# calavera/patrol

Hardware: AMD Instinct MI355X
Metric: bucket-state merges/sec + achieved HBM GB/s at 1/2/4/8 MI355X (higher is better)
Workload: dtype f64; 1 GPU; C2 merge: 100000000 replica messages -> 10000000-bucket table (2^25 slots), Zipf(1.1); keys_per_gpu=10000000, slots_per_gpu=33554432, parallelism=shard1, name_bytes=2-8 (b<id>), world_size=1, full=False, exchange=False, batches_in_hbm=28

## Files before the change

### patrol_amd/csrc/phip_engine.hip

```cpp
#include <sys/random.h>

#include <chrono>
#include <cstdlib>
#include <cstring>
#include <hip/hip_runtime.h>
#include <rocprim/rocprim.hpp>

#include <algorithm>
#include <cstdarg>
#include <cstdio>
#include <cstring>
#include <mutex>
#include <string>
#include <vector>

#include "patrolhip.h"
#include "phip_kernels.hpp"
#include "phip_host.hpp"

using namespace phip;

namespace {

#ifndef PHIP_SORT_BITS
#define PHIP_SORT_BITS 9
#endif
#ifndef PHIP_SORT_BLOCK
#define PHIP_SORT_BLOCK 1024
#endif
#ifndef PHIP_SORT_ITEMS
#define PHIP_SORT_ITEMS 8
#endif
using SlotSortConfig = rocprim::radix_sort_config<
    rocprim::default_config, rocprim::default_config,
    rocprim::radix_sort_onesweep_config<
        rocprim::kernel_config<PHIP_SORT_BLOCK, PHIP_SORT_ITEMS>,
        rocprim::kernel_config<PHIP_SORT_BLOCK, PHIP_SORT_ITEMS>, PHIP_SORT_BITS,
        rocprim::block_radix_rank_algorithm::match>>;

enum BufId {
  B_NAMES, B_OFFS, B_A, B_T, B_E, B_KIND, B_NOW, B_FREQ, B_PER, B_COUNT,
  B_STATUS, B_REM, B_HAVE, B_REPLY,
  B_BYTES, B_DOFFS, B_NOFF, B_NLEN, B_DA, B_DT, B_DE,
  B_MISS, B_MISS2, B_RETRY, B_CSLOT, B_CMSG,
  B_SLOT, B_IDX, B_SSLOT, B_SIDX, B_USLOT, B_SCNT, B_SSTART, B_LONG, B_HUGE, B_TEMP, B_DUMP,
  B_OPS, B_HOFF, B_HOP, B_HVAL, B_RPOS, B_RST, B_RUNN, B_SEGEX, B_WOFF, B_SUMS, B_WRUN,
  B_WING, B_SEGXF, B_FOLDDBG, B_SMALL, B_HUGE2, B_LONG2,
  B_STATES, B_NAME1, B_HOT, B_ROUTE, B_EXPORT, B_MSHARD, B_MSCNT, B_FSCNT, B_DEDUP, B_DSET, B_TSTATS, B_SEGT, B_RHOT,
  B_DLIST, B_DTAB, B_DMARK, B_SMAP, B_SOFF, B_SLEN, B_SA, B_ST, B_SE, B_SSTAT, B_SREP, B_NCHK,
  B_EVICT, B_ULOG, B_ULCNT, B_SWEEP, B_DIGEST, B_DIGOUT,
  B_COUNT_
};

struct DevBuf {
  void* p = nullptr;
  size_t cap = 0;
};

struct Timing {
  const char* name;
  hipEvent_t a, b;
};

enum class PassKind { kOptimistic, kClassified, kIsolating };
struct FastPass {
  PassKind kind = PassKind::kClassified;
  u32 n = 0;
  u32 par = 0;
  u32* c = nullptr;
  const HotHdr* hot = nullptr;
  const HotEntry* dir = nullptr;
  void* hot_zero = nullptr;
  bool hot_join = false;
  u8* mark = nullptr;
  UndoLog log{};
};

}

struct phip_handle {
  int device = 0;
  int ncu = 256;
  bool iso_always = false;
  u32 iso_left = 0;
  bool classify_first = false;
  u32 opt_left = 0;
  struct LastStats {
    uint64_t hot_entries = 0, hot_hits = 0, misses = 0;
    uint64_t ordered = 0;
    uint64_t log_count = 0, log_over = 0;
  } stats;
  hipStream_t stream = nullptr;
  hipStream_t own_stream = nullptr;
  hipStream_t stream2 = nullptr;
  hipStream_t stream3 = nullptr;
  hipStream_t stream4 = nullptr;
  hipEvent_t ev_t4a = nullptr, ev_t4b = nullptr;
  hipEvent_t ev_fork = nullptr, ev_join = nullptr;
  void* hot_clean = nullptr;
  hipEvent_t ev_fork3 = nullptr, ev_join3 = nullptr;
  hipEvent_t ev_gather = nullptr, ev_gather3 = nullptr;
  hipEvent_t ev_pack = nullptr;
  std::mutex mu;
  std::string err;
  u32 L = 0;
  u32 L_open = 0;
  u64 cap = 0;
  u64 max_load = 0;
  u32 load_pct = 90;
  bool grow = true;
  bool small = true;
  u64 grows = 0;
  u64 layout_gen = 1;
  u64 long_need = 0;
  Rec* recs = nullptr;
  u32* aux = nullptr;
  u8* arena = nullptr;
  u64 arena_cap = 0;
  u64 arena_open = 0;
  u64* arena_cursor = nullptr;
  u32* ctr = nullptr;
  u32* ctr_host = nullptr;
  u32* ctr_map = nullptr;
  u32 fpar = 0;
  u64 nfast = 0;
  u64 n_buckets = 0;
  u64 tag_mask = ~0ull;
  u64 seed = 0;
  DevBuf buf[B_COUNT_];
  bool timing = false;
  bool timing_accumulate = false;
  std::vector<Timing> timings;
  std::vector<Timing> event_pool;
  size_t pool_used = 0;
  u8* small_pin = nullptr;
  size_t small_pin_cap = 0;
  struct Pending {
    bool active = false;
    SoaIn<NamesOffs> in{};
    i64 now = 0;
    OutView ow{};
    FastPass pass{};
  } pend;
  hipEvent_t ev_ctr = nullptr;
  int deferred_rc = 0;
};

namespace {

int set_err(phip_handle* h, int code, const char* fmt, ...) {
  char tmp[512];
  va_list ap;
  va_start(ap, fmt);
  vsnprintf(tmp, sizeof tmp, fmt, ap);
  va_end(ap);
  if (h) h->err = tmp;
  return code;
}

#define HIPCHK(h, x)                                                                      \
  do {                                                                                    \
    hipError_t e_ = (x);                                                                  \
    if (e_ != hipSuccess)                                                                 \
      return set_err((h), PHIP_ERR_HIP, "%s failed: %s (%s:%d)", #x, hipGetErrorString(e_), \
                     __FILE__, __LINE__);                                                 \
  } while (0)

template <class T>
int ensure(phip_handle* h, BufId id, size_t count, T** out) {
  size_t bytes = std::max<size_t>(count * sizeof(T), 64) + 64;
  DevBuf& b = h->buf[id];
  if (b.cap < bytes) {
    size_t want = std::max(bytes, b.cap * 3 / 2);
    if (b.p) HIPCHK(h, hipFree(b.p));
    b.p = nullptr;
    b.cap = 0;
    HIPCHK(h, hipMalloc(&b.p, want));
    b.cap = want;
  }
  *out = (T*)b.p;
  return PHIP_OK;
}

inline Table table(phip_handle* h) {
  Table t;
  t.recs = h->recs;
  t.aux = h->aux;
  t.arena = h->arena;
  t.L = h->L;
  t.tag_mask = h->tag_mask;
  t.seed = h->seed;
  return t;
}

inline unsigned grid_for(u64 n, unsigned block = kBlock) {
  return (unsigned)std::max<u64>(1, (n + block - 1) / block);
}

struct Launch {
  phip_handle* h;
  const char* name;
  size_t idx = ~size_t(0);
  hipStream_t s;
  Launch(phip_handle* h_, const char* n, hipStream_t st = nullptr)
      : h(h_), name(n), s(st ? st : h_->stream) {
    if (!h->timing) return;
    if (h->pool_used == h->event_pool.size()) {
      Timing tm{n, nullptr, nullptr};
      if (hipEventCreate(&tm.a) != hipSuccess) return;
      if (hipEventCreate(&tm.b) != hipSuccess) {
        (void)hipEventDestroy(tm.a);
        return;
      }
      h->event_pool.push_back(tm);
    }
    idx = h->pool_used++;
    h->event_pool[idx].name = n;
    if (hipEventRecord(h->event_pool[idx].a, s) != hipSuccess) idx = ~size_t(0);
  }
  ~Launch() {
    if (idx < h->event_pool.size()) {
      Timing& t = h->event_pool[idx];
      if (hipEventRecord(t.b, s) == hipSuccess) h->timings.push_back(t);
    }
  }
};

int read_ctr(phip_handle* h) {
  HIPCHK(h, hipMemcpyAsync(h->ctr_host, h->ctr, kCtrWords * sizeof(u32), hipMemcpyDeviceToHost,
                           h->stream));
  HIPCHK(h, hipStreamSynchronize(h->stream));
  return PHIP_OK;
}

int reset_ctr(phip_handle* h) {
  k_batch_reset<<<1, kShards, 0, h->stream>>>(h->ctr, nullptr);
  HIPCHK(h, hipGetLastError());
  return PHIP_OK;
}

int check_flags(phip_handle* h) {
  if (h->ctr_host[kCtrBadName])
    return set_err(h, PHIP_ERR_INVALID, "malformed name offsets (names_len check): nothing applied");
  if (h->ctr_host[kCtrTableFull]) return set_err(h, PHIP_ERR_FULL, "hash table full (probe wrapped)");
  if (h->ctr_host[kCtrArenaFull]) return set_err(h, PHIP_ERR_ARENA, "long-name arena exhausted");
  return PHIP_OK;
}

template <int N>
int copy_words(const uint64_t (&v)[N], uint64_t* out, int max) {
  int k = 0;
  for (; k < max && k < N; ++k) out[k] = v[k];
  return k;
}

int finish_pending(phip_handle* h, bool* worked = nullptr);
int after_error(phip_handle* h, int rc);

int begin_call(phip_handle* h, bool finish_queued = true) {
  if (h->deferred_rc) {
    const int rc = h->deferred_rc;
    h->deferred_rc = 0;
    return rc;
  }
  h->err.clear();
  if (h->timing && !h->timing_accumulate) {
    h->timings.clear();
    h->pool_used = 0;
  }
  HIPCHK(h, hipSetDevice(h->device));
  if (finish_queued && h->pend.active) {
    int rc = finish_pending(h);
    if (rc) return after_error(h, rc);
  }
  return PHIP_OK;
}

template <class T>
int stage(phip_handle* h, BufId id, const T* src, size_t count, bool dev, const T** out) {
  if (!src) { *out = nullptr; return PHIP_OK; }
  if (dev) { *out = src; return PHIP_OK; }
  T* d;
  int rc = ensure(h, id, count, &d);
  if (rc) return rc;
  if (count) HIPCHK(h, hipMemcpyAsync(d, src, count * sizeof(T), hipMemcpyHostToDevice, h->stream));
  *out = d;
  return PHIP_OK;
}

template <class T>
int out_buf(phip_handle* h, BufId id, T* user, size_t count, bool dev, T** out) {
  if (!user) { *out = nullptr; return PHIP_OK; }
  if (dev) { *out = user; return PHIP_OK; }
  return ensure(h, id, count, out);
}

template <class T>
int copy_back(phip_handle* h, T* user, const T* dev_buf, size_t count, bool dev) {
  if (!user || dev || !count) return PHIP_OK;
  HIPCHK(h, hipMemcpyAsync(user, dev_buf, count * sizeof(T), hipMemcpyDeviceToHost, h->stream));
  return PHIP_OK;
}

inline u64 load_limit(u64 cap, u32 pct) { return cap * pct / 100; }

int grow_table(phip_handle* h, u32 newL) {
  const u64 ncap = 1ull << newL;
  Rec* nrecs = nullptr;
  u32* naux = nullptr;
  if (hipMalloc(&nrecs, ncap * sizeof(Rec)) != hipSuccess) {
    (void)hipGetLastError();
    return set_err(h, PHIP_ERR_FULL, "table growth to 2^%u slots: device memory", newL);
  }
  if (hipMalloc(&naux, ncap * sizeof(u32)) != hipSuccess) {
    (void)hipGetLastError();
    (void)hipFree(nrecs);
    return set_err(h, PHIP_ERR_FULL, "table growth to 2^%u slots: device memory", newL);
  }
  auto drop_new = [&](int rc) {
    (void)hipStreamSynchronize(h->stream);
    (void)hipFree(nrecs);
    (void)hipFree(naux);
    return rc;
  };
  if (hipMemsetAsync(nrecs, 0, ncap * sizeof(Rec), h->stream) != hipSuccess ||
      hipMemsetAsync(naux, 0, ncap * sizeof(u32), h->stream) != hipSuccess ||
      hipMemsetAsync(h->ctr + kCtrTableFull, 0, sizeof(u32), h->stream) != hipSuccess)
    return drop_new(set_err(h, PHIP_ERR_HIP, "table growth: clearing the new table failed"));
  Table nt = table(h);
  nt.recs = nrecs;
  nt.aux = naux;
  nt.L = newL;
  {
    Launch l(h, "k_rehash");
    k_rehash<<<grid_for(h->cap), kBlock, 0, h->stream>>>(h->recs, h->aux, h->cap, nt, h->ctr);
  }
  if (hipGetLastError() != hipSuccess)
    return drop_new(set_err(h, PHIP_ERR_HIP, "k_rehash launch failed"));
  int rc;
  if ((rc = read_ctr(h))) return drop_new(rc);
  if (h->ctr_host[kCtrTableFull])
    return drop_new(set_err(h, PHIP_ERR_INVALID, "internal: rehash probe wrapped"));
  HIPCHK(h, hipFree(h->recs));
  HIPCHK(h, hipFree(h->aux));
  h->recs = nrecs;
  h->aux = naux;
  h->L = newL;
  h->cap = ncap;
  h->max_load = load_limit(ncap, h->load_pct);
  ++h->grows;
  ++h->layout_gen;
  return PHIP_OK;
}

int grow_arena(phip_handle* h, u64 used, u64 want) {
  u64 ncap = std::max<u64>(h->arena_cap * 2, want);
  u8* na = nullptr;
  if (hipMalloc(&na, ncap + 64) != hipSuccess) {
    (void)hipGetLastError();
    return set_err(h, PHIP_ERR_ARENA, "arena growth to %llu bytes: device memory",
                   (unsigned long long)ncap);
  }
  if (used) HIPCHK(h, hipMemcpyAsync(na, h->arena, used, hipMemcpyDeviceToDevice, h->stream));
  HIPCHK(h, hipStreamSynchronize(h->stream));
  HIPCHK(h, hipFree(h->arena));
  h->arena = na;
  h->arena_cap = ncap;
  return PHIP_OK;
}

template <class Src>
int reserve(phip_handle* h, Src src, const u32* list, u32 nlist, u64 bound, bool* grew) {
  u64* lb = (u64*)(h->ctr + kCtrLongBytes);
  HIPCHK(h, hipMemsetAsync(lb, 0, sizeof(u64), h->stream));
  k_list_long_bytes<Src><<<grid_for(nlist), kBlock, 0, h->stream>>>(src, nlist, list, lb);
  HIPCHK(h, hipGetLastError());
  u64 used = 0;
  HIPCHK(h, hipMemcpyAsync(&used, h->arena_cursor, sizeof(u64), hipMemcpyDeviceToHost, h->stream));
  int rc;
  if ((rc = read_ctr(h))) return rc;
  u64 need;
  std::memcpy(&need, h->ctr_host + kCtrLongBytes, sizeof need);
  h->long_need = need;
  if (used + need > h->arena_cap) {
    if (!h->grow)
      return set_err(h, PHIP_ERR_ARENA, "long-name arena: %llu of %llu bytes used, %llu more needed",
                     (unsigned long long)used, (unsigned long long)h->arena_cap,
                     (unsigned long long)need);
    if ((rc = grow_arena(h, used, used + need))) return rc;
  }
  if (h->n_buckets + bound > h->max_load) {
    u32 L = h->L;
    while (L < 31 && h->n_buckets + bound > load_limit(1ull << L, h->load_pct)) ++L;
    if (!h->grow || h->n_buckets + bound > load_limit(1ull << L, h->load_pct))
      return set_err(h, PHIP_ERR_FULL,
                     "table load limit: %llu buckets + up to %llu new > %llu allowed in 2^%u slots",
                     (unsigned long long)h->n_buckets, (unsigned long long)bound,
                     (unsigned long long)(h->grow ? load_limit(1ull << L, h->load_pct) : h->max_load),
                     h->grow ? L : h->L);
    if ((rc = grow_table(h, L))) return rc;
    *grew = true;
  }
  return PHIP_OK;
}

template <class Src>
int dedupe_names(phip_handle* h, Src src, const u32* list, u32 n, u32** out, u32* nout);

template <class Src>
int insert_names(phip_handle* h, Src src, u32* list, u32 nlist, const int64_t* now_arr, i64 now0,
                 u32* n_claimed, bool* grew = nullptr, bool distinct = false) {
  u32 *cslot, *cmsg, *retry, *cur = list;
  int rc;
  *n_claimed = 0;
  bool g = false;
  u64 bound = nlist;
  const u32* blist = list;
  u32 nb = nlist;
  if (!distinct && nlist > 1 && h->n_buckets + nlist > h->max_load) {
    u32 *dd, nd = 0;
    if ((rc = dedupe_names(h, src, list, nlist, &dd, &nd))) return rc;
    if (h->tag_mask == ~0ull) {
      bound = nd;
      blist = dd;
      nb = nd;
    }
  }
  if ((rc = reserve(h, src, blist, nb, bound, &g))) return rc;
  if (grew) *grew = g;
  if ((rc = ensure(h, B_CSLOT, nlist, &cslot)) || (rc = ensure(h, B_CMSG, nlist, &cmsg)) ||
      (rc = ensure(h, B_RETRY, nlist, &retry)))
    return rc;
  u32 total = 0, ncur = nlist;
  HIPCHK(h, hipMemsetAsync(h->ctr + kCtrClaimed, 0, sizeof(u32), h->stream));
  u32* nxt = retry;
  u32* spare = nullptr;
  if ((rc = ensure(h, B_MISS2, nlist, &spare))) return rc;
  while (ncur > 0) {
    HIPCHK(h, hipMemsetAsync(h->ctr + kCtrRetry, 0, sizeof(u32), h->stream));
    {
      Launch l(h, "k_claim");
      k_claim<Src><<<grid_for(ncur), kBlock, 0, h->stream>>>(src, ncur, cur, table(h), cslot, cmsg,
                                                              nxt, h->ctr);
    }
    HIPCHK(h, hipGetLastError());
    if ((rc = read_ctr(h))) return rc;
    u32 claimed_total = h->ctr_host[kCtrClaimed];
    u32 fresh = claimed_total - total;
    if (fresh) {
      Launch l(h, "k_publish");
      k_publish<Src><<<grid_for(fresh), kBlock, 0, h->stream>>>(
          src, total, fresh, cslot, cmsg, table(h), h->arena, h->arena_cap, h->arena_cursor, now_arr,
          now0, h->ctr);
    }
    HIPCHK(h, hipGetLastError());
    h->n_buckets += fresh;
    total = claimed_total;
    *n_claimed = total;
    ncur = h->ctr_host[kCtrRetry];
    if ((rc = check_flags(h))) return rc;
    if (fresh == 0 && ncur != 0)
      return set_err(h, PHIP_ERR_INVALID, "internal: insert round made no progress");
    cur = nxt;
    nxt = (nxt == retry) ? spare : retry;
  }
  *n_claimed = total;
  if (h->long_need) {
    if ((rc = read_ctr(h)) || (rc = check_flags(h))) return rc;
  }
  return PHIP_OK;
}

int clear_new(phip_handle* h, u32 n_claimed) {
  if (!n_claimed) return PHIP_OK;
  u32* cslot = (u32*)h->buf[B_CSLOT].p;
  Launch l(h, "k_clear_new");
  k_clear_new<<<grid_for(n_claimed), kBlock, 0, h->stream>>>(cslot, n_claimed, table(h));
  HIPCHK(h, hipGetLastError());
  return PHIP_OK;
}

int after_error(phip_handle* h, int rc) {
  if (rc == PHIP_OK) return rc;
  if (h->stream2) (void)hipStreamSynchronize(h->stream2);
  if (h->stream3) (void)hipStreamSynchronize(h->stream3);
  if (h->stream4) (void)hipStreamSynchronize(h->stream4);
  if (rc == PHIP_ERR_HIP) return rc;
  std::string keep = h->err;
  k_clear_new_all<<<grid_for(h->cap), kBlock, 0, h->stream>>>(table(h), h->cap);
  if (hipGetLastError() == hipSuccess) (void)hipStreamSynchronize(h->stream);
  h->err = keep;
  return rc;
}

template <class Src>
int build_hot(phip_handle* h, Src src, u32 n, hipStream_t st, u8* status, const HotHdr** hdr_out,
              const HotEntry** dir_out, void** zero_out) {
  *hdr_out = nullptr;
  *dir_out = nullptr;
  *zero_out = nullptr;
  if (n < kHotMinBatch) return PHIP_OK;
  constexpr size_t kCnt = size_t(1) << kHotCntBits;
  u8* base;
  int rc;
  if ((rc = ensure(h, B_HOT, kHotZeroBytes + kHotCandMax * sizeof(u32) + sizeof(HotHdr) +
                                 kHotMax * sizeof(HotEntry), &base)))
    return rc;
  u32* ckeys = (u32*)base;
  u32* ccnt = ckeys + kCnt;
  u32* sync = ccnt + kCnt;
  u32* cand = sync + kHotSyncWords;
  HotHdr* hdr = (HotHdr*)(cand + kHotCandMax);
  HotEntry* dir = (HotEntry*)(hdr + 1);
  if (h->hot_clean != base) HIPCHK(h, hipMemsetAsync(base, 0, kHotZeroBytes, st));
  h->hot_clean = nullptr;
  const u32 stride = std::max<u32>(64, (n + kHotSampleMax - 1) / kHotSampleMax);
  const u32 nsample = (n + stride - 1) / stride;
  {
    Launch l(h, "k_hot_dir", st);
    if (status) {
      constexpr unsigned kT = kHotAloneThreads;
      const unsigned nblk = grid_for(nsample, kT);
      const unsigned fill =
          std::min<unsigned>(grid_for(n, kT * 64), 1024 / kT * (unsigned)h->ncu);
      k_hot_dir<Src, kT, 1><<<nblk + fill, kT, 0, st>>>(
          src, n, stride, nsample, table(h), ckeys, ccnt, sync, cand, hdr, dir, nblk, status);
    } else {
      const unsigned nblk = grid_for(nsample, kHotSamplePerBlock);
      k_hot_dir<Src, 256, 4><<<nblk, 256, 0, st>>>(
          src, n, stride, nsample, table(h), ckeys, ccnt, sync, cand, hdr, dir, nblk, nullptr);
    }
  }
  HIPCHK(h, hipGetLastError());
  *hdr_out = hdr;
  *dir_out = dir;
  *zero_out = base;
  return PHIP_OK;
}

inline unsigned fast_grid_on(u32 ncu, u32 n) {
  const u64 tiles = ((u64)n + kFastBlock - 1) / kFastBlock;
  return (unsigned)std::max<u64>(1, std::min<u64>(tiles, (u64)ncu * kFastPerCU));
}
inline unsigned fast_grid(phip_handle* h, u32 n) { return fast_grid_on((u32)h->ncu, n); }


int sharded(phip_handle* h, BufId base_id, u32 units, u32 per_unit, Sharded* out,
            bool zero = true) {
  int rc;
  out->cap = shard_cap(units, per_unit);
  if ((rc = ensure(h, base_id, (size_t)kShards * out->cap, &out->base)) ||
      (rc = ensure(h, B_MSCNT, 2 * kShards, &out->cnt)))
    return rc;
  if (zero) HIPCHK(h, hipMemsetAsync(out->cnt, 0, kShards * sizeof(u32), h->stream));
  return PHIP_OK;
}

int pack_sharded(phip_handle* h, const Sharded& sh, u32 total_slot, u32* out, u32* total) {
  k_shard_scan<<<1, kShards, 0, h->stream>>>(sh.cnt, h->ctr, total_slot, nullptr, 0, nullptr,
                                             nullptr);
  HIPCHK(h, hipGetLastError());
  int rc;
  if ((rc = read_ctr(h))) return rc;
  *total = h->ctr_host[total_slot];
  if (*total) {
    Launch l(h, "k_shard_compact");
    dim3 grid(grid_for(h->ctr_host[kCtrShardMax]), kShards);
    k_shard_compact<<<grid, 256, 0, h->stream>>>(sh.base, sh.cap, sh.cnt, out);
    HIPCHK(h, hipGetLastError());
  }
  return PHIP_OK;
}


enum class PassAsk { kPolicy, kMayUndo, kIsolate, kNoIsolate };

template <class In>
PassKind pass_kind(const phip_handle* h, PassAsk ask) {
  if (ask == PassAsk::kIsolate) return PassKind::kIsolating;
  if (ask == PassAsk::kNoIsolate) return PassKind::kClassified;
  if (h->iso_always || h->iso_left > 0) return PassKind::kIsolating;
  if (ask == PassAsk::kMayUndo && In::kSoa && !h->classify_first && h->opt_left == 0)
    return PassKind::kOptimistic;
  return PassKind::kClassified;
}

inline size_t undo_counts(const phip_handle* h) { return (size_t)h->ncu * kFastPerCU * (kFastBlock / 64); }

struct UndoLayout {
  u32 grid, waves, cap;
  u64 halves;
};
inline UndoLayout undo_layout(u32 n, u32 ncu) {
  UndoLayout l;
  l.grid = fast_grid_on(ncu, n);
  l.waves = l.grid * (kFastBlock / 64);
  l.cap = undo_wave_cap(n, l.grid);
  l.halves = (u64)l.waves * l.cap * 2;
  return l;
}

inline u32* fctr(phip_handle* h, u32 par) { return h->ctr + kCtrWords * (1 + par); }

inline u32* fast_counts(phip_handle* h, u32 par) {
  return (u32*)h->buf[B_FSCNT].p + par * 2 * kShards;
}

int dirty_set(phip_handle* h, DirtySet* d, u32** dlist) {
  int rc;
  u64* b;
  if ((rc = ensure(h, B_DTAB, DirtySet::kWords, &b)) || (rc = ensure(h, B_DLIST, kDirtyCap, dlist)))
    return rc;
  *d = DirtySet::at(b);
  return PHIP_OK;
}
struct SubBatch {
  uint64_t *off, *a, *t;
  int64_t* e;
  u8* len;
  u32* map;
};
int sub_batch(phip_handle* h, SubBatch* b) {
  constexpr size_t m = kSubBatchCap;
  int rc;
  if ((rc = ensure(h, B_SOFF, m, &b->off)) || (rc = ensure(h, B_SLEN, m, &b->len)) ||
      (rc = ensure(h, B_SA, m, &b->a)) || (rc = ensure(h, B_ST, m, &b->t)) ||
      (rc = ensure(h, B_SE, m, &b->e)) || (rc = ensure(h, B_SMAP, m, &b->map)))
    return rc;
  return PHIP_OK;
}

int fast_shards(phip_handle* h, u32 n, u32 par, Sharded* out) {
  int rc;
  u32* c;
  out->cap = shard_cap((n + 63) / 64, 64);
  if ((rc = ensure(h, B_MSHARD, (size_t)kShards * out->cap, &out->base)) ||
      (rc = ensure(h, B_FSCNT, 4 * kShards, &c)))
    return rc;
  out->cnt = fast_counts(h, par);
  return PHIP_OK;
}

template <class Src>
int fork_hot(phip_handle* h, Src src, FastPass* p) {
  if (p->n < kHotMinBatch) return PHIP_OK;
  HIPCHK(h, hipStreamWaitEvent(h->stream2, h->ev_fork, 0));
  int rc;
  if ((rc = build_hot(h, src, p->n, h->stream2, nullptr, &p->hot, &p->dir, &p->hot_zero))) return rc;
  HIPCHK(h, hipEventRecord(h->ev_join, h->stream2));
  p->hot_join = true;
  return PHIP_OK;
}

template <class HotSrc>
int front_optimistic(phip_handle* h, HotSrc hsrc, u8* status, FastPass* p) {
  int rc;
  if ((rc = ensure(h, B_ULCNT, undo_counts(h), &p->log.cnt))) return rc;
  if (p->n >= kHotMinBatch && status)
    return build_hot(h, hsrc, p->n, h->stream, status, &p->hot, &p->dir, &p->hot_zero);
  if (status) HIPCHK(h, hipMemsetAsync(status, PHIP_ST_MERGED, p->n, h->stream));
  if (p->n >= kHotMinBatch) HIPCHK(h, hipEventRecord(h->ev_fork, h->stream));
  return fork_hot(h, hsrc, p);
}

template <class In, class HotSrc>
int front_classified(phip_handle* h, In in, HotSrc hsrc, u8* status, FastPass* p) {
  int rc;
  const u32 n = p->n;
  u32* dlist = nullptr;
  DirtySet dset;
  if ((rc = dirty_set(h, &dset, &dlist))) return rc;
  if (p->kind == PassKind::kIsolating) {
    p->mark = status;
    if (!status) {
      if ((rc = ensure(h, B_DMARK, n, &p->mark))) return rc;
      HIPCHK(h, hipMemsetAsync(p->mark, 0, n, h->stream));
    }
  }
  const bool hot_first = n < (1u << 23);
  if (n >= kHotMinBatch) HIPCHK(h, hipEventRecord(h->ev_fork, h->stream));
  if (hot_first && (rc = fork_hot(h, hsrc, p))) return rc;
  {
    bool done = false;
    if constexpr (In::kSoa) {
      if ((((uintptr_t)in.ma | (uintptr_t)in.mt) & 15) == 0) {
        Launch l(h, "k_classify");
        NamesOffs chk{};
        if constexpr (In::kOffs) chk = in.src;
        k_classify_soa2<<<grid_for((n + 1) / 2), kBlock, 0, h->stream>>>(in.ma, in.mt, in.me, n,
                                                                          p->c, status, chk, dlist);
        done = true;
      }
    }
    if (!done) {
      if (status) HIPCHK(h, hipMemsetAsync(status, PHIP_ST_MERGED, n, h->stream));
      Launch l(h, "k_classify");
      k_classify<In><<<grid_for(n), kBlock, 0, h->stream>>>(in, n, p->c, dlist);
    }
  }
  HIPCHK(h, hipGetLastError());
  return hot_first ? PHIP_OK : fork_hot(h, hsrc, p);
}

template <class In, class HotSrc>
int fast_begin(phip_handle* h, In in, HotSrc hsrc, u32 n, u8* status, PassAsk ask, bool reset,
               FastPass* p) {
  int rc;
  u32* c;
  *p = FastPass{};
  p->kind = pass_kind<In>(h, ask);
  p->n = n;
  if ((rc = ensure(h, B_FSCNT, 4 * kShards, &c))) return rc;
  p->par = h->fpar ^= 1u;
  p->c = fctr(h, p->par);
  ++h->nfast;
  if (reset) {
    k_batch_reset<<<1, kShards, 0, h->stream>>>(p->c, fast_counts(h, p->par));
    HIPCHK(h, hipGetLastError());
  }
  if (p->kind == PassKind::kOptimistic) return front_optimistic(h, hsrc, status, p);
  return front_classified(h, in, hsrc, status, p);
}

template <class In>
int fast_back(phip_handle* h, In in, FastPass& p, bool queued) {
  const u32 n = p.n;
  const bool iso = p.kind == PassKind::kIsolating;
  u32* miss;
  int rc;
  Sharded msh;
  DirtySet dset{};
  SubBatch sb{};
  u32* dlist = nullptr;
  if ((rc = ensure(h, B_MISS, n, &miss)) || (rc = fast_shards(h, n, p.par, &msh))) return rc;
  if (iso) {
    if ((rc = dirty_set(h, &dset, &dlist)) || (rc = sub_batch(h, &sb))) return rc;
    Launch l(h, "k_dirty_build");
    k_dirty_build<In><<<1, 1024, 0, h->stream>>>(in, n, p.c, dlist, dset, table(h));
    HIPCHK(h, hipGetLastError());
  }
  if (p.hot_join) HIPCHK(h, hipStreamWaitEvent(h->stream, h->ev_join, 0));
  switch (p.kind) {
    case PassKind::kOptimistic:
      if constexpr (In::kSoa) {
        const UndoLayout ul = undo_layout(n, (u32)h->ncu);
        p.log.cap = ul.cap;
        if ((rc = ensure(h, B_ULOG, (size_t)ul.halves, &p.log.base))) return rc;
        Launch l(h, "k_receive_fast");
        k_receive_fast<In, true><<<ul.grid, kFastBlock, 0, h->stream>>>(
            in, 0, n, table(h), msh, p.c, p.hot, p.dir, nullptr, nullptr, p.log,
            (uint4*)p.hot_zero);
      }
      break;
    case PassKind::kClassified:
    case PassKind::kIsolating: {
      Launch l(h, "k_receive_fast");
      k_receive_fast<In><<<fast_grid(h, n), kFastBlock, 0, h->stream>>>(
          in, 0, n, table(h), msh, p.c, p.hot, p.dir, iso ? dset.key : nullptr, p.mark,
          UndoLog{}, (uint4*)p.hot_zero);
    }
  }
  HIPCHK(h, hipGetLastError());
  if (p.hot_zero) h->hot_clean = p.hot_zero;
  if (iso) {
    {
      Launch l(h, "k_dirty_pass");
      const unsigned g = (unsigned)std::max<u64>(
          1, std::min<u64>(((u64)n + 1023) / 1024, (u64)h->ncu * 2));
      k_dirty_pass<In><<<g, 1024, 0, h->stream>>>(in, n, p.c, p.mark, dset.key, table(h), msh);
      HIPCHK(h, hipGetLastError());
    }
    k_batch_end<In><<<1, kShards, 0, h->stream>>>(
        in, p.c, dset.key, table(h),
        SubOut{sb.off, sb.len, sb.a, sb.t, sb.e, sb.map, kSubBatchCap}, msh.cnt, h->ctr_map,
        kCtrWords, queued ? fast_counts(h, p.par ^ 1u) : nullptr, fctr(h, p.par ^ 1u));
  } else {
    k_shard_scan<<<1, kShards, 0, h->stream>>>(msh.cnt, p.c, kCtrMiss, h->ctr_map, kCtrWords,
                                               queued ? fast_counts(h, p.par ^ 1u) : nullptr,
                                               fctr(h, p.par ^ 1u));
  }
  HIPCHK(h, hipGetLastError());
  HIPCHK(h, hipEventRecord(h->ev_ctr, h->stream));
  if (!queued) HIPCHK(h, hipEventSynchronize(h->ev_ctr));
  return PHIP_OK;
}

constexpr u32 kIsoKeep = 256;
constexpr u32 kOptBackoff = 256;

bool apply_policy(phip_handle* h, const FastPass& p) {
  const u32* c = h->ctr_host;
  if (p.kind == PassKind::kOptimistic) {
    h->stats.log_count = c[kCtrLogCount];
    h->stats.log_over = c[kCtrLogOver];
    if (c[kCtrLogOver]) h->opt_left = kOptBackoff;
    if (c[kCtrDirty] < p.n || c[kCtrStop] < p.n || c[kCtrLogOver]) return true;
  } else if (h->opt_left) {
    --h->opt_left;
  }
  if (c[kCtrDirty] < p.n) h->iso_left = kIsoKeep;
  else if (h->iso_left) --h->iso_left;
  return false;
}

struct FastOutcome {
  u32 first_dirty = 0;
  u32 nmiss = 0;
  u32 stop = 0;
  u32 ndef = 0;
  bool iso_ran = false;
  bool again = false;
};

int fast_collect(phip_handle* h, const FastPass& p, FastOutcome* o) {
  int rc;
  if ((rc = check_flags(h))) return rc;
  o->nmiss = h->ctr_host[kCtrMiss];
  if (o->nmiss) {
    Sharded msh;
    if ((rc = fast_shards(h, p.n, p.par, &msh))) return rc;
    Launch l(h, "k_shard_compact");
    dim3 grid(grid_for(h->ctr_host[kCtrShardMax]), kShards);
    k_shard_compact<<<grid, 256, 0, h->stream>>>(msh.base, msh.cap, msh.cnt,
                                                 (u32*)h->buf[B_MISS].p);
    HIPCHK(h, hipGetLastError());
  }
  const u32 nd = h->ctr_host[kCtrNDirty];
  o->iso_ran = p.kind == PassKind::kIsolating;
  const bool apart = o->iso_ran && nd != 0 && nd <= kDirtyCap;
  o->first_dirty = apart ? p.n : std::min<u32>(h->ctr_host[kCtrDirty], p.n);
  o->stop = std::min<u32>(h->ctr_host[kCtrStop], p.n);
  o->ndef = apart ? h->ctr_host[kCtrNDefer] : 0;
  h->stats.ordered = 0;
  h->stats.hot_entries = h->ctr_host[kCtrHotEntries];
  h->stats.hot_hits = h->ctr_host[kCtrHotHits];
  h->stats.misses = o->nmiss;
  return PHIP_OK;
}

template <class In, class HotSrc>
int fast_settle(phip_handle* h, In in, HotSrc hsrc, u8* status, FastPass* p, FastOutcome* o) {
  int rc;
  o->again = apply_policy(h, *p);
  if (o->again) {
    {
      Launch l(h, "k_undo");
      k_undo<<<fast_grid(h, p->n) * (kFastBlock / 64), 256, 0, h->stream>>>(p->log, table(h));
      HIPCHK(h, hipGetLastError());
    }
    if ((rc = fast_begin(h, in, hsrc, p->n, status, PassAsk::kPolicy, true, p)) ||
        (rc = fast_back(h, in, *p, false)))
      return rc;
    (void)apply_policy(h, *p);
  }
  return fast_collect(h, *p, o);
}

template <class In, class HotSrc>
int fast_apply(phip_handle* h, In in, HotSrc hsrc, u32 n, u8* status, PassAsk ask,
               FastOutcome* o) {
  int rc;
  FastPass p;
  if ((rc = fast_begin(h, in, hsrc, n, status, ask, true, &p)) ||
      (rc = fast_back(h, in, p, false)))
    return rc;
  return fast_settle(h, in, hsrc, status, &p, o);
}

template <class Src>
int dedupe_names(phip_handle* h, Src src, const u32* list, u32 n, u32** out, u32* nout) {
  int rc;
  u32 setbits = 1;
  while ((1ull << setbits) < 2ull * n) ++setbits;
  u64* set;
  Sharded dsh;
  if ((rc = ensure(h, B_DSET, size_t(1) << setbits, &set)) ||
      (rc = ensure(h, B_DEDUP, n, out)) ||
      (rc = sharded(h, B_MSHARD, grid_for(n), kBlock, &dsh)))
    return rc;
  HIPCHK(h, hipMemsetAsync(set, 0, (size_t(1) << setbits) * sizeof(u64), h->stream));
  {
    Launch l(h, "k_dedupe");
    k_dedupe<Src><<<grid_for(n), kBlock, 0, h->stream>>>(src, n, list, table(h), set, setbits, dsh);
    HIPCHK(h, hipGetLastError());
  }
  return pack_sharded(h, dsh, kCtrAux, *out, nout);
}

template <class Src>
int finish_many_misses(phip_handle* h, Src src, const uint64_t* a, const uint64_t* t,
                       const int64_t* e, u32 prefix, i64 now, u8* status, FastOutcome* o) {
  u32* miss = (u32*)h->buf[B_MISS].p;
  const u32 nmiss = o->nmiss;
  int rc;
  u32 *dedup, nd = 0;
  if ((rc = dedupe_names(h, src, miss, nmiss, &dedup, &nd))) return rc;
  u32 n_claimed = 0;
  if ((rc = insert_names(h, src, dedup, nd, nullptr, now, &n_claimed, nullptr, true))) return rc;
  if (status) {
    Launch l(h, "k_first_seen");
    k_first_seen<Src><<<grid_for(nmiss), kBlock, 0, h->stream>>>(src, nmiss, miss, table(h));
    HIPCHK(h, hipGetLastError());
  }
  FastOutcome o2;
  if ((rc = fast_apply(h, SoaIn<Src>{src, a, t, e}, src, prefix, status,
                       o->iso_ran ? PassAsk::kIsolate : PassAsk::kNoIsolate, &o2)))
    return rc;
  o->nmiss = o2.nmiss;
  o->ndef = o2.ndef;
  if (status && n_claimed) {
    Launch l(h, "k_mark_created");
    k_mark_created_slots<<<grid_for(n_claimed), kBlock, 0, h->stream>>>(
        (const u32*)h->buf[B_CSLOT].p, n_claimed, table(h), status);
    HIPCHK(h, hipGetLastError());
  }
  return clear_new(h, n_claimed);
}

template <class Src>
int finish_misses(phip_handle* h, Src src, const uint64_t* a, const uint64_t* t, const int64_t* e,
                  i64 now, u8* status, FastOutcome* o) {
  if (o->nmiss == 0) return PHIP_OK;
  int rc;
  if (o->nmiss >= kManyMisses &&
      (rc = finish_many_misses(h, src, a, t, e, std::min(o->stop, o->first_dirty), now, status, o)))
    return rc;
  const u32 nmiss = o->nmiss;
  if (nmiss == 0) return PHIP_OK;
  u32* miss = (u32*)h->buf[B_MISS].p;
  u32 n_claimed = 0;
  if ((rc = insert_names(h, src, miss, nmiss, nullptr, now, &n_claimed))) return rc;
  HIPCHK(h, hipMemsetAsync(h->ctr + kCtrMiss, 0, sizeof(u32), h->stream));
  u32* miss2;
  if ((rc = ensure(h, B_MISS2, nmiss, &miss2))) return rc;
  {
    Launch l(h, "k_receive_list");
    k_receive_list<Src><<<grid_for(nmiss), kBlock, 0, h->stream>>>(
        src, a, t, e, nmiss, miss, table(h), status, miss2, h->ctr);
  }
  HIPCHK(h, hipGetLastError());
  {
    Launch l(h, "k_mark_created");
    k_mark_created<Src><<<grid_for(nmiss), kBlock, 0, h->stream>>>(src, nmiss, miss, table(h),
                                                                    status);
  }
  HIPCHK(h, hipGetLastError());
  if ((rc = read_ctr(h))) return rc;
  if (const u32 left = h->ctr_host[kCtrMiss])
    return set_err(h, PHIP_ERR_INVALID, "internal: %u names missing after insert", left);
  return clear_new(h, n_claimed);
}


#define PHIP_OUT_DISPATCH(mask, CALL) \
  switch (mask) {                     \
    case 0: CALL(0); break;           \
    case 1: CALL(1); break;           \
    case 2: CALL(2); break;           \
    case 3: CALL(3); break;           \
    case 4: CALL(4); break;           \
    case 5: CALL(5); break;           \
    case 6: CALL(6); break;           \
    case 7: CALL(7); break;           \
    case 8: CALL(8); break;           \
    case 9: CALL(9); break;           \
    case 10: CALL(10); break;         \
    case 11: CALL(11); break;         \
    case 12: CALL(12); break;         \
    case 13: CALL(13); break;         \
    case 14: CALL(14); break;         \
    default: CALL(15); break;         \
  }

template <class Src>
int resolve_all(phip_handle* h, Src src, u32 n, const int64_t* now_arr, i64 now0, u32** slot_out,
                u32* n_claimed, SortVals sv = SortVals{nullptr, 0, nullptr}) {
  u32 *slot, *miss;
  int rc;
  Sharded rsh;
  if ((rc = ensure(h, B_SLOT, n, &slot)) || (rc = ensure(h, B_MISS, n, &miss)) ||
      (rc = sharded(h, B_MSHARD, grid_for(n), kBlock, &rsh)))
    return rc;
  if ((rc = reset_ctr(h))) return rc;
  {
    Launch l(h, "k_resolve");
    k_resolve_batch<Src><<<grid_for(n, kBlock * kResPer), kBlock, 0, h->stream>>>(
        src, n, table(h), slot, rsh, h->ctr, sv);
  }
  HIPCHK(h, hipGetLastError());
// ... 269 lines not shown
int stage_names(phip_handle* h, const uint8_t* names, const uint32_t* offs, u32 n, bool dev,
                NamesOffs* src, u32 names_len = 0) {
  const u32* d_offs;
  int rc;
  if ((rc = stage(h, B_OFFS, offs, (size_t)n + 1, dev, &d_offs))) return rc;
  const u8* d_names;
  size_t nb = 0;
  if (!dev) nb = offs[n];
  if ((rc = stage(h, B_NAMES, names, nb, dev, &d_names))) return rc;
  if (!dev && nb == 0) {
    u8* p;
    if ((rc = ensure(h, B_NAMES, 1, &p))) return rc;
    d_names = p;
  }
  src->blob = d_names;
  src->offs = d_offs;
  src->lim = dev ? names_len : 0;
  return PHIP_OK;
}

bool datagrams_ok(const uint64_t* offs, u32 n) {
  for (u32 i = 0; i < n; ++i)
    if (offs[i + 1] < offs[i]) return false;
  return true;
}

bool names_ok(const uint32_t* offs, u32 n) {
  for (u32 i = 0; i < n; ++i) {
    if (offs[i + 1] < offs[i]) return false;
    if (offs[i + 1] - offs[i] > PHIP_MAX_NAME_LEN) return false;
  }
  return true;
}

int outputs(phip_handle* h, const phip_results* res, u32 n, bool dev, OutView* ow) {
  int rc;
  phip_results r{};
  if (res) r = *res;
  if ((rc = out_buf(h, B_STATUS, r.status, n, dev, &ow->status)) ||
      (rc = out_buf(h, B_REM, r.remaining, n, dev, &ow->remaining)) ||
      (rc = out_buf(h, B_HAVE, r.have, n, dev, &ow->have)) ||
      (rc = out_buf(h, B_REPLY, r.reply, n, dev, &ow->reply)))
    return rc;
  if (ow->reply) HIPCHK(h, hipMemsetAsync(ow->reply, 0, (size_t)n * sizeof(phip_state), h->stream));
  return PHIP_OK;
}

int copy_outputs(phip_handle* h, const phip_results* res, u32 n, bool dev, const OutView& ow) {
  if (!res || dev) {
    HIPCHK(h, hipStreamSynchronize(h->stream));
    return PHIP_OK;
  }
  int rc;
  if ((rc = copy_back(h, res->status, ow.status, n, dev)) ||
      (rc = copy_back(h, res->remaining, ow.remaining, n, dev)) ||
      (rc = copy_back(h, res->have, ow.have, n, dev)) ||
      (rc = copy_back(h, res->reply, ow.reply, n, dev)))
    return rc;
  HIPCHK(h, hipStreamSynchronize(h->stream));
  return PHIP_OK;
}

inline NamesOffs shifted(NamesOffs s, u32 k) {
  s.offs += k;
  return s;
}
inline NamesPairs shifted(NamesPairs s, u32 k) {
  s.off += k;
  s.len += k;
  return s;
}
inline OutView shifted(OutView o, u32 k) {
  if (o.status) o.status += k;
  if (o.remaining) o.remaining += k;
  if (o.have) o.have += k;
  if (o.reply) o.reply += k;
  return o;
}

template <class Src>
int run_deferred(phip_handle* h, Src src, i64 now, const OutView& ow, u32 nd) {
  if (nd > kSubBatchCap) {
    h->stats.ordered = 0;
    return set_err(h, PHIP_ERR_HIP, "ordered sub-batch over its %u entries", kSubBatchCap);
  }
  h->stats.ordered = nd;
  if (nd == 0) return PHIP_OK;
  int rc;
  SubBatch sb;
  u8* st2 = nullptr;
  phip_state* rep2 = nullptr;
  if ((rc = sub_batch(h, &sb)) || (ow.status && (rc = ensure(h, B_SSTAT, nd, &st2))) ||
      (ow.reply && (rc = ensure(h, B_SREP, nd, &rep2))))
    return rc;
  if (rep2) HIPCHK(h, hipMemsetAsync(rep2, 0, (size_t)nd * sizeof(phip_state), h->stream));
  OpView ov{};
  ov.kind = nullptr; ov.kind0 = PHIP_OP_RECEIVE;
  ov.now = nullptr; ov.now0 = now;
  ov.a = sb.a; ov.t = sb.t; ov.e = sb.e;
  if ((rc = ordered(h, NamesPairs{src.blob, sb.off, sb.len}, nd, ov,
                    OutView{st2, nullptr, nullptr, rep2})))
    return rc;
  if (st2 || rep2) {
    k_defer_scatter<<<grid_for(nd), kBlock, 0, h->stream>>>(sb.map, nd, st2, rep2, ow);
    HIPCHK(h, hipGetLastError());
  }
  return PHIP_OK;
}

template <class Src>
int finish_receive(phip_handle* h, Src src, const uint64_t* a, const uint64_t* t,
                   const int64_t* e, i64 now, const OutView& ow, FastOutcome o) {
  int rc;
  const bool deferred = o.ndef != 0;
  if ((rc = finish_misses(h, src, a, t, e, now, ow.status, &o))) return rc;
  if (deferred) return run_deferred(h, src, now, ow, o.ndef);
  const u32 stop = o.stop, k = o.first_dirty;
  h->stats.ordered = k < stop ? stop - k : 0;
  if (k >= stop) return PHIP_OK;
  OpView ov{};
  ov.kind = nullptr; ov.kind0 = PHIP_OP_RECEIVE;
  ov.now = nullptr; ov.now0 = now;
  ov.a = a + k; ov.t = t + k; ov.e = e + k;
  return ordered(h, shifted(src, k), stop - k, ov, shifted(ow, k));
}

int fill_stopped(phip_handle* h, u8* status, u32 n, u32 stop) {
  if (!status || stop >= n) return PHIP_OK;
  HIPCHK(h, hipMemsetAsync(status + stop, PHIP_ST_NOT_PROCESSED, n - stop, h->stream));
  HIPCHK(h, hipMemsetAsync(status + stop, PHIP_ST_SHORT, 1, h->stream));
  return PHIP_OK;
}

int stopped_at_bad_name(phip_handle* h, const OutView& ow, u32 n, u32 stop) {
  if (stop >= n) return PHIP_OK;
  if (int rc = fill_stopped(h, ow.status, n, stop)) return rc;
  if (ow.status) HIPCHK(h, hipStreamSynchronize(h->stream));
  return set_err(h, PHIP_ERR_INVALID,
                 "malformed name offsets at message %u (names_len check): the batch stopped there",
                 stop);
}

template <class Src>
int receive_decoded(phip_handle* h, Src src, const uint64_t* a, const uint64_t* t,
                    const int64_t* e, u32 n, i64 now, const OutView& ow, PassAsk ask) {
  int rc;
  FastOutcome o;
  if ((rc = fast_apply(h, SoaIn<Src>{src, a, t, e}, src, n, ow.status, ask, &o)) ||
      (rc = finish_receive(h, src, a, t, e, now, ow, o)))
    return rc;
  return stopped_at_bad_name(h, ow, n, o.stop);
}

int finish_pending(phip_handle* h, bool* worked) {
  if (worked) *worked = false;
  if (!h->pend.active) return PHIP_OK;
  phip_handle::Pending p = h->pend;
  h->pend.active = false;
  HIPCHK(h, hipEventSynchronize(h->ev_ctr));
  int rc;
  FastOutcome o;
  if ((rc = fast_settle(h, p.in, p.in.src, p.ow.status, &p.pass, &o))) return rc;
  if (!o.again && o.nmiss == 0 && o.first_dirty >= o.stop && o.ndef == 0)
    return stopped_at_bad_name(h, p.ow, p.pass.n, o.stop);
  if (worked) *worked = true;
  if ((rc = finish_receive(h, p.in.src, p.in.ma, p.in.mt, p.in.me, p.now, p.ow, o)) ||
      (rc = stopped_at_bad_name(h, p.ow, p.pass.n, o.stop)))
    return rc;
  HIPCHK(h, hipStreamSynchronize(h->stream));
  return PHIP_OK;
}

inline bool has_reply_state(u8 status, u8 kind) {
  const u8 st = status & 0x7F;
  return kind == PHIP_OP_TAKE || kind == PHIP_OP_UPSERT || st == PHIP_ST_INCAST_REPLY ||
         st == PHIP_ST_INCAST_NOREPLY;
}

int small_mixed(phip_handle* h, const phip_ops* ops, const phip_results* res, bool* done) {
  *done = false;
  const u32 n = ops->n;
  if (n > kSmallMax || h->n_buckets + n > h->max_load) return PHIP_OK;
  const u64 nbytes = ops->name_offs[n];
  if (nbytes > (u64)kSmallMax * PHIP_MAX_NAME_LEN) return PHIP_OK;
  auto al = [](size_t x) { return (x + 15) & ~(size_t)15; };
  const bool take = ops->freq != nullptr, state = ops->added != nullptr;
  const size_t o_kind = al(4 * ((size_t)n + 1)), o_now = o_kind + al(n), o_freq = o_now + 8 * n;
  const size_t o_per = o_freq + 8 * n, o_count = o_per + 8 * n, o_a = o_count + 8 * n;
  const size_t o_t = o_a + 8 * n, o_e = o_t + 8 * n, o_names = o_e + 8 * n;
  const size_t in_bytes = al(o_names + nbytes + 8);
  const size_t o_st = sizeof(SmallHdr), o_rem = al(o_st + n), o_have = o_rem + 8 * n;
  const size_t o_reply = o_have + 8 * n, out_bytes = o_reply + sizeof(phip_state) * n;
  const size_t total = in_bytes + out_bytes;
  if (h->small_pin_cap < total) {
    if (h->small_pin) HIPCHK(h, hipHostFree(h->small_pin));
    h->small_pin = nullptr;
    h->small_pin_cap = 0;
    const size_t want = std::max<size_t>(total, 1 << 20);
    HIPCHK(h, hipHostMalloc(&h->small_pin, want, 0));
    h->small_pin_cap = want;
  }
  u8 *d = nullptr, *pin = h->small_pin;
  int rc;
  if ((rc = ensure(h, B_SMALL, total, &d))) return rc;
  std::memcpy(pin, ops->name_offs, 4 * ((size_t)n + 1));
  std::memcpy(pin + o_kind, ops->kind, n);
  std::memcpy(pin + o_now, ops->now, 8 * n);
  if (take) {
    std::memcpy(pin + o_freq, ops->freq, 8 * n);
    std::memcpy(pin + o_per, ops->per, 8 * n);
    std::memcpy(pin + o_count, ops->count, 8 * n);
  }
  if (state) {
    std::memcpy(pin + o_a, ops->added, 8 * n);
    std::memcpy(pin + o_t, ops->taken, 8 * n);
    std::memcpy(pin + o_e, ops->elapsed, 8 * n);
  }
  std::memcpy(pin + o_names, ops->names, nbytes);
  std::memset(pin + o_names + nbytes, 0, 8);
  std::memset(pin + in_bytes, 0, sizeof(SmallHdr));
  HIPCHK(h, hipMemcpyAsync(d, pin, in_bytes + sizeof(SmallHdr), hipMemcpyHostToDevice, h->stream));
  NamesOffs src{d + o_names, (const u32*)d};
  OpView ov{};
  ov.kind = d + o_kind;
  ov.now = (const int64_t*)(d + o_now);
  if (take) {
    ov.freq = (const int64_t*)(d + o_freq);
    ov.per = (const int64_t*)(d + o_per);
    ov.count = (const uint64_t*)(d + o_count);
  }
  if (state) {
    ov.a = (const uint64_t*)(d + o_a);
    ov.t = (const uint64_t*)(d + o_t);
    ov.e = (const int64_t*)(d + o_e);
  }
  u8* dout = d + in_bytes;
  phip_results r{};
  if (res) r = *res;
  OutView ow{};
  ow.status = r.status ? dout + o_st : nullptr;
  ow.remaining = r.remaining ? (uint64_t*)(dout + o_rem) : nullptr;
  ow.have = r.have ? (uint64_t*)(dout + o_have) : nullptr;
  ow.reply = r.reply ? (phip_state*)(dout + o_reply) : nullptr;
  {
    Launch l(h, "k_small_mixed");
    k_small_mixed<<<1, kSmallMax, 0, h->stream>>>(src, ov, n, table(h), h->arena, h->arena_cap,
                                                  h->arena_cursor, ow, (SmallHdr*)dout);
  }
  HIPCHK(h, hipGetLastError());
  const size_t back = r.reply ? out_bytes : r.have ? o_reply : r.remaining ? o_have : o_rem;
  u8* pout = pin + in_bytes;
  HIPCHK(h, hipMemcpyAsync(pout, dout, back, hipMemcpyDeviceToHost, h->stream));
  HIPCHK(h, hipStreamSynchronize(h->stream));
  SmallHdr hd;
  std::memcpy(&hd, pout, sizeof hd);
  h->n_buckets += hd.created;
  if (hd.fallback) return PHIP_OK;
  if (hd.full) return set_err(h, PHIP_ERR_FULL, "internal: small batch probe wrapped the table");
  if (r.status) std::memcpy(r.status, pout + o_st, n);
  if (r.remaining) std::memcpy(r.remaining, pout + o_rem, 8 * n);
  if (r.have) std::memcpy(r.have, pout + o_have, 8 * n);
  if (r.reply) {
    const phip_state* src_r = (const phip_state*)(pout + o_reply);
    std::vector<u8> st;
    const u8* stp = r.status;
    if (!stp) {
      st.assign(n, 0);
      HIPCHK(h, hipMemcpy(st.data(), dout + o_st, n, hipMemcpyDeviceToHost));
      stp = st.data();
    }
    for (u32 i = 0; i < n; ++i)
      r.reply[i] = has_reply_state(stp[i], ops->kind ? ops->kind[i] : (u8)PHIP_OP_RECEIVE)
                       ? src_r[i] : phip_state{};
  }
  *done = true;
  return PHIP_OK;
}


int small_uniform(phip_handle* h, const phip_msgs* m, u8 kind, int64_t now, const phip_results* res,
                  bool* done) {
  *done = false;
  if (!h->small || m->n > kSmallMax) return PHIP_OK;
  std::vector<u8> kinds(m->n, kind);
  std::vector<int64_t> nows(m->n, now);
  phip_ops ops{};
  ops.n = m->n;
  ops.kind = kinds.data();
  ops.names = m->names;
  ops.name_offs = m->name_offs;
  ops.now = nows.data();
  ops.added = m->added;
  ops.taken = m->taken;
  ops.elapsed = m->elapsed;
  return small_mixed(h, &ops, res, done);
}

int small_datagrams(phip_handle* h, const uint8_t* bytes, const uint64_t* offs, uint32_t n,
                    int64_t now, const phip_results* res, uint32_t* stop_index, bool* done) {
  *done = false;
  if (!h->small || n > kSmallMax) return PHIP_OK;
  std::vector<uint64_t> a(n), t(n);
  std::vector<int64_t> e(n);
  std::vector<uint32_t> no(n + 1);
  std::vector<uint8_t> names;
  names.reserve((size_t)n * 16 + 8);
  auto be64 = [](const uint8_t* p) {
    uint64_t v = 0;
    for (int k = 0; k < 8; ++k) v = (v << 8) | p[k];
    return v;
  };
  u32 stop = n;
// ... 115 lines not shown
  u8 *base, *temp;
  RouteCells c;
  size_t tb;
  int rc;
  if ((rc = route_scratch(h, n, world, &base, &c.pctr, &tb, &temp))) return rc;
  c.cnt = (u32*)base;
  c.bytes = c.cnt + p.cells;
  c.cbase = c.bytes + p.cells;
  c.bbase = c.cbase + p.cells;
  c.code = (u16*)(c.bbase + p.cells);
  count(p, c);
  HIPCHK(h, hipGetLastError());
  {
    Launch l(h, "route_scan", st);
    HIPCHK(h, rocprim::exclusive_scan(temp, tb, c.cnt, c.cbase, 0u, p.cells, rocprim::plus<u32>(),
                                      st));
    HIPCHK(h, rocprim::exclusive_scan(temp, tb, c.bytes, c.bbase, 0u, p.cells, rocprim::plus<u32>(),
                                      st));
  }
  scatter(p, c);
  k_route_totals<<<1, kRouteMaxWorld, 0, st>>>(c.cnt, c.bytes, c.cbase, c.bbase, p.ntile, world,
                                               counts, nbytes);
  HIPCHK(h, hipGetLastError());
  return PHIP_OK;
}

static int route_pack_on(phip_handle* h, hipStream_t st, const phip_msgs& m, u32 world, const void* dir,
                  uint8_t* send_names, uint32_t* send_lens, uint64_t* send_added,
                  uint64_t* send_taken, int64_t* send_elapsed, uint64_t* counts,
                  uint64_t* nbytes) {
  const u32 n = m.n;
  const HotHdr* hot = (const HotHdr*)dir;
  const RouteHot* rdir = hot ? (const RouteHot*)(hot + 1) : nullptr;
  NamesOffs src{m.names, m.name_offs, m.names_len};
  return route_pack_with(
      h, st, n, world, counts, nbytes,
      [&](const RoutePlan& p, const RouteCells& c) {
        k_batch_reset<<<1, kShards, 0, st>>>(c.pctr, nullptr);
        Launch l(h, "k_route_count", st);
        k_route_count<NamesOffs><<<p.nblk, kRouteBlock, 0, st>>>(
            src, m.added, m.taken, m.elapsed, n, p.span, world, p.ntile, hot, rdir, c.pctr, c.code,
            c.cnt, c.bytes, hot ? kRouteCombine : kRoutePlain);
        if (hot)
          k_route_count<NamesOffs><<<p.nblk, kRouteBlock, 0, st>>>(
              src, m.added, m.taken, m.elapsed, n, p.span, world, p.ntile, hot, rdir, c.pctr, c.code,
              c.cnt, c.bytes, kRouteRecount);
      },
      [&](const RoutePlan& p, const RouteCells& c) {
        Launch l(h, "k_route_scatter", st);
        k_route_scatter<NamesOffs><<<p.nblk, kRouteBlock, 0, st>>>(
            src, m.added, m.taken, m.elapsed, n, p.span, world, p.ntile, hot, rdir, c.pctr, c.code,
            c.cbase, c.bbase, send_names, send_lens, send_added, send_taken, send_elapsed);
      });
}

static int route_pack_ops_on(phip_handle* h, hipStream_t st, const phip_ops& ops, u32 world,
                             uint8_t* send_names, uint32_t* send_lens, uint8_t* send_kind,
                             int64_t* send_now, uint64_t* send_x0, uint64_t* send_x1,
                             uint64_t* send_x2, uint32_t* send_src, uint64_t* counts,
                             uint64_t* nbytes) {
  const u32 n = ops.n;
  NamesOffs src{ops.names, ops.name_offs, ops.names_len};
  const RouteOps ro{ops.kind, ops.now, ops.freq, ops.per, ops.count, ops.added, ops.taken,
                    ops.elapsed};
  return route_pack_with(
      h, st, n, world, counts, nbytes,
      [&](const RoutePlan& p, const RouteCells& c) {
        Launch l(h, "k_route_ops_count", st);
        k_route_ops_count<NamesOffs><<<p.nblk, kRouteBlock, 0, st>>>(src, n, p.span, world, p.ntile,
                                                                      c.code, c.cnt, c.bytes);
      },
      [&](const RoutePlan& p, const RouteCells& c) {
        Launch l(h, "k_route_ops_scatter", st);
        k_route_ops_scatter<NamesOffs><<<p.nblk, kRouteBlock, 0, st>>>(
            src, ro, n, p.span, world, p.ntile, c.code, c.cbase, c.bbase, send_names, send_lens,
            send_kind, send_now, send_x0, send_x1, send_x2, send_src);
      });
}

static int check_offsets_on(phip_handle* h, hipStream_t st, const uint8_t* names,
                            const uint32_t* name_offs, u32 names_len, u32 n, u32* first_bad) {
  *first_bad = ~0u;
  if (n == 0 || names_len == 0) return PHIP_OK;
  u32* d;
  int rc;
  if ((rc = ensure(h, B_NCHK, 1, &d))) return rc;
  HIPCHK(h, hipMemsetAsync(d, 0xFF, sizeof(u32), st));
  {
    Launch l(h, "k_offs_check", st);
    k_offs_check<<<grid_for(n), kBlock, 0, st>>>(NamesOffs{names, name_offs, names_len}, n, d);
  }
  HIPCHK(h, hipGetLastError());
  HIPCHK(h, hipMemcpyAsync(first_bad, d, sizeof(u32), hipMemcpyDeviceToHost, st));
  HIPCHK(h, hipStreamSynchronize(st));
  return PHIP_OK;
}

extern "C" {

int phip_abi_version(void) { return PHIP_ABI_VERSION; }

#ifdef PHIP_BUILD_ID
const char* phip_build_id(void) { return PHIP_BUILD_ID; }
#endif

int phip_open(const phip_config* cfg, phip_handle** out) {
  if (!cfg || !out) return PHIP_ERR_INVALID;
  *out = nullptr;
  if (cfg->log2_slots < 4 || cfg->log2_slots > 31) return PHIP_ERR_INVALID;
  int ndev = 0;
  if (hipGetDeviceCount(&ndev) != hipSuccess || ndev == 0) return PHIP_ERR_NO_DEVICE;
  if (cfg->device < 0 || cfg->device >= ndev) return PHIP_ERR_NO_DEVICE;
  phip_handle* h = new phip_handle;
  h->device = cfg->device;
  h->L = h->L_open = cfg->log2_slots;
  h->cap = 1ull << h->L;
  h->load_pct = cfg->max_load_pct ? std::min<u32>(cfg->max_load_pct, 95) : 90;
  h->max_load = load_limit(h->cap, h->load_pct);
  h->grow = !(cfg->flags & PHIP_CFG_NO_GROW);
  h->iso_always = cfg->flags & PHIP_CFG_ISOLATE;
  h->classify_first = cfg->flags & PHIP_CFG_CLASSIFY_FIRST;
  h->small = !(cfg->flags & PHIP_CFG_NO_SMALL);
  h->arena_cap = h->arena_open = cfg->arena_bytes ? cfg->arena_bytes : (1ull << 20);
  if (cfg->debug_tag_bits && cfg->debug_tag_bits < 64) h->tag_mask = (1ull << cfg->debug_tag_bits) - 1;
  if (cfg->flags & PHIP_CFG_FIXED_SEED) {
    h->seed = cfg->hash_seed;
  } else if (getrandom(&h->seed, sizeof h->seed, 0) != (ssize_t)sizeof h->seed) {
    h->seed = seeded_mix((u64)std::chrono::steady_clock::now().time_since_epoch().count(),
                         (u64)(uintptr_t)h);
  }
  auto fail = [&](hipError_t e) {
    phip_close(h);
    (void)e;
    return PHIP_ERR_HIP;
  };
  hipError_t e;
  if ((e = hipSetDevice(h->device)) != hipSuccess) return fail(e);
  if ((e = hipDeviceGetAttribute(&h->ncu, hipDeviceAttributeMultiprocessorCount, h->device)) !=
      hipSuccess)
    return fail(e);
  if ((e = hipStreamCreateWithFlags(&h->own_stream, hipStreamNonBlocking)) != hipSuccess)
    return fail(e);
  h->stream = h->own_stream;
  if ((e = hipStreamCreateWithFlags(&h->stream2, hipStreamNonBlocking)) != hipSuccess) return fail(e);
  if ((e = hipStreamCreateWithFlags(&h->stream3, hipStreamNonBlocking)) != hipSuccess) return fail(e);
  if ((e = hipEventCreateWithFlags(&h->ev_fork, hipEventDisableTiming)) != hipSuccess) return fail(e);
  if ((e = hipEventCreateWithFlags(&h->ev_join, hipEventDisableTiming)) != hipSuccess) return fail(e);
  if ((e = hipEventCreateWithFlags(&h->ev_fork3, hipEventDisableTiming)) != hipSuccess) return fail(e);
  if ((e = hipEventCreateWithFlags(&h->ev_join3, hipEventDisableTiming)) != hipSuccess) return fail(e);
  if ((e = hipEventCreateWithFlags(&h->ev_gather, hipEventDisableTiming)) != hipSuccess) return fail(e);
  if ((e = hipEventCreateWithFlags(&h->ev_gather3, hipEventDisableTiming)) != hipSuccess)
    return fail(e);
  if ((e = hipEventCreateWithFlags(&h->ev_pack, hipEventDisableTiming)) != hipSuccess) return fail(e);
  if ((e = hipEventCreateWithFlags(&h->ev_ctr, hipEventDisableTiming)) != hipSuccess) return fail(e);
  if ((e = hipMalloc(&h->recs, h->cap * sizeof(Rec))) != hipSuccess) return fail(e);
  if ((e = hipMalloc(&h->aux, h->cap * sizeof(u32))) != hipSuccess) return fail(e);
  if ((e = hipMalloc(&h->arena, h->arena_cap + 64)) != hipSuccess) return fail(e);
  if ((e = hipMalloc(&h->arena_cursor, 64)) != hipSuccess) return fail(e);
  if ((e = hipMalloc(&h->ctr, 3 * kCtrWords * sizeof(u32))) != hipSuccess) return fail(e);
  if ((e = hipHostMalloc(&h->ctr_host, kCtrWords * sizeof(u32),
                         hipHostMallocMapped | hipHostMallocCoherent)) != hipSuccess ||
      (e = hipHostGetDevicePointer((void**)&h->ctr_map, h->ctr_host, 0)) != hipSuccess)
    return fail(e);
  if ((e = hipMemsetAsync(h->recs, 0, h->cap * sizeof(Rec), h->stream)) != hipSuccess) return fail(e);
  if ((e = hipMemsetAsync(h->aux, 0, h->cap * sizeof(u32), h->stream)) != hipSuccess) return fail(e);
  if ((e = hipMemsetAsync(h->arena_cursor, 0, 64, h->stream)) != hipSuccess) return fail(e);
  if ((e = hipMemsetAsync(h->ctr, 0, 3 * kCtrWords * sizeof(u32), h->stream)) != hipSuccess)
    return fail(e);
  if ((e = hipStreamSynchronize(h->stream)) != hipSuccess) return fail(e);
  *out = h;
  return PHIP_OK;
}

void phip_close(phip_handle* h) {
  if (!h) return;
  (void)hipSetDevice(h->device);
  if (h->pend.active) (void)after_error(h, finish_pending(h));
  if (h->stream) (void)hipStreamSynchronize(h->stream);
  if (h->stream2) (void)hipStreamSynchronize(h->stream2);
  if (h->stream3) (void)hipStreamSynchronize(h->stream3);
  if (h->stream4) (void)hipStreamSynchronize(h->stream4);
  for (auto& b : h->buf)
    if (b.p) (void)hipFree(b.p);
  for (auto& t : h->event_pool) {
    (void)hipEventDestroy(t.a);
    (void)hipEventDestroy(t.b);
  }
  if (h->recs) (void)hipFree(h->recs);
  if (h->aux) (void)hipFree(h->aux);
  if (h->arena) (void)hipFree(h->arena);
  if (h->arena_cursor) (void)hipFree(h->arena_cursor);
  if (h->ctr) (void)hipFree(h->ctr);
  if (h->ctr_host) (void)hipHostFree(h->ctr_host);
  if (h->small_pin) (void)hipHostFree(h->small_pin);
  if (h->ev_fork) (void)hipEventDestroy(h->ev_fork);
  if (h->ev_join) (void)hipEventDestroy(h->ev_join);
  if (h->ev_fork3) (void)hipEventDestroy(h->ev_fork3);
  if (h->ev_join3) (void)hipEventDestroy(h->ev_join3);
  if (h->ev_gather) (void)hipEventDestroy(h->ev_gather);
  if (h->ev_gather3) (void)hipEventDestroy(h->ev_gather3);
  if (h->ev_pack) (void)hipEventDestroy(h->ev_pack);
  if (h->ev_ctr) (void)hipEventDestroy(h->ev_ctr);
  if (h->stream2) (void)hipStreamDestroy(h->stream2);
  if (h->stream3) (void)hipStreamDestroy(h->stream3);
  if (h->stream4) (void)hipStreamDestroy(h->stream4);
  if (h->ev_t4a) (void)hipEventDestroy(h->ev_t4a);
  if (h->ev_t4b) (void)hipEventDestroy(h->ev_t4b);
  if (h->own_stream) {
    (void)hipStreamSynchronize(h->own_stream);
    (void)hipStreamDestroy(h->own_stream);
  }
  delete h;
}

const char* phip_last_error(const phip_handle* h) { return h ? h->err.c_str() : "null handle"; }

int phip_flush(phip_handle* h) {
  if (!h) return PHIP_ERR_INVALID;
  std::lock_guard<std::mutex> g(h->mu);
  if (int rc0 = begin_call(h)) return rc0;
  HIPCHK(h, hipStreamSynchronize(h->stream));
  return PHIP_OK;
}

uint64_t phip_len(phip_handle* h) {
  if (!h) return 0;
  std::lock_guard<std::mutex> g(h->mu);
  if (!h->deferred_rc) h->deferred_rc = begin_call(h);
  return h->n_buckets;
}
uint64_t phip_capacity(phip_handle* h) {
  if (!h) return 0;
  std::lock_guard<std::mutex> g(h->mu);
  if (!h->deferred_rc) h->deferred_rc = begin_call(h);
  return h->cap;
}

int phip_seed(phip_handle* h, const uint8_t* names, const uint32_t* name_offs, uint32_t n,
              const phip_state* states, uint32_t flags) {
  if (!h || (n && (!names || !name_offs || !states))) return PHIP_ERR_INVALID;
  std::lock_guard<std::mutex> g(h->mu);
  if (int rc0 = begin_call(h)) return rc0;
  if (n == 0) return PHIP_OK;
  bool dev = flags & PHIP_DEVICE_PTRS;
  if (!dev && !names_ok(name_offs, n)) return set_err(h, PHIP_ERR_NAME_TOO_LARGE, "name > 231 bytes");
  int rc;
  NamesOffs src;
  if ((rc = stage_names(h, names, name_offs, n, dev, &src))) return rc;
  const phip_state* d_st;
  if ((rc = stage(h, B_STATES, states, n, dev, &d_st))) return rc;
  u32* slot;
  u32 n_claimed = 0;
  if ((rc = resolve_all(h, src, n, nullptr, 0, &slot, &n_claimed))) return after_error(h, rc);
  k_seed_finish<<<grid_for(n), kBlock, 0, h->stream>>>(slot, n, table(h));
  k_seed_pick<<<grid_for(n), kBlock, 0, h->stream>>>(slot, n, table(h));
  k_seed_apply<<<grid_for(n), kBlock, 0, h->stream>>>(slot, n, d_st, table(h));
  k_seed_finish<<<grid_for(n), kBlock, 0, h->stream>>>(slot, n, table(h));
  HIPCHK(h, hipGetLastError());
  HIPCHK(h, hipStreamSynchronize(h->stream));
  return PHIP_OK;
}

int phip_get(phip_handle* h, const uint8_t* name, uint32_t len, phip_state* out) {
  if (!h || (!name && len) || !out) return PHIP_ERR_INVALID;
  if (len > PHIP_MAX_NAME_LEN) return 0;
  std::lock_guard<std::mutex> g(h->mu);
  if (int rc0 = begin_call(h)) return rc0;
  u8* d_name;
  Rec* d_rec;
  int rc;
  if ((rc = ensure(h, B_NAME1, 256 + sizeof(Rec) + 16, &d_name))) return rc;
  d_rec = (Rec*)(d_name + 256);
  int* d_found = (int*)(d_name + 256 + sizeof(Rec));
  if (len) HIPCHK(h, hipMemcpyAsync(d_name, name, len, hipMemcpyHostToDevice, h->stream));
  k_get_one<<<1, 64, 0, h->stream>>>(d_name, len, table(h), d_rec, d_found);
  HIPCHK(h, hipGetLastError());
  Rec r;
  int found = 0;
  HIPCHK(h, hipMemcpyAsync(&r, d_rec, sizeof(Rec), hipMemcpyDeviceToHost, h->stream));
  HIPCHK(h, hipMemcpyAsync(&found, d_found, sizeof(int), hipMemcpyDeviceToHost, h->stream));
  HIPCHK(h, hipStreamSynchronize(h->stream));
  if (!found) return 0;
  out->added = dec_f64(r.added);
  out->taken = dec_f64(r.taken);
  out->elapsed = r.elapsed;
  out->created = r.created;
  return 1;
}

struct SnapHeader {
  char magic[8];
  u32 abi, log2_slots;
  u64 n_buckets, arena_used, rec_bytes, reserved[3];
};
static_assert(sizeof(SnapHeader) == 64, "snapshot header");
constexpr char kSnapMagic[8] = {'P', 'H', 'I', 'P', 'S', 'N', 'P', '1'};

static u64 arena_used(phip_handle* h) {
  u64 used = 0;
  if (hipMemcpyAsync(&used, h->arena_cursor, sizeof(u64), hipMemcpyDeviceToHost, h->stream) !=
          hipSuccess ||
      hipStreamSynchronize(h->stream) != hipSuccess)
    return ~0ull;
  return std::min<u64>(used, h->arena_cap);
}

uint64_t phip_snapshot_bytes(phip_handle* h) {
  if (!h) return 0;
  std::lock_guard<std::mutex> g(h->mu);
  if (begin_call(h)) return 0;
  const u64 used = arena_used(h);
  if (used == ~0ull) return 0;
  return sizeof(SnapHeader) + h->cap * sizeof(Rec) + used;
}

int phip_snapshot(phip_handle* h, uint8_t* out, uint64_t cap) {
  if (!h || !out) return PHIP_ERR_INVALID;
  std::lock_guard<std::mutex> g(h->mu);
  if (int rc0 = begin_call(h)) return rc0;
  const u64 used = arena_used(h);
  if (used == ~0ull) return set_err(h, PHIP_ERR_HIP, "snapshot: arena cursor read failed");
  const u64 need = sizeof(SnapHeader) + h->cap * sizeof(Rec) + used;
  if (cap < need) return set_err(h, PHIP_ERR_INVALID, "snapshot needs %llu bytes", (unsigned long long)need);
  SnapHeader hd{};
  std::memcpy(hd.magic, kSnapMagic, 8);
  hd.abi = PHIP_ABI_VERSION;
  hd.log2_slots = h->L;
  hd.n_buckets = h->n_buckets;
  hd.arena_used = used;
  hd.rec_bytes = sizeof(Rec);
  hd.reserved[0] = h->seed;
  std::memcpy(out, &hd, sizeof hd);
  u8* p = out + sizeof hd;
  HIPCHK(h, hipMemcpyAsync(p, h->recs, h->cap * sizeof(Rec), hipMemcpyDeviceToHost, h->stream));
  if (used) HIPCHK(h, hipMemcpyAsync(p + h->cap * sizeof(Rec), h->arena, used, hipMemcpyDeviceToHost, h->stream));
  HIPCHK(h, hipStreamSynchronize(h->stream));
  return PHIP_OK;
}

int phip_restore(phip_handle* h, const uint8_t* in, uint64_t len) {
  if (!h || !in || len < sizeof(SnapHeader)) return PHIP_ERR_INVALID;
  std::lock_guard<std::mutex> g(h->mu);
  if (int rc0 = begin_call(h)) return rc0;
  SnapHeader hd;
  std::memcpy(&hd, in, sizeof hd);
  if (std::memcmp(hd.magic, kSnapMagic, 8) || hd.abi != PHIP_ABI_VERSION || hd.rec_bytes != sizeof(Rec))
    return set_err(h, PHIP_ERR_INVALID, "not a snapshot of this ABI");
  if (hd.log2_slots < 4 || hd.log2_slots > 31)
    return set_err(h, PHIP_ERR_INVALID, "snapshot of 2^%u slots", hd.log2_slots);
  const u64 scap = 1ull << hd.log2_slots;
  if (len != sizeof hd + scap * sizeof(Rec) + hd.arena_used)
    return set_err(h, PHIP_ERR_INVALID, "snapshot truncated");
  if (hd.n_buckets > load_limit(scap, h->load_pct))
    return set_err(h, PHIP_ERR_FULL, "snapshot above the handle's load limit");
  if (hd.arena_used > h->arena_cap) {
    if (!h->grow) return set_err(h, PHIP_ERR_ARENA, "snapshot arena larger than the handle's");
    if (int rc = grow_arena(h, 0, hd.arena_used)) return rc;
  }
  if (hd.log2_slots != h->L) {
    Rec* nrecs = nullptr;
    u32* naux = nullptr;
    if (hipMalloc(&nrecs, scap * sizeof(Rec)) != hipSuccess ||
        hipMalloc(&naux, scap * sizeof(u32)) != hipSuccess) {
      (void)hipGetLastError();
      if (nrecs) (void)hipFree(nrecs);
      return set_err(h, PHIP_ERR_FULL, "restore: no device memory for 2^%u slots", hd.log2_slots);
    }
    HIPCHK(h, hipStreamSynchronize(h->stream));
    HIPCHK(h, hipFree(h->recs));
    HIPCHK(h, hipFree(h->aux));
    h->recs = nrecs;
    h->aux = naux;
    h->L = hd.log2_slots;
    h->cap = scap;
    h->max_load = load_limit(scap, h->load_pct);
  }
  ++h->layout_gen;
  const u8* p = in + sizeof hd;
  HIPCHK(h, hipMemcpyAsync(h->recs, p, h->cap * sizeof(Rec), hipMemcpyHostToDevice, h->stream));
  if (hd.arena_used)
    HIPCHK(h, hipMemcpyAsync(h->arena, p + h->cap * sizeof(Rec), hd.arena_used, hipMemcpyHostToDevice, h->stream));
  HIPCHK(h, hipMemsetAsync(h->aux, 0, h->cap * sizeof(u32), h->stream));
  HIPCHK(h, hipMemcpyAsync(h->arena_cursor, &hd.arena_used, sizeof(u64), hipMemcpyHostToDevice, h->stream));
  HIPCHK(h, hipStreamSynchronize(h->stream));
  h->n_buckets = hd.n_buckets;
  h->seed = hd.reserved[0];
  return PHIP_OK;
}

int phip_export_datagrams(phip_handle* h, const uint8_t* names, const uint32_t* name_offs,
                          uint32_t n, uint8_t* out, uint8_t* found, uint32_t flags) {
  if (!h || (n && (!names || !name_offs || !out || !found))) return PHIP_ERR_INVALID;
  std::lock_guard<std::mutex> g(h->mu);
  if (int rc0 = begin_call(h)) return rc0;
  if (n == 0) return PHIP_OK;
  const bool dev = flags & PHIP_DEVICE_PTRS;
  if (!dev && !names_ok(name_offs, n)) return set_err(h, PHIP_ERR_NAME_TOO_LARGE, "name > 231 bytes");
  int rc;
  NamesOffs src;
  if ((rc = stage_names(h, names, name_offs, n, dev, &src))) return rc;
  const size_t nbytes = dev ? 0 : (size_t)PHIP_BUCKET_FIXED_SIZE * n + (name_offs[n] - name_offs[0]);
  u8 *d_out, *d_found;
  if ((rc = out_buf(h, B_EXPORT, out, nbytes, dev, &d_out)) ||
      (rc = out_buf(h, B_STATUS, found, n, dev, &d_found)))
    return rc;
  {
    Launch l(h, "k_export");
    k_export<<<grid_for(n), kBlock, 0, h->stream>>>(src, n, table(h), d_out, d_found);
  }
  HIPCHK(h, hipGetLastError());
  if ((rc = copy_back(h, out, d_out, nbytes, dev)) || (rc = copy_back(h, found, d_found, n, dev)))
    return rc;
  HIPCHK(h, hipStreamSynchronize(h->stream));
  return PHIP_OK;
}

int phip_dump(phip_handle* h, uint8_t* names, uint64_t names_cap, uint64_t* name_offs,
              phip_state* states, uint64_t max_n, uint64_t* n_out, uint64_t* names_bytes_out) {
  if (!h) return PHIP_ERR_INVALID;
  std::lock_guard<std::mutex> g(h->mu);
  if (int rc0 = begin_call(h)) return rc0;
  int rc;
  u32* list;
  if ((rc = reset_ctr(h))) return rc;
  k_dump_collect<<<grid_for(h->cap), kBlock, 0, h->stream>>>(h->recs, h->cap, nullptr, h->ctr);
  HIPCHK(h, hipGetLastError());
  if ((rc = read_ctr(h))) return rc;
  const u32 occupied = h->ctr_host[kCtrOccupied];
  if ((rc = ensure(h, B_DUMP, (size_t)occupied + 1, &list))) return rc;
  if ((rc = reset_ctr(h))) return rc;
  k_dump_collect<<<grid_for(h->cap), kBlock, 0, h->stream>>>(h->recs, h->cap, list, h->ctr);
  HIPCHK(h, hipGetLastError());
  if ((rc = read_ctr(h))) return rc;
  u32 n = h->ctr_host[kCtrOccupied];
  if (n != occupied) return set_err(h, PHIP_ERR_INVALID, "internal: table changed during dump");
  Rec* d_out;
  if ((rc = ensure(h, B_TEMP, (size_t)n * sizeof(Rec), (u8**)&d_out))) return rc;
  k_dump_gather<<<grid_for(n), kBlock, 0, h->stream>>>(list, n, h->recs, d_out);
  HIPCHK(h, hipGetLastError());
  std::vector<Rec> recs(n);
  if (n) HIPCHK(h, hipMemcpyAsync(recs.data(), d_out, n * sizeof(Rec), hipMemcpyDeviceToHost, h->stream));
  HIPCHK(h, hipStreamSynchronize(h->stream));
  std::vector<u8> arena;
  u64 cursor = 0;
  HIPCHK(h, hipMemcpy(&cursor, h->arena_cursor, 8, hipMemcpyDeviceToHost));
  cursor = std::min(cursor, h->arena_cap);
  if (cursor) {
    arena.resize(cursor);
    HIPCHK(h, hipMemcpy(arena.data(), h->arena, cursor, hipMemcpyDeviceToHost));
  }
  u64 total = 0;
  for (auto& r : recs) total += r.name0 & 0xFF;
  if (n_out) *n_out = n;
  if (names_bytes_out) *names_bytes_out = total;
  if (!names) return PHIP_OK;
  if (total > names_cap || n > max_n || !name_offs || !states)
    return set_err(h, PHIP_ERR_INVALID, "dump buffers too small");
  u64 o = 0;
  for (u32 k = 0; k < n; ++k) {
    const Rec& r = recs[k];
    u32 len = r.name0 & 0xFF;
    name_offs[k] = o;
    if (len <= kInlineName) {
      const u64 w[3] = {r.name0, r.name1, r.name2};
      for (u32 j = 0; j < len; ++j) names[o + j] = (u8)(w[(j + 2) >> 3] >> (((j + 2) & 7) * 8));
    } else {
      u64 aoff = r.name0 >> 32;
      if (aoff + len <= arena.size()) std::memcpy(names + o, arena.data() + aoff, len);
    }
    o += len;
    states[k].added = dec_f64(r.added);
    states[k].taken = dec_f64(r.taken);
    states[k].elapsed = r.elapsed;
    states[k].created = r.created;
  }
  name_offs[n] = o;
  return PHIP_OK;
}

int phip_receive_soa(phip_handle* h, const phip_msgs* m, int64_t now, const phip_results* res,
                     uint32_t flags) {
  if (!h || !m) return PHIP_ERR_INVALID;
  std::lock_guard<std::mutex> g(h->mu);
  bool dev = flags & PHIP_DEVICE_PTRS;
  u32 n = m->n;
  const PassAsk ask = (flags & PHIP_RECV_CLASSIFY) ? PassAsk::kPolicy : PassAsk::kMayUndo;
  if ((flags & PHIP_RECV_ASYNC) && dev && n >= kHotMinBatch && m->names && m->name_offs &&
      m->added && m->taken && m->elapsed) {
    if (int rc0 = begin_call(h, false)) return rc0;
    NamesOffs src{m->names, m->name_offs, m->names_len};
    SoaIn<NamesOffs> in{src, m->added, m->taken, m->elapsed};
    OutView ow{};
    FastPass pass;
    int rc;
    bool worked = false;
    if ((rc = outputs(h, res, n, true, &ow))) return rc;
    const bool prev = h->pend.active;
    if ((rc = fast_begin(h, in, src, n, ow.status, ask, !prev, &pass)))
      return after_error(h, rc);
    const u64 nfast = h->nfast, grows = h->grows;
    if (prev && (rc = finish_pending(h, &worked))) return after_error(h, rc);
    if (worked && (h->nfast != nfast || h->grows != grows) &&
        (rc = fast_begin(h, in, src, n, ow.status, ask, true, &pass)))
      return after_error(h, rc);
    if ((rc = fast_back(h, in, pass, true))) return after_error(h, rc);
    h->pend = {true, in, now, ow, pass};
    return PHIP_OK;
  }
  if (int rc0 = begin_call(h)) return rc0;
  if (n == 0) return PHIP_OK;
  if (!m->names || !m->name_offs || !m->added || !m->taken || !m->elapsed) return PHIP_ERR_INVALID;
  if (!dev && !names_ok(m->name_offs, n)) return set_err(h, PHIP_ERR_NAME_TOO_LARGE, "name > 231 bytes");
  int rc;
  if (!dev) {
    bool done = false;
    if ((rc = small_uniform(h, m, PHIP_OP_RECEIVE, now, res, &done))) return after_error(h, rc);
    if (done) return PHIP_OK;
  }
  NamesOffs src;
  const uint64_t *a, *t;
  const int64_t* e;
  OutView ow{};
  if ((rc = stage_names(h, m->names, m->name_offs, n, dev, &src, m->names_len)) ||
      (rc = stage(h, B_A, m->added, n, dev, &a)) || (rc = stage(h, B_T, m->taken, n, dev, &t)) ||
      (rc = stage(h, B_E, m->elapsed, n, dev, &e)) || (rc = outputs(h, res, n, dev, &ow)))
    return rc;
  if ((rc = receive_decoded(h, src, a, t, e, n, now, ow, ask))) return after_error(h, rc);
  return copy_outputs(h, res, n, dev, ow);
}

}

namespace {
int receive_datagrams_dev(phip_handle* h, const u8* d_bytes, const uint64_t* d_offs, u32 n,
                          int64_t now, const phip_results* res, uint32_t* stop_index, bool dev) {
  int rc;
  OutView ow{};
  if ((rc = outputs(h, res, n, dev, &ow))) return rc;
  FastOutcome o;
  if ((rc = fast_apply(h, WireIn{d_bytes, d_offs}, Datagrams{d_bytes, d_offs}, n, ow.status,
                       PassAsk::kPolicy, &o)))
    return after_error(h, rc);
  const u32 stop = o.stop;
  if ((rc = fill_stopped(h, ow.status, n, stop))) return rc;
  if (o.first_dirty < stop || o.nmiss || o.ndef) {
    uint64_t *a, *t, *no;
    int64_t* e;
    u8* nl;
    if ((rc = ensure(h, B_DA, n, &a)) || (rc = ensure(h, B_DT, n, &t)) ||
        (rc = ensure(h, B_DE, n, &e)) || (rc = ensure(h, B_NOFF, n, &no)) ||
        (rc = ensure(h, B_NLEN, n, &nl)))
      return rc;
    if (o.first_dirty < stop || o.nmiss) {
      Launch l(h, "k_decode");
      k_decode<<<grid_for(stop), kBlock, 0, h->stream>>>(d_bytes, d_offs, stop, a, t, e, no, nl,
                                                          h->ctr);
      HIPCHK(h, hipGetLastError());
    }
    if ((rc = finish_receive(h, NamesPairs{d_bytes, no, nl}, a, t, e, now, ow, o)))
      return after_error(h, rc);
  }
  if ((rc = copy_outputs(h, res, n, dev, ow))) return rc;
  if (dev) HIPCHK(h, hipStreamSynchronize(h->stream));
  if (stop_index) *stop_index = stop;
  if (stop < n) return set_err(h, PHIP_ERR_SHORT_BUFFER, "short buffer at datagram %u", stop);
  return PHIP_OK;
}
}

extern "C" {

int phip_receive_datagrams(phip_handle* h, const uint8_t* bytes, const uint64_t* offs, uint32_t n,
                           int64_t now, const phip_results* res, uint32_t* stop_index,
                           uint32_t flags) {
  if (!h || (n && (!bytes || !offs))) return PHIP_ERR_INVALID;
  std::lock_guard<std::mutex> g(h->mu);
  if (int rc0 = begin_call(h)) return rc0;
  if (stop_index) *stop_index = n;
  if (n == 0) return PHIP_OK;
  bool dev = flags & PHIP_DEVICE_PTRS;
  int rc;
  const uint64_t* d_offs;
  const u8* d_bytes;
  if (!dev && !datagrams_ok(offs, n))
    return set_err(h, PHIP_ERR_INVALID, "datagram offsets decrease");
  if (!dev) {
    bool done = false;
    rc = small_datagrams(h, bytes, offs, n, now, res, stop_index, &done);
    if (done || (rc && rc != PHIP_ERR_SHORT_BUFFER)) return rc == PHIP_ERR_SHORT_BUFFER ? rc : after_error(h, rc);
  }
  if ((rc = stage(h, B_DOFFS, offs, (size_t)n + 1, dev, &d_offs))) return rc;
  size_t nb = dev ? 0 : offs[n];
  if ((rc = stage(h, B_BYTES, bytes, nb, dev, &d_bytes))) return rc;
  return receive_datagrams_dev(h, d_bytes, d_offs, n, now, res, stop_index, dev);
}

struct phip_ring {
  phip_handle* h = nullptr;
  hipStream_t copy = nullptr;
  std::mutex mu;
  u32 max_msgs = 0;
  u64 max_bytes = 0;
  enum State { kFree, kAcquired, kSubmitted };
  struct Slot {
    u8* hbytes = nullptr;
    uint64_t* hoffs = nullptr;
    u8* dbytes = nullptr;
    uint64_t* doffs = nullptr;
    hipEvent_t copied = nullptr;
    u32 n = 0;
    State state = kFree;
  };
  std::vector<Slot> slots;
  u32 next_acquire = 0, next_receive = 0;
  std::string err;
};

void phip_ring_close(phip_ring* r) {
  if (!r) return;
  (void)hipSetDevice(r->h->device);
  if (r->copy) (void)hipStreamSynchronize(r->copy);
  for (auto& s : r->slots) {
    if (s.hbytes) (void)hipHostFree(s.hbytes);
    if (s.hoffs) (void)hipHostFree(s.hoffs);
    if (s.dbytes) (void)hipFree(s.dbytes);
    if (s.doffs) (void)hipFree(s.doffs);
    if (s.copied) (void)hipEventDestroy(s.copied);
  }
  if (r->copy) (void)hipStreamDestroy(r->copy);
  delete r;
}

int phip_ring_open(phip_handle* h, uint32_t nslots, uint32_t max_msgs, uint64_t max_bytes,
                   phip_ring** out) {
  if (!out) return PHIP_ERR_INVALID;
  *out = nullptr;
  if (!h || nslots < 1 || nslots > 64 || max_msgs < 1 || max_bytes < 1) return PHIP_ERR_INVALID;
  std::lock_guard<std::mutex> g(h->mu);
  if (int rc0 = begin_call(h)) return rc0;
  phip_ring* r = new phip_ring;
  r->h = h;
  r->max_msgs = max_msgs;
  r->max_bytes = max_bytes;
  r->slots.resize(nslots);
  auto fail = [&](hipError_t e, const char* what) {
    set_err(h, PHIP_ERR_HIP, "phip_ring_open: %s failed: %s", what, hipGetErrorString(e));
    phip_ring_close(r);
    return PHIP_ERR_HIP;
  };
  hipError_t e;
  if ((e = hipStreamCreateWithFlags(&r->copy, hipStreamNonBlocking)) != hipSuccess)
    return fail(e, "hipStreamCreate");
// ... 593 lines not shown
            h->recs, s0, s_end, now, idle_ns, tile_cnt, tile_bytes, ctr, SweepParts<false>{});
    }
    {
      Launch l(h, "k_sweep_scan");
      k_sweep_scan<<<1, kSweepBlock, 0, h->stream>>>(tile_cnt, tile_bytes, ntiles, ctr);
    }
    HIPCHK(h, hipGetLastError());
    u8* d_out = out;
    u64* d_offs = reinterpret_cast<u64*>(offs);
    if (!dev) {
      HIPCHK(h, hipMemcpyAsync(c, ctr, sizeof c, hipMemcpyDeviceToHost, h->stream));
      HIPCHK(h, hipStreamSynchronize(h->stream));
      if ((rc = ensure(h, B_EXPORT, (size_t)std::min<u64>(out_cap, c[kSwBytes]), &d_out)) ||
          (rc = ensure(h, B_OFFS, (size_t)std::min<u64>(max_msgs, c[kSwN]) + 1, &d_offs)))
        return rc;
    }
    {
      Launch l(h, "k_sweep_write");
      if (parts)
        k_sweep_write<true><<<ntiles, kSweepBlock, 0, h->stream>>>(
            h->recs, h->arena, h->arena_cap, s0, s_end, now, idle_ns, tile_cnt, tile_bytes,
            max_msgs, budget, d_out, d_offs, ctr, sp);
      else
        k_sweep_write<false><<<ntiles, kSweepBlock, 0, h->stream>>>(
            h->recs, h->arena, h->arena_cap, s0, s_end, now, idle_ns, tile_cnt, tile_bytes,
            max_msgs, budget, d_out, d_offs, ctr, SweepParts<false>{});
    }
    HIPCHK(h, hipGetLastError());
    HIPCHK(h, hipMemcpyAsync(c, ctr, sizeof c, hipMemcpyDeviceToHost, h->stream));
    HIPCHK(h, hipStreamSynchronize(h->stream));
    if (c[kSwErr]) return set_err(h, PHIP_ERR_INVALID, "internal: sweep met a long name outside the arena");
    if (c[kSwN] > max_msgs || c[kSwBytes] > budget)
      return set_err(h, PHIP_ERR_INVALID, "internal: sweep wrote %llu datagrams, %llu bytes",
                     (unsigned long long)c[kSwN], (unsigned long long)c[kSwBytes]);
    s.n = c[kSwN];
    s.bytes = c[kSwBytes];
    if (c[kSwNext] != ~0ull) next = c[kSwNext];
    if (!dev) {
      if (s.bytes) HIPCHK(h, hipMemcpyAsync(out, d_out, s.bytes, hipMemcpyDeviceToHost, h->stream));
      HIPCHK(h, hipMemcpyAsync(offs, d_offs, (s.n + 1) * sizeof(u64), hipMemcpyDeviceToHost,
                               h->stream));
      HIPCHK(h, hipStreamSynchronize(h->stream));
    }
  } else if (dev) {
    HIPCHK(h, hipMemsetAsync(offs, 0, sizeof(u64), h->stream));
    HIPCHK(h, hipStreamSynchronize(h->stream));
  } else {
    offs[0] = 0;
  }
  cur->slot = next;
  cur->layout = h->layout_gen;
  s.done = next >= h->cap;
  *st = s;
  return PHIP_OK;
}

int phip_export_sweep(phip_handle* h, phip_sweep_cursor* cur, int64_t now, int64_t idle_ns,
                      uint8_t* out, uint64_t out_cap, uint64_t* offs, uint32_t max_msgs,
                      phip_sweep_stats* st, uint32_t flags) {
  return export_sweep(h, cur, now, idle_ns, false, 0, nullptr, out, out_cap, offs, max_msgs, st,
                      flags);
}

int phip_export_sweep_parts(phip_handle* h, phip_sweep_cursor* cur, int64_t now, int64_t idle_ns,
                            uint32_t log2_parts, const uint64_t* part_mask, uint8_t* out,
                            uint64_t out_cap, uint64_t* offs, uint32_t max_msgs,
                            phip_sweep_stats* st, uint32_t flags) {
  return export_sweep(h, cur, now, idle_ns, true, log2_parts, part_mask, out, out_cap, offs,
                      max_msgs, st, flags);
}

int phip_table_digest(phip_handle* h, uint32_t log2_parts, phip_digest_part* out,
                      phip_digest_stats* st, uint32_t flags) {
  if (!h) return PHIP_ERR_INVALID;
  std::lock_guard<std::mutex> g(h->mu);
  if (int rc0 = begin_call(h)) return rc0;
  if (flags & ~PHIP_DEVICE_PTRS)
    return set_err(h, PHIP_ERR_INVALID, "digest: unknown flag bits 0x%x", flags);
  if (!out || log2_parts > PHIP_DIGEST_MAX_LOG2_PARTS)
    return set_err(h, PHIP_ERR_INVALID, "digest: out and log2_parts <= %d are required",
                   PHIP_DIGEST_MAX_LOG2_PARTS);
  const bool dev = flags & PHIP_DEVICE_PTRS;
  if (dev && (reinterpret_cast<uintptr_t>(out) & 7))
    return set_err(h, PHIP_ERR_INVALID, "digest: a device buffer is 8-byte aligned");
  const u32 k = log2_parts;
  const size_t nparts = (size_t)1 << k;
  const bool lds = k <= kDigestLdsLog2;
  const unsigned grid =
      std::min<unsigned>(grid_for(h->cap, 2 * kDigestBlock), 2u * (unsigned)h->ncu);
  int rc;
  u64* stats;
  if ((rc = ensure(h, B_DIGEST, kDgWords + (size_t)grid * kDgWords + (lds ? 2 * grid * nparts : 0),
                   &stats)))
    return rc;
  u64* pstat = stats + kDgWords;
  u64* partial = pstat + (size_t)grid * kDgWords;
  phip_digest_part* res = out;
  if (!dev && (rc = ensure(h, B_DIGOUT, nparts, &res))) return rc;
  if (!lds) HIPCHK(h, hipMemsetAsync(res, 0, nparts * sizeof(phip_digest_part), h->stream));
  {
    Launch l(h, "k_digest");
    if (lds)
      k_digest<true><<<grid, kDigestBlock, 0, h->stream>>>(h->recs, h->cap, k, partial, nullptr,
                                                           pstat);
    else
      k_digest<false><<<grid, kDigestBlock, 0, h->stream>>>(h->recs, h->cap, k, nullptr, res,
                                                            pstat);
  }
  {
    Launch l(h, "k_digest_reduce");
    const unsigned rgrid = lds ? (unsigned)((nparts + 63) / 64) + 1 : 1;
    k_digest_reduce<<<rgrid, kDigestBlock, 0, h->stream>>>(partial, grid, k, res, pstat, stats);
  }
  HIPCHK(h, hipGetLastError());
  u64 sw[kDgWords] = {};
  HIPCHK(h, hipMemcpyAsync(sw, stats, sizeof sw, hipMemcpyDeviceToHost, h->stream));
  if (!dev)
    HIPCHK(h, hipMemcpyAsync(out, res, nparts * sizeof(phip_digest_part), hipMemcpyDeviceToHost,
                             h->stream));
  HIPCHK(h, hipStreamSynchronize(h->stream));
  if (st) {
    st->records = sw[kDgRecords];
    st->bytes = sw[kDgBytes];
    st->slots_scanned = h->cap;
  }
  return PHIP_OK;
}

int phip_table_stats(phip_handle* h, uint64_t* out, int max) {
  if (!h || !out) return PHIP_ERR_INVALID;
  std::lock_guard<std::mutex> g(h->mu);
  if (int rc0 = begin_call(h)) return rc0;
  u64* d;
  int rc;
  if ((rc = ensure(h, B_TSTATS, 2, &d))) return rc;
  HIPCHK(h, hipMemsetAsync(d, 0, 2 * sizeof(u64), h->stream));
  {
    Launch l(h, "k_table_stats");
    k_table_stats<<<grid_for(h->cap), kBlock, 0, h->stream>>>(table(h), h->cap, d);
  }
  HIPCHK(h, hipGetLastError());
  u64 r[2] = {0, 0};
  HIPCHK(h, hipMemcpyAsync(r, d, sizeof r, hipMemcpyDeviceToHost, h->stream));
  HIPCHK(h, hipStreamSynchronize(h->stream));
  const uint64_t v[4] = {h->n_buckets, h->cap, r[0], r[1]};
  return copy_words(v, out, max);
}

int phip_last_stats(phip_handle* h, uint64_t* out, int max) {
  if (!h || !out) return 0;
  std::lock_guard<std::mutex> g(h->mu);
  if (h->pend.active && !h->deferred_rc) h->deferred_rc = begin_call(h);
  const phip_handle::LastStats& s = h->stats;
  const uint64_t v[7] = {s.hot_entries, s.hot_hits,  s.misses,  h->grows,
                         s.ordered,     s.log_count, s.log_over};
  return copy_words(v, out, max);
}

int phip_undo_log_layout(uint32_t n, uint32_t compute_units, uint64_t* out, int max) {
  if (!out || !compute_units) return 0;
  const UndoLayout l = undo_layout(n, compute_units);
  const uint64_t v[4] = {l.grid, l.waves, l.cap, l.halves * sizeof(u64x2)};
  return copy_words(v, out, max);
}

}

namespace phip_host {
void* handle_stream(phip_handle* h) { return h ? (void*)h->stream : nullptr; }
int finish_queued(phip_handle* h) {
  HIPCHK(h, hipSetDevice(h->device));
  if (!h->pend.active) return PHIP_OK;
  const int rc = finish_pending(h);
  return rc ? after_error(h, rc) : PHIP_OK;
}
int route_dir(phip_handle* h, void* stream, const phip_msgs* m, uint32_t world, const void** dir) {
  std::lock_guard<std::mutex> g(h->mu);
  if (int rc0 = finish_queued(h)) return rc0;
  return route_dir_on(h, (hipStream_t)stream, *m, world, dir);
}
int route_pack(phip_handle* h, void* stream, const phip_msgs* m, uint32_t world, const void* dir,
               uint8_t* names, uint32_t* lens, uint64_t* a, uint64_t* t, int64_t* e,
               uint64_t* counts, uint64_t* nbytes) {
  std::lock_guard<std::mutex> g(h->mu);
  if (int rc0 = finish_queued(h)) return rc0;
  return route_pack_on(h, (hipStream_t)stream, *m, world, dir, names, lens, a, t, e, counts, nbytes);
}
int route_pack_ops(phip_handle* h, void* stream, const phip_ops* ops, uint32_t world,
                   uint8_t* names, uint32_t* lens, uint8_t* kind, int64_t* now, uint64_t* x0,
                   uint64_t* x1, uint64_t* x2, uint32_t* src, uint64_t* counts, uint64_t* nbytes) {
  std::lock_guard<std::mutex> g(h->mu);
  if (int rc0 = finish_queued(h)) return rc0;
  return route_pack_ops_on(h, (hipStream_t)stream, *ops, world, names, lens, kind, now, x0, x1, x2,
                           src, counts, nbytes);
}
int results_scatter(phip_handle* h, void* stream, const uint32_t* src, uint32_t n,
                    const uint8_t* status, const uint64_t* remaining, const uint64_t* have,
                    const phip_state* reply, const phip_results* out) {
  if (!n || !out) return PHIP_OK;
  const OutView ow{out->status, out->remaining, out->have, out->reply};
  if (!ow.status && !ow.remaining && !ow.have && !ow.reply) return PHIP_OK;
  k_route_results_scatter<<<grid_for(n), kBlock, 0, (hipStream_t)stream>>>(src, n, status, remaining,
                                                                           have, reply, ow);
  HIPCHK(h, hipGetLastError());
  return PHIP_OK;
}
int check_offsets(phip_handle* h, void* stream, const uint8_t* names, const uint32_t* name_offs,
                  uint32_t names_len, uint32_t n, uint32_t* first_bad) {
  std::lock_guard<std::mutex> g(h->mu);
  if (int rc0 = finish_queued(h)) return rc0;
  return check_offsets_on(h, (hipStream_t)stream, names, name_offs, names_len, n, first_bad);
}
const char* last_error(phip_handle* h) { return h ? h->err.c_str() : ""; }
int handle_device(const phip_handle* h) { return h ? h->device : -1; }
}
```

### patrol_amd/csrc/phip_kernels.hpp

```cpp
#pragma once
#include <type_traits>

#include "phip_device.hpp"

namespace phip {

constexpr int kBlock = 256;

template <bool NT, class T>
__device__ inline T ld(const T* p) {
  if constexpr (NT) return __builtin_nontemporal_load(p);
  else return *p;
}

__device__ inline u64 load_be64(const u8* p) {
  u64 v = 0;
#pragma unroll
  for (int k = 0; k < 8; ++k) v = (v << 8) | p[k];
  return v;
}

struct NamesOffs {
  const u8* blob;
  const u32* offs;
// ... 18 lines not shown
  template <bool NT = false>
  __device__ inline bool get(u32 i, u64& o, u32& l) const {
    o = ld<NT>(off + i);
    l = ld<NT>(len + i);
    return false;
  }
};

struct Datagrams {
  const u8* blob;
  const uint64_t* offs;
  template <bool NT = false>
  __device__ inline bool get(u32 i, u64& o, u32& l) const {
    const u64 a = ld<NT>(offs + i), b = ld<NT>(offs + i + 1);
    o = a + 25;
    const u64 room = b > o ? b - o : 0;
    const u32 want = b >= a + 25 ? blob[a + 24] : 0;
    l = want < room ? want : (u32)room;
    return false;
  }
};

__device__ inline u64 ld_co(const u64* p) {
  return __hip_atomic_load(p, __ATOMIC_RELAXED, __HIP_MEMORY_SCOPE_AGENT);
}
template <bool Co = false>
__device__ inline u64 str_word(const u64* p, u32 sh, u32 k, u32 lastw) {
  const u64* a = p + (k < lastw ? k : lastw);
  const u64* b = p + (k + 1 < lastw ? k + 1 : lastw);
  const u64 lo = Co ? ld_co(a) : *a, hi = Co ? ld_co(b) : *b;
  return sh ? (lo >> sh) | (hi << (64 - sh)) : lo;
}
__device__ inline u64 low_bytes(u64 w, u32 n) { return n >= 8 ? w : (w & ((1ull << (8 * n)) - 1)); }

__device__ inline void fnv_step32(u32& lo, u32& hi, u32 c) {
  lo ^= c;
  const u64 p = (u64)lo * 0x1b3u;
  hi = (u32)((u64)hi * 0x1b3u + (p >> 32)) + (lo << 8);
  lo = (u32)p;
}
__device__ inline void fnv_word32(u32& lo, u32& hi, u64 w, u32 n) {
#pragma unroll
  for (u32 b = 0; b < 8; ++b)
    if (b < n) fnv_step32(lo, hi, (u32)(w >> (8 * b)) & 0xFFu);
}

__device__ inline void load_name_long(const u8* src, u64 off, u32 len, Name& nm) {
  const u64* p = reinterpret_cast<const u64*>(src + (off & ~7ull));
  const u32 sh = (u32)(off & 7) * 8;
  const u32 lastw = ((u32)(off & 7) + len - 1) >> 3;
  u32 lo = (u32)kFnvOffset, hi = (u32)(kFnvOffset >> 32);
  const u64 w1 = str_word(p, sh, 0, lastw), w2 = str_word(p, sh, 1, lastw);
  fnv_word32(lo, hi, w1, 8);
  fnv_word32(lo, hi, w2, 8);
  for (u32 k = 16; k < len; k += 8) {
    const u32 n = len - k < 8 ? len - k : 8;
    fnv_word32(lo, hi, str_word(p, sh, k >> 3, lastw), n);
  }
  nm.h = ((u64)hi << 32) | lo; nm.len = len; nm.off = off;
  nm.w0 = len; nm.w1 = w1; nm.w2 = w2;
}

template <bool Co = false>
__device__ inline bool long_tail_equal(const u8* arena, u64 aoff, const u8* src, u64 off, u32 len) {
  const u64 a0 = aoff + 16, s0 = off + 16;
  const u32 n = len - 16;
  const u64* pa = reinterpret_cast<const u64*>(arena + (a0 & ~7ull));
  const u64* ps = reinterpret_cast<const u64*>(src + (s0 & ~7ull));
  const u32 sha = (u32)(a0 & 7) * 8, shs = (u32)(s0 & 7) * 8;
  const u32 la = ((u32)(a0 & 7) + n - 1) >> 3, ls = ((u32)(s0 & 7) + n - 1) >> 3;
  for (u32 k = 0; k < n; k += 8) {
    const u32 m = n - k < 8 ? n - k : 8;
    if (low_bytes(str_word<Co>(pa, sha, k >> 3, la), m) != low_bytes(str_word(ps, shs, k >> 3, ls), m))
      return false;
  }
  return true;
}

template <bool NT>
__device__ inline void load_name_wide(const u8* src, u64 off, u32 len, Name& nm) {
  if (len > kInlineName) { load_name_long(src, off, len, nm); return; }
  const u32 sh = (u32)(off & 7) * 8;
  const u32 nw = ((u32)(off & 7) + len + 7) >> 3;
  const u64* p = reinterpret_cast<const u64*>(src + (off & ~7ull));
  const u64 w0 = nw > 0 ? ld<NT>(p) : 0, w1 = nw > 1 ? ld<NT>(p + 1) : 0;
  const u64 w2 = nw > 2 ? ld<NT>(p + 2) : 0, w3 = nw > 3 ? ld<NT>(p + 3) : 0;
  u64 b0 = sh ? (w0 >> sh) | (w1 << (64 - sh)) : w0;
  u64 b1 = sh ? (w1 >> sh) | (w2 << (64 - sh)) : w1;
  u64 b2 = sh ? (w2 >> sh) | (w3 << (64 - sh)) : w2;
  if (len < 8) { b0 = len ? b0 & ((1ull << (8 * len)) - 1) : 0; b1 = 0; b2 = 0; }
  else if (len < 16) { b1 = len > 8 ? b1 & ((1ull << (8 * (len - 8))) - 1) : 0; b2 = 0; }
  else if (len < 24) { b2 = len > 16 ? b2 & ((1ull << (8 * (len - 16))) - 1) : 0; }
  u32 lo = (u32)kFnvOffset, hi = (u32)(kFnvOffset >> 32);
  fnv_word32(lo, hi, b0, len);
  if (len > 8) fnv_word32(lo, hi, b1, len - 8);
  if (len > 16) fnv_word32(lo, hi, b2, len - 16);
  nm.h = ((u64)hi << 32) | lo; nm.len = len; nm.off = off;
  nm.w0 = (u64)len | (b0 << 16);
  nm.w1 = (b0 >> 48) | (b1 << 16);
  nm.w2 = (b1 >> 48) | (b2 << 16);
}

__device__ inline u32 wave_append(u32* counter, bool pred) {
  u64 mask = __ballot(pred);
  if (!pred) return 0;
  u32 lane = __lane_id();
  u32 leader = __ffsll((long long)mask) - 1;
  u32 rank = __popcll(mask & ((1ull << lane) - 1));
  u32 base = 0;
  if (lane == leader) base = atomicAdd(counter, (u32)__popcll(mask));
  base = __shfl(base, leader);
  return base + rank;
}

constexpr u32 kShards = 256;
__host__ __device__ inline u32 shard_cap(u32 units, u32 per_unit) {
  return per_unit * ((units + kShards - 1) / kShards);
}
struct Sharded {
  u32* base = nullptr;
  u32* cnt = nullptr;
  u32 cap = 0;
  __device__ inline void append(u32 unit, bool pred, u32 v) const {
    const u32 sh = unit & (kShards - 1);
    const u32 pos = wave_append(&cnt[sh], pred);
    if (pred) base[(size_t)sh * cap + pos] = v;
  }
};


constexpr u32 kCtrNDirty = 0;
constexpr u32 kCtrBadName = 1;
constexpr u32 kCtrMiss = 2;
constexpr u32 kCtrOccupied = kCtrMiss;
constexpr u32 kCtrClaimed = 3;
constexpr u32 kCtrRetry = 4;
constexpr u32 kCtrStop = 5;
constexpr u32 kCtrLongSegs = 6;
constexpr u32 kCtrHugeSegs = 9;
constexpr u32 kCtrLogOver = kCtrLongSegs;
constexpr u32 kCtrLogCount = kCtrHugeSegs;
constexpr u32 kCtrArenaFull = 7;
constexpr u32 kCtrTableFull = 8;
constexpr u32 kCtrHotHits = 10;
constexpr u32 kCtrHotEntries = 11;
constexpr u32 kCtrDirty = 12;
constexpr u32 kCtrShardMax = 13;
constexpr u32 kCtrAux = 14;
constexpr u32 kCtrSegs = 15;
constexpr u32 kCtrResetWords = 16;
constexpr u32 kCtrLongBytes = 16;
constexpr u32 kCtrNDefer = 18;
constexpr u32 kCtrNSorted = 19;
constexpr u32 kCtrWords = 32;
__host__ __device__ constexpr u32 ctr_reset_value(u32 w) {
  return (w == kCtrStop || w == kCtrDirty) ? ~0u : 0u;
}
static_assert(kCtrNDirty < kCtrResetWords && kCtrBadName < kCtrResetWords &&
                  kCtrOccupied < kCtrResetWords && kCtrStop < kCtrResetWords &&
                  kCtrLogOver < kCtrResetWords && kCtrLogCount < kCtrResetWords &&
                  kCtrArenaFull < kCtrResetWords && kCtrTableFull < kCtrResetWords &&
                  kCtrHotHits < kCtrResetWords && kCtrDirty < kCtrResetWords,
              "the words kernels accumulate into from the batch's reset value");
static_assert(kCtrTableFull == kCtrArenaFull + 1, "evict_idle clears both flags in one memset");
static_assert(kCtrLongBytes % 2 == 0 && kCtrLongBytes >= kCtrResetWords &&
              kCtrLongBytes + 2 <= kCtrWords, "an aligned u64 outside the reset");
static_assert(kCtrNDefer >= kCtrResetWords && kCtrNDefer < kCtrWords &&
              kCtrNSorted >= kCtrResetWords && kCtrNSorted < kCtrWords, "outside the reset");
static_assert(kCtrResetWords <= kShards && kCtrWords <= kShards,
              "k_batch_reset and shard_scan's host mirror: one lane per word");

__global__ __launch_bounds__(kShards) void k_batch_reset(u32* ctr, u32* shard_cnt) {
  const u32 t = threadIdx.x;
  if (t < kCtrResetWords) ctr[t] = ctr_reset_value(t);
  if (shard_cnt) shard_cnt[t] = 0;
}

__device__ inline void shard_scan(u32* cnt, u32* ctr, u32 tot, u32* host, u32 words, u32* next,
                                  u32* next_ctr);
__global__ __launch_bounds__(kShards) void k_shard_scan(u32* cnt, u32* ctr, u32 tot, u32* host,
                                                        u32 words, u32* next, u32* next_ctr) {
  shard_scan(cnt, ctr, tot, host, words, next, next_ctr);
}
__device__ inline void shard_scan(u32* cnt, u32* ctr, u32 tot, u32* host, u32 words, u32* next,
                                  u32* next_ctr) {
  __shared__ u32 v[kShards];
  __shared__ u32 wmax[kShards / 64];
  const u32 t = threadIdx.x, c = cnt[t];
  v[t] = c;
  u32 m = c;
  for (u32 d = 32; d; d >>= 1) m = max(m, (u32)__shfl_xor((int)m, d));
  if ((t & 63) == 0) wmax[t >> 6] = m;
  __syncthreads();
  for (u32 off = 1; off < kShards; off <<= 1) {
    const u32 x = t >= off ? v[t - off] : 0u;
    __syncthreads();
    v[t] += x;
    __syncthreads();
  }
  cnt[kShards + t] = v[t] - c;
  const u32 total = v[kShards - 1];
  u32 mx = 0;
  for (u32 w = 0; w < kShards / 64; ++w) mx = max(mx, wmax[w]);
  if (t == 0) {
    ctr[tot] = total;
    ctr[kCtrShardMax] = mx;
  }
  if (host && t < words) {
    const u32 w = t == tot ? total : t == kCtrShardMax ? mx : ctr[t];
    __hip_atomic_store(&host[t], w, __ATOMIC_RELAXED, __HIP_MEMORY_SCOPE_SYSTEM);
  }
  if (next) {
    if (t < kCtrResetWords) next_ctr[t] = ctr_reset_value(t);
    next[t] = 0;
  }
}

__global__ __launch_bounds__(256) void k_shard_compact(const u32* __restrict__ base, u32 cap,
                                                       const u32* __restrict__ cnt,
                                                       u32* __restrict__ out) {
  const u32 s = blockIdx.y, j = blockIdx.x * 256 + threadIdx.x;
  if (j < cnt[s]) out[cnt[kShards + s] + j] = base[(size_t)s * cap + j];
}

template <bool Co = false>
__device__ inline bool name_equal(const Rec& r, const Name& nm, const u8* src, const u8* arena) {
  const u64 r0 = r.name0 & ~0xFF00ull;
  if ((r0 & 0xFFu) != (nm.w0 & 0xFFu)) return false;
  if (nm.len <= kInlineName) return r0 == nm.w0 && r.name1 == nm.w1 && r.name2 == nm.w2;
  if (r.name1 != nm.w1 || r.name2 != nm.w2) return false;
  return long_tail_equal<Co>(arena, r.name0 >> 32, src, nm.off, nm.len);
}

enum ProbeResult : int { kFound = 0, kMiss = 1, kPending = 2, kFull = 3 };

__host__ __device__ inline u64 seeded_mix(u64 tag, u64 seed) {
  u64 x = tag ^ seed;
  x ^= x >> 33;
  x *= 0xff51afd7ed558ccdull;
  x ^= x >> 33;
  x *= 0xc4ceb9fe1a85ec53ull;
  x ^= x >> 33;
  return x;
}

struct Table {
  Rec* recs;
  u32* aux;
  const u8* arena;
  u32 L;
  u64 tag_mask;
  u64 seed;
  __device__ inline u64 tag(u64 h) const { return tag_of(h & tag_mask); }
  __device__ inline u32 home(u64 tag) const { return (u32)(seeded_mix(tag, seed) >> (64 - L)); }
  __device__ inline u32 mask() const { return (u32)((1ull << L) - 1); }
};

__device__ inline Rec load_rec(const Rec* p) {
  const uint4* q = reinterpret_cast<const uint4*>(p);
  uint4 a = q[0], b = q[1], c = q[2], d = q[3];
  Rec r;
  r.tag = ((u64)a.y << 32) | a.x;
  r.added = ((u64)a.w << 32) | a.z;
  r.taken = ((u64)b.y << 32) | b.x;
  r.elapsed = (i64)(((u64)b.w << 32) | b.z);
  r.name0 = ((u64)c.y << 32) | c.x;
  r.name1 = ((u64)c.w << 32) | c.z;
  r.created = (i64)(((u64)d.y << 32) | d.x);
  r.name2 = ((u64)d.w << 32) | d.z;
  return r;
}

#ifndef PHIP_REC48_X2
#define PHIP_REC48_X2 1
#endif
__device__ inline Rec load_rec48(const Rec* p) {
#if PHIP_REC48_X2
  const u64* w = reinterpret_cast<const u64*>(p);
  const u64 w0 = w[0], w1 = w[1], w2 = w[2], w3 = w[3], w4 = w[4], w5 = w[5];
  const uint4 a{(u32)w0, (u32)(w0 >> 32), (u32)w1, (u32)(w1 >> 32)};
  const uint4 b{(u32)w2, (u32)(w2 >> 32), (u32)w3, (u32)(w3 >> 32)};
  const uint4 c{(u32)w4, (u32)(w4 >> 32), (u32)w5, (u32)(w5 >> 32)};
#else
  const uint4* q = reinterpret_cast<const uint4*>(p);
  uint4 a = q[0], b = q[1], c = q[2];
#endif
  Rec r;
  r.tag = ((u64)a.y << 32) | a.x;
  r.added = ((u64)a.w << 32) | a.z;
  r.taken = ((u64)b.y << 32) | b.x;
  r.elapsed = (i64)(((u64)b.w << 32) | b.z);
  r.name0 = ((u64)c.y << 32) | c.x;
  r.name1 = ((u64)c.w << 32) | c.z;
  r.created = 0;
  r.name2 = 0;
  return r;
}

__device__ inline int probe(const Table& T, const Name& nm, const u8* src, u32* slot, Rec* rec) {
  const u64 tag = T.tag(nm.h);
  const u32 mask = T.mask();
  u32 s = T.home(tag);
  const bool shortname = nm.len <= kShortName;
  for (u32 k = 0; k <= mask; ++k) {
    Rec r = shortname ? load_rec48(&T.recs[s]) : load_rec(&T.recs[s]);
    if (r.tag == 0) return kMiss;
    if (r.tag == tag) {
      if (!(rec_flags(r) & kRecPublished)) return kPending;
      if (name_equal(r, nm, src, T.arena)) { *slot = s; *rec = r; return kFound; }
    }
    s = (s + 1) & mask;
  }
  return kFull;
}


__device__ inline void note_min(bool d, u32 i, u32* word) {
  const u64 m = __ballot(d);
  if (m && __lane_id() == (u32)(__ffsll((long long)m) - 1)) atomicMin(word, i);
}
__device__ inline void note_dirty(bool d, u32 i, u32* ctr) { note_min(d, i, &ctr[kCtrDirty]); }

constexpr u32 kDirtyCap = 4096;
constexpr u32 kDirtySlots = 2 * kDirtyCap;
constexpr u32 kSubBatchCap = 5 * kDirtyCap;
constexpr u32 kSubBatchOver = ~0u;
constexpr u64 kRecDirty = 4u;
__device__ inline void note_dirty_list(bool d, u32 i, u32* ctr, u32* dlist) {
  const u32 pos = wave_append(&ctr[kCtrNDirty], d);
  if (d && pos < kDirtyCap) dlist[pos] = i;
}
struct DirtySet {
  u64* key;
  u64* w;
  u32* ready;
  u32* first;
  u32* start;
  u32* cnt;
  u32* rslot;
  u32* idx;
// ... 33 lines not shown
  if (x == 0) return 0x7FF8000000000000ull;
  if (x == kInfBits) return 0;
  if (x > kInfBits) return x - kInfBits - 1;
  return kSign | (kInfBits - x);
}

__device__ inline bool replica_dirty(u64 ab, u64 tb, i64 e) {
  const bool inc = is_zero_bits(ab) && is_zero_bits(tb) && e == 0;
  return inc || ab == kSign || tb == kSign;
}

constexpr u32 kCombEmpty = 0xFFFFFFFFu;
constexpr u32 kCombSlots = 256;
constexpr u32 kCombBits = 8;
static_assert((1u << kCombBits) == kCombSlots, "combining table size");

template <bool NT>
__device__ inline void load_words3(const u8* blob, u64 off, u32 len, u64& w0, u64& w1, u64& w2) {
  const u64* p = reinterpret_cast<const u64*>(blob);
  const u64 wb = off >> 3;
  const u64 we = (off + (len ? len : 1u) - 1) >> 3;
  w0 = ld<NT>(p + wb);
  w1 = ld<NT>(p + (wb + 1 < we ? wb + 1 : we));
  w2 = ld<NT>(p + (wb + 2 < we ? wb + 2 : we));
}

__device__ inline void short_name(u64 w0, u64 w1, u64 w2, u64 off, u32 len, Name& nm) {
  const u32 sh = (u32)(off & 7) * 8;
  u64 b0 = (w0 >> sh) | ((w1 << 1) << (63 - sh));
  u64 b1 = (w1 >> sh) | ((w2 << 1) << (63 - sh));
  b0 = len >= 8 ? b0 : (b0 & ((1ull << (8 * len)) - 1));
  b1 = len > 8 ? (b1 & ((1ull << (8 * (len - 8))) - 1)) : 0;
  u32 lo = (u32)kFnvOffset, hi = (u32)(kFnvOffset >> 32);
  const u32 q[4] = {(u32)b0, (u32)(b0 >> 32), (u32)b1, (u32)(b1 >> 32)};
  if (__builtin_amdgcn_ballot_w64(len > 8) == 0) {
#pragma unroll
    for (u32 k = 0; k < 8; ++k)
      if (k < len) fnv_step32(lo, hi, (q[k >> 2] >> (8 * (k & 3))) & 0xFFu);
  } else
  {
#pragma unroll
    for (u32 k = 0; k < kShortName; ++k)
      if (k < len) fnv_step32(lo, hi, (q[k >> 2] >> (8 * (k & 3))) & 0xFFu);
  }
  nm.h = ((u64)hi << 32) | lo; nm.len = len; nm.off = off;
  nm.w0 = (u64)len | (b0 << 16);
  nm.w1 = (b0 >> 48) | (b1 << 16);
  nm.w2 = 0;
}

__device__ inline void inline_name(u64 w0, u64 w1, u64 w2, u64 w3, u64 off, u32 len, Name& nm) {
  const u32 sh = (u32)(off & 7) * 8;
  const u64 b0 = sh ? (w0 >> sh) | (w1 << (64 - sh)) : w0;
  u64 b1 = sh ? (w1 >> sh) | (w2 << (64 - sh)) : w1;
  u64 b2 = sh ? (w2 >> sh) | (w3 << (64 - sh)) : w2;
  b1 = low_bytes(b1, len - 8);
  b2 = len > 16 ? low_bytes(b2, len - 16) : 0;
  u32 lo = (u32)kFnvOffset, hi = (u32)(kFnvOffset >> 32);
  fnv_word32(lo, hi, b0, 8);
  fnv_word32(lo, hi, b1, len - 8);
  if (len > 16) fnv_word32(lo, hi, b2, len - 16);
  nm.h = ((u64)hi << 32) | lo; nm.len = len; nm.off = off;
  nm.w0 = (u64)len | (b0 << 16);
  nm.w1 = (b0 >> 48) | (b1 << 16);
  nm.w2 = (b1 >> 48) | (b2 << 16);
}

__device__ inline u64 enc_replica_nz(u64 b) {
  const u64 mag = b & ~kSign;
  const u64 e = (b >> 63) ? kInfBits - mag : kInfBits + mag + (mag != 0);
  return mag > kInfBits ? 0ull : e;
}

#ifndef PHIP_HOT_MAX
#define PHIP_HOT_MAX 736
#endif
#ifndef PHIP_HOT_LDS
#define PHIP_HOT_LDS 4096
#endif
constexpr u32 kHotMax = PHIP_HOT_MAX;
constexpr u32 kHotLds = PHIP_HOT_LDS;
constexpr u32 kRouteHotMax = 512;
static_assert(kHotLds * 2 >= kRouteHotMax * 3 && kHotLds * 2 >= kHotMax * 3, "LDS lookup load");
constexpr u32 kHotCntBits = 18;
constexpr u32 kHotSampleMax = 1u << 17;
constexpr u32 kHotSamplePerBlock = 1024;
#ifndef PHIP_HOT_ALONE
#define PHIP_HOT_ALONE 256
#endif
constexpr u32 kHotAloneThreads = PHIP_HOT_ALONE;
constexpr u32 kHotHist = 4096;
constexpr u32 kHotMinCount = 8;
constexpr u32 kHotCandMax = kHotSampleMax / kHotMinCount;
constexpr u32 kHotSyncWords = 16;
constexpr size_t kHotZeroBytes = (2 * (size_t(1) << kHotCntBits) + kHotSyncWords) * sizeof(u32);
constexpr u32 kHotMinBatch = 1u << 16;
constexpr u32 kRouteMinBatch = 1u << 20;
#ifndef PHIP_MANY_MISSES
#define PHIP_MANY_MISSES (1u << 16)
#endif
constexpr u32 kManyMisses = PHIP_MANY_MISSES;

constexpr u32 kHotTailName = 40;
constexpr u32 kHotTailWords = (kHotTailName - 16) / 8;
struct HotEntry {
  u64 tag, w0, w1, w2;
  u64 tail[kHotTailWords];
  u32 slot, aoff;
};
struct HotHdr {
  u32 n;
  u32 thresh;
  u32 pad[14];
};

__device__ inline u32 hot_home(u64 tag) { return (u32)(tag ^ (tag >> 29)) & (kHotLds - 1); }

__device__ inline HotEntry hot_entry(const Table& T, u32 s) {
  const Rec r = load_rec(&T.recs[s]);
  HotEntry d;
  const bool arena = (r.name0 & 0xFFu) > kInlineName;
  d.tag = r.tag;
  d.w0 = arena ? (r.name0 & 0xFFu) : (r.name0 & ~0xFF00ull);
  d.w1 = r.name1;
  d.w2 = r.name2;
  d.slot = s;
  d.aoff = arena ? (u32)(r.name0 >> 32) : 0u;
  const u32 len = (u32)(r.name0 & 0xFFu);
  for (u32 k = 0; k < kHotTailWords; ++k) d.tail[k] = 0;
  if (arena && len <= kHotTailName) {
    const u64 a0 = (r.name0 >> 32) + 16;
    const u64* p = reinterpret_cast<const u64*>(T.arena + (a0 & ~7ull));
    const u32 sh = (u32)(a0 & 7) * 8, lastw = ((u32)(a0 & 7) + len - 17) >> 3;
    for (u32 k = 0; 8 * k < len - 16; ++k) {
      const u32 m = len - 16 - 8 * k;
      d.tail[k] = low_bytes(str_word(p, sh, k, lastw), m);
    }
  }
  return d;
}

__device__ inline u32 ld_co32(const u32* p) {
  return __hip_atomic_load(p, __ATOMIC_RELAXED, __HIP_MEMORY_SCOPE_AGENT);
}
__device__ inline void st_co32(u32* p, u32 v) {
  __hip_atomic_store(p, v, __ATOMIC_RELAXED, __HIP_MEMORY_SCOPE_AGENT);
}

template <class Src, u32 kThreads, u32 kRounds>
__global__ __launch_bounds__(kThreads) void k_hot_dir(Src src, u32 n, u32 stride, u32 nsample,
                                                      Table T, u32* ckeys, u32* ccnt, u32* sync,
                                                      u32* cand, HotHdr* hdr,
                                                      HotEntry* __restrict__ dir, u32 nblk,
                                                      u8* __restrict__ status) {
  constexpr u32 kPerBlock = kThreads * kRounds;
  constexpr u32 kL = 2 * kPerBlock;
  static_assert(kHotHist % kThreads == 0 && 4096 % kThreads == 0, "the last workgroup's shares");
  constexpr u32 kWords = 2 * kL > kHotHist ? 2 * kL : kHotHist;
  __shared__ u32 lds[kWords];
  __shared__ u32 part[kThreads];
  __shared__ u32 sel[kHotMax];
  __shared__ u32 best, nsel, last;
  if (blockIdx.x >= nblk) {
    constexpr u32 b4 = PHIP_ST_MERGED * 0x01010101u;
    const u64 head = min((u64)n, (u64)(-(uintptr_t)status & 15));
    const u64 n16 = (n - head) / 16;
    uint4* body = reinterpret_cast<uint4*>(status + head);
    const u64 step = (u64)(gridDim.x - nblk) * kThreads;
    for (u64 k = (u64)(blockIdx.x - nblk) * kThreads + threadIdx.x; k < n16; k += step)
      body[k] = uint4{b4, b4, b4, b4};
    if (blockIdx.x == nblk) {
      if (threadIdx.x < head) status[threadIdx.x] = PHIP_ST_MERGED;
      const u64 done = head + n16 * 16;
      if (done + threadIdx.x < n) status[done + threadIdx.x] = PHIP_ST_MERGED;
    }
    return;
  }
  u32* lkey = lds;
  u32* lcnt = lds + kL;
  for (u32 e = threadIdx.x; e < 2 * kL; e += kThreads) lds[e] = 0;
  __syncthreads();
  for (u32 r = 0; r < kRounds; ++r) {
    const u32 j = blockIdx.x * kPerBlock + r * kThreads + threadIdx.x;
    const u64 i = (u64)j * stride;
    if (j >= nsample || i >= n) continue;
    u64 off; u32 len;
    src.template get<true>((u32)i, off, len);
    Name nm;
    load_name_wide<true>(src.blob, off, len, nm);
    u32 s;
    Rec rec;
    if (probe(T, nm, src.blob, &s, &rec) != kFound) continue;
    u32 h = (s * 2654435761u) & (kL - 1);
    for (;;) {
      const u32 old = atomicCAS(&lkey[h], 0u, s + 1);
      if (old == 0 || old == s + 1) { atomicAdd(&lcnt[h], 1u); break; }
      h = (h + 1) & (kL - 1);
    }
  }
  __syncthreads();
  constexpr u32 mask = (1u << kHotCntBits) - 1;
  constexpr u32 kE = kL / kThreads;
  u32 key[kE], cnt[kE], hh[kE], before[kE];
#pragma unroll
  for (u32 k = 0; k < kE; ++k) {
    key[k] = lkey[k * kThreads + threadIdx.x];
    cnt[k] = lcnt[k * kThreads + threadIdx.x];
    hh[k] = ((key[k] - 1) * 2654435761u) >> (32 - kHotCntBits);
    before[k] = ~0u;
  }
  for (u32 tries = 0; tries <= mask; ++tries) {
    u32 old[kE];
#pragma unroll
    for (u32 k = 0; k < kE; ++k)
      if (key[k] && before[k] == ~0u) old[k] = atomicCAS(&ckeys[hh[k]], 0u, key[k]);
    bool again = false;
#pragma unroll
    for (u32 k = 0; k < kE; ++k) {
      if (!key[k] || before[k] != ~0u) continue;
      if (old[k] == 0 || old[k] == key[k]) before[k] = atomicAdd(&ccnt[hh[k]], cnt[k]);
      else { hh[k] = (hh[k] + 1) & mask; again = true; }
    }
    if (!again) break;
  }
  u32 ncross = 0;
#pragma unroll
  for (u32 k = 0; k < kE; ++k) {
    const bool cross = key[k] && before[k] < kHotMinCount && before[k] + cnt[k] >= kHotMinCount;
    if (!cross) key[k] = 0;
    ncross += cross;
  }
  if (ncross) {
    u32 at = atomicAdd(&sync[1], ncross);
#pragma unroll
    for (u32 k = 0; k < kE; ++k)
      if (key[k] && at < kHotCandMax) st_co32(&cand[at++], hh[k]);
  }
  asm volatile("s_waitcnt vmcnt(0)" ::: "memory");
  __syncthreads();
  if (threadIdx.x == 0) {
    const u32 t = __hip_atomic_fetch_add(&sync[0], 1u, __ATOMIC_RELAXED, __HIP_MEMORY_SCOPE_AGENT);
    last = t == nblk - 1;
    if (last) {
      __builtin_amdgcn_fence(__ATOMIC_ACQUIRE, "agent");
      asm volatile("s_waitcnt vmcnt(0)" ::: "memory");
    }
  }
  __syncthreads();
  if (!last) return;

  constexpr u32 kU = 4096 / kThreads;
  static_assert(4096 <= kHotCandMax, "the list entries read before its length");
  u32 hh0[kU];
#pragma unroll
  for (u32 k = 0; k < kU; ++k) hh0[k] = ld_co32(&cand[k * kThreads + threadIdx.x]);
  const u32 ncand = min(ld_co32(&sync[1]), kHotCandMax);
#pragma unroll
  for (u32 k = 0; k < kU; ++k) hh0[k] = k * kThreads + threadIdx.x < ncand ? hh0[k] & mask : ~0u;
  u32* hist = lds;
  for (u32 e = threadIdx.x; e < kHotHist; e += kThreads) hist[e] = 0;
  if (threadIdx.x == 0) { best = kHotHist; nsel = 0; }
  __syncthreads();
  auto counts = [&](const u32 (&hh)[kU], u32 (&cc)[kU], u32 (&kk)[kU]) {
#pragma unroll
    for (u32 k = 0; k < kU; ++k) {
      cc[k] = hh[k] != ~0u ? ld_co32(&ccnt[hh[k]]) : 0u;
      kk[k] = hh[k] != ~0u ? ld_co32(&ckeys[hh[k]]) : 0u;
    }
  };
  auto load = [&](u32 base, u32 (&cc)[kU], u32 (&kk)[kU]) {
    u32 hh[kU];
#pragma unroll
    for (u32 k = 0; k < kU; ++k) {
      const u32 c = base + k * kThreads + threadIdx.x;
      hh[k] = c < ncand ? ld_co32(&cand[c]) & mask : ~0u;
    }
    counts(hh, cc, kk);
  };
  auto count = [&](const u32 (&cc)[kU]) {
#pragma unroll
    for (u32 k = 0; k < kU; ++k)
      if (cc[k] >= kHotMinCount) atomicAdd(&hist[cc[k] < kHotHist ? cc[k] : kHotHist - 1], 1u);
  };
  u32 cc0[kU], kk0[kU];
  counts(hh0, cc0, kk0);
  count(cc0);
  for (u32 base = kThreads * kU; base < ncand; base += kThreads * kU) {
    u32 cc[kU], kk[kU];
    load(base, cc, kk);
    count(cc);
  }
  __syncthreads();
  {
    constexpr u32 kBins = kHotHist / kThreads;
    const u32 t = threadIdx.x;
    u32 s = 0;
    for (u32 k = 0; k < kBins; ++k) s += hist[t * kBins + k];
    part[t] = s;
    __syncthreads();
    u32 run = 0;
    for (u32 u = t + 1; u < kThreads; ++u) run += part[u];
    u32 lo = kHotHist;
    for (int b = (int)kBins - 1; b >= 0; --b) {
      run += hist[t * kBins + b];
      if (run <= kHotMax) lo = t * kBins + b;
    }
    atomicMin(&best, lo);
    __syncthreads();
  }
  const u32 thresh = best > kHotMinCount ? best : kHotMinCount;
  auto pick = [&](const u32 (&cc)[kU], const u32 (&kk)[kU]) {
#pragma unroll
    for (u32 k = 0; k < kU; ++k) {
      if (cc[k] < thresh) continue;
      const u32 idx = atomicAdd(&nsel, 1u);
      if (idx < kHotMax) sel[idx] = kk[k] - 1;
    }
  };
  pick(cc0, kk0);
  for (u32 base = kThreads * kU; base < ncand; base += kThreads * kU) {
    u32 cc[kU], kk[kU];
    load(base, cc, kk);
    pick(cc, kk);
  }
  __syncthreads();
  const u32 ns = min(nsel, kHotMax);
#pragma unroll
  for (u32 k = 0; k < (kHotMax + kThreads - 1) / kThreads; ++k) {
    const u32 j = k * kThreads + threadIdx.x;
    if (j < ns) dir[j] = hot_entry(T, sel[j]);
  }
  if (threadIdx.x == 0) {
    hdr->n = nsel;
    hdr->thresh = thresh;
    st_co32(&sync[0], 0u);
    st_co32(&sync[1], 0u);
  }
}

__global__ void k_hot_hist(const u32* __restrict__ ccnt, u32* __restrict__ hist) {
  const u32 e = blockIdx.x * blockDim.x + threadIdx.x;
  if (e >= (1u << kHotCntBits)) return;
  const u32 c = ccnt[e];
  if (c >= kHotMinCount) atomicAdd(&hist[c < kHotHist ? c : kHotHist - 1], 1u);
}

__global__ __launch_bounds__(256) void k_hot_select(const u32* __restrict__ hist, HotHdr* hdr,
                                                    u32 maxn) {
  constexpr u32 kPer = kHotHist / 256;
  __shared__ u32 part[256];
  __shared__ u32 best;
  const u32 t = threadIdx.x;
  u32 s = 0;
  for (u32 k = 0; k < kPer; ++k) s += hist[t * kPer + k];
  part[t] = s;
  if (t == 0) best = kHotHist;
  __syncthreads();
  u32 run = 0;
  for (u32 u = t + 1; u < 256; ++u) run += part[u];
  u32 lo = kHotHist;
  for (int b = (int)kPer - 1; b >= 0; --b) {
    run += hist[t * kPer + b];
    if (run <= maxn) lo = t * kPer + b;
  }
  atomicMin(&best, lo);
  __syncthreads();
  if (t == 0) {
    hdr->n = 0;
    hdr->thresh = best > kHotMinCount ? best : kHotMinCount;
  }
}

#ifndef PHIP_FAST_BLOCK
#define PHIP_FAST_BLOCK 1024
#endif
#ifndef PHIP_FAST_PER_CU
#define PHIP_FAST_PER_CU 2
#endif
constexpr u32 kFastBlock = PHIP_FAST_BLOCK;
constexpr u32 kFastPerCU = PHIP_FAST_PER_CU;

template <class Src>
struct SoaIn {
  Src src;
  const uint64_t* ma;
  const uint64_t* mt;
  const int64_t* me;
  static constexpr bool kSoa = true;
  __device__ inline const u8* blob() const { return src.blob; }
  struct PreOffs { u32 a, b; };
  struct PreGen { u64 off; u32 len; };
  static constexpr bool kOffs = std::is_same<Src, NamesOffs>::value;
  using Pre = typename std::conditional<kOffs, PreOffs, PreGen>::type;
  __device__ inline Pre pre(u32 i) const {
    Pre p;
    if constexpr (kOffs) {
      p.a = ld<true>(src.offs + i);
      p.b = ld<true>(src.offs + i + 1);
    } else {
      src.template get<true>(i, p.off, p.len);
    }
    return p;
  }
  __device__ inline void load(u32 i, const Pre& p, u64& off, u32& len, u64& w0, u64& w1, u64& w2,
                              u64& ra, u64& rt, i64& re) const {
    if constexpr (kOffs) { off = p.a; len = p.b - p.a; }
    else { off = p.off; len = p.len; }
    ra = ld<true>(ma + i); rt = ld<true>(mt + i); re = ld<true>(me + i);
    load_words3<false>(src.blob, off, len, w0, w1, w2);
  }
  __device__ inline bool dirty(u32 i, u32* ctr) const {
    if constexpr (kOffs) {
      if (src.lim && src.bad(src.offs[i], src.offs[i + 1])) {
        atomicMin(&ctr[kCtrStop], i);
        return false;
      }
    }
    const u64 ab = __builtin_nontemporal_load(ma + i), tb = __builtin_nontemporal_load(mt + i);
    if (is_zero_bits(ab) && is_zero_bits(tb)) return me[i] == 0 || ab == kSign || tb == kSign;
    return ab == kSign || tb == kSign;
  }
};

__device__ inline u64 funnel8(u64 lo, u64 hi, u32 sb) {
  return sb ? (lo >> (8 * sb)) | (hi << (64 - 8 * sb)) : lo;
}
struct WireIn {
  const u8* bytes;
  const uint64_t* offs;
  static constexpr bool kSoa = false;
  __device__ inline const u8* blob() const { return bytes; }
  struct Pre { u64 o; u32 sz; };
  __device__ inline Pre pre(u32 i) const {
    const u64 o = ld<true>(offs + i), end = ld<true>(offs + i + 1);
    return Pre{o, (u32)min(end - o, (u64)0xFFFFFFFFu)};
  }
  __device__ inline void load(u32 i, const Pre& pr, u64& off, u32& len, u64& w0, u64& w1, u64& w2,
                              u64& ra, u64& rt, i64& re) const {
    const u64 o = pr.o, end = pr.o + pr.sz;
    const u64* p = reinterpret_cast<const u64*>(bytes);
    const u64 last = (end > o ? end - 1 : o) >> 3;
    const u64 hb = o >> 3;
    u64 h[4];
#pragma unroll
    for (u32 k = 0; k < 4; ++k) h[k] = ld<false>(p + (hb + k < last ? hb + k : last));
    off = o + 25;
    const u64 nb = off >> 3;
    const u64 nb0 = nb < last ? nb : last, nb1 = nb + 1 < last ? nb + 1 : last;
    const u64 nb2 = nb + 2 < last ? nb + 2 : last;
    w0 = ld<false>(p + nb0); w1 = ld<false>(p + nb1); w2 = ld<false>(p + nb2);
    const u32 sb = (u32)(o & 7);
    ra = __builtin_bswap64(funnel8(h[0], h[1], sb));
    rt = __builtin_bswap64(funnel8(h[1], h[2], sb));
    re = (i64)__builtin_bswap64(funnel8(h[2], h[3], sb));
    len = (u32)(h[3] >> (8 * sb)) & 0xFFu;
  }
  __device__ inline bool dirty(u32 i, u32* ctr) const {
    const u64 o = offs[i], end = offs[i + 1], sz = end - o;
    const u64* p = reinterpret_cast<const u64*>(bytes);
    const u64 last = (end > o ? end - 1 : o) >> 3, hb = o >> 3;
    u64 h[4];
#pragma unroll
    for (u32 k = 0; k < 4; ++k) h[k] = p[hb + k < last ? hb + k : last];
    const u32 sb = (u32)(o & 7);
    const u32 len = (u32)(h[3] >> (8 * sb)) & 0xFFu;
    if (sz < PHIP_BUCKET_FIXED_SIZE || sz - PHIP_BUCKET_FIXED_SIZE < len) {
      atomicMin(&ctr[kCtrStop], i);
      return false;
    }
    return replica_dirty(__builtin_bswap64(funnel8(h[0], h[1], sb)),
                         __builtin_bswap64(funnel8(h[1], h[2], sb)),
                         (i64)__builtin_bswap64(funnel8(h[2], h[3], sb)));
  }
};

template <class In>
__global__ __launch_bounds__(kBlock) void k_classify(In in, u32 n, u32* ctr, u32* dlist) {
  const u32 i = blockIdx.x * kBlock + threadIdx.x;
  const bool d = i < n && in.dirty(i, ctr);
  note_dirty(d, i, ctr);
  if (dlist && __ballot(d)) note_dirty_list(d, i, ctr, dlist);
}

template <class In>
__global__ __launch_bounds__(1024) void k_dirty_build(In in, u32 n, u32* ctr, const u32* dlist,
// ... 43 lines not shown
          continue;
        if (D.w[2 * s] == nm.w0 && D.w[2 * s + 1] == nm.w1) break;
      }
      s = (s + 1) & (kDirtySlots - 1);
    }
    atomicMin(&D.first[s], i);
    sk[j] = ((u64)s << 32) | i;
    ++valid;
  }
  if (valid) atomicAdd(&nvalid, valid);
  __syncthreads();
  if (longname) {
    if (tid == 0) ctr[kCtrNDirty] = ~0u;
    return;
  }
  u32 P = 1;
  while (P < nd) P <<= 1;
  for (u32 j = nd + tid; j < P; j += 1024) sk[j] = ~0ull;
  __syncthreads();
  for (u32 k = 2; k <= P; k <<= 1) {
    for (u32 j = k >> 1; j > 0; j >>= 1) {
      for (u32 t = tid; t < P; t += 1024) {
        const u32 u = t ^ j;
        if (u > t) {
          const u64 x = sk[t], y = sk[u];
          if ((x > y) == ((t & k) == 0)) { sk[t] = y; sk[u] = x; }
        }
      }
      __syncthreads();
    }
  }
  const u32 nv = nvalid;
  for (u32 j = tid; j < nv; j += 1024) {
    const u32 s = (u32)(sk[j] >> 32);
    D.idx[j] = (u32)sk[j];
    D.dslot[j] = s;
    D.cell[3 * j] = 0; D.cell[3 * j + 1] = 0; D.cell[3 * j + 2] = 0;
    u64* pc = D.cell + 3 * ((size_t)kDirtyCap + j);
    pc[0] = 0; pc[1] = 0; pc[2] = 0;
    D.premin[j] = ~0u;
    if (j == 0 || (u32)(sk[j - 1] >> 32) != s) D.start[s] = j;
  }
  __syncthreads();
  for (u32 j = tid; j < nv; j += 1024) {
    const u32 s = (u32)(sk[j] >> 32);
    if (j + 1 == nv || (u32)(sk[j + 1] >> 32) != s) D.cnt[s] = j + 1 - D.start[s];
    if (j == 0 || (u32)(sk[j - 1] >> 32) != s) {
      const u32 i = (u32)sk[j];
      u64 off, w0, w1, w2, ra, rt;
      u32 len;
      i64 re;
      const typename In::Pre p = in.pre(i);
      in.load(i, p, off, len, w0, w1, w2, ra, rt, re);
      Name nm;
      short_name(w0, w1, w2, off, len, nm);
      u32 slot;
      Rec cur;
      if (probe(T, nm, in.blob(), &slot, &cur) == kFound) {
        D.rslot[s] = slot;
        atomicOr(reinterpret_cast<unsigned long long*>(&T.recs[slot].name0),
                 (unsigned long long)(kRecDirty << 8));
      } else {
        D.rslot[s] = ~0u;
      }
    }
  }
  if (tid == 0) {
    ctr[kCtrNSorted] = nv;
    if (nv == 0) ctr[kCtrNDirty] = 0;
  }
}

typedef unsigned long long u64x2 __attribute__((ext_vector_type(2)));
__global__ __launch_bounds__(kBlock) void k_classify_soa2(const uint64_t* __restrict__ ma,
                                                          const uint64_t* __restrict__ mt,
                                                          const int64_t* __restrict__ me, u32 n,
                                                          u32* ctr, u8* status, NamesOffs names,
                                                          u32* dlist) {
  const u32 i0 = 2 * (blockIdx.x * kBlock + threadIdx.x);
  if (names.lim) {
    bool b0 = false, b1 = false;
    if (i0 < n) {
      const u32 o0 = names.offs[i0], o1 = names.offs[i0 + 1];
      const u32 o2 = i0 + 1 < n ? names.offs[i0 + 2] : o1;
      b0 = names.bad(o0, o1);
      b1 = i0 + 1 < n && names.bad(o1, o2);
    }
    note_min(b0 || b1, b0 ? i0 : i0 + 1, &ctr[kCtrStop]);
  }
  if (status) {
    if (i0 + 1 < n && ((uintptr_t)status & 1) == 0)
      *reinterpret_cast<u16*>(status + i0) = (u16)(PHIP_ST_MERGED | (PHIP_ST_MERGED << 8));
    else {
      if (i0 < n) status[i0] = PHIP_ST_MERGED;
      if (i0 + 1 < n) status[i0 + 1] = PHIP_ST_MERGED;
    }
  }
  bool d = false, e0 = false, e1 = false;
  u32 at = i0;
  if (i0 + 1 < n) {
    const u64x2 a = __builtin_nontemporal_load(reinterpret_cast<const u64x2*>(ma + i0));
    const u64x2 t = __builtin_nontemporal_load(reinterpret_cast<const u64x2*>(mt + i0));
    const bool z0 = is_zero_bits(a.x) && is_zero_bits(t.x);
    const bool z1 = is_zero_bits(a.y) && is_zero_bits(t.y);
    const bool d0 = (z0 && me[i0] == 0) || a.x == kSign || t.x == kSign;
    const bool d1 = (z1 && me[i0 + 1] == 0) || a.y == kSign || t.y == kSign;
    d = d0 || d1;
    at = d0 ? i0 : i0 + 1;
    e0 = d0;
    e1 = d1;
  } else if (i0 < n) {
    const u64 a = ma[i0], t = mt[i0];
    d = (is_zero_bits(a) && is_zero_bits(t) && me[i0] == 0) || a == kSign || t == kSign;
    e0 = d;
  }
  note_dirty(d, at, ctr);
  if (dlist && __ballot(d)) {
    note_dirty_list(e0, i0, ctr, dlist);
    note_dirty_list(e1, i0 + 1, ctr, dlist);
  }
}

__device__ inline void load_name_tail(const u8* src, u64 off, u32 len, Name& nm, u64 (&tail)[kHotTailWords]) {
  const u64* p = reinterpret_cast<const u64*>(src + (off & ~7ull));
  const u32 sh = (u32)(off & 7) * 8;
  const u32 lastw = ((u32)(off & 7) + len - 1) >> 3;
  u32 lo = (u32)kFnvOffset, hi = (u32)(kFnvOffset >> 32);
  const u64 w1 = str_word(p, sh, 0, lastw), w2 = str_word(p, sh, 1, lastw);
  fnv_word32(lo, hi, w1, 8);
  fnv_word32(lo, hi, w2, 8);
#pragma unroll
  for (u32 k = 0; k < kHotTailWords; ++k) {
    const u32 m = len > 16 + 8 * k ? len - 16 - 8 * k : 0;
    const u64 w = m ? low_bytes(str_word(p, sh, k + 2, lastw), m) : 0;
    fnv_word32(lo, hi, w, m);
    tail[k] = w;
  }
  nm.h = ((u64)hi << 32) | lo; nm.len = len; nm.off = off;
  nm.w0 = len; nm.w1 = w1; nm.w2 = w2;
}
__device__ inline bool tail_match(const u64 (&htail)[kHotTailWords][kHotMax], u32 j,
                                  const u64 (&tail)[kHotTailWords]) {
  bool eq = true;
#pragma unroll
  for (u32 k = 0; k < kHotTailWords; ++k) eq &= htail[k][j] == tail[k];
  return eq;
}

constexpr u8 kMarkDirty = 0x40;

#ifndef PHIP_UNDO_NT
#define PHIP_UNDO_NT 1
#endif
constexpr u32 kUndoFlushReserve = 64 * ((kHotMax + kFastBlock - 1) / kFastBlock);
struct UndoLog {
  u64x2* base = nullptr;
  u32* cnt = nullptr;
  u32 cap = 0;
};
__host__ __device__ inline u32 fast_wave_chunks(u32 n, u32 grid) {
  const u32 nchunks = (n + 63) / 64, kw = kFastBlock / 64;
  if (grid % 8 == 0) {
    const u32 per = (nchunks + 7) / 8, waves = grid / 8 * kw;
    return (per + waves - 1) / waves;
  }
  return (nchunks + grid * kw - 1) / (grid * kw);
}
constexpr u32 kUndoSlack = 24;
__host__ __device__ inline u32 undo_wave_cap(u32 n, u32 grid) {
  return fast_wave_chunks(n, grid) * 32 + kUndoSlack + kUndoFlushReserve;
}
__device__ inline u32 lane_rank(u64 m) {
  return __builtin_amdgcn_mbcnt_hi((u32)(m >> 32), __builtin_amdgcn_mbcnt_lo((u32)m, 0u));
}
__device__ inline void undo_store(u64x2* p, u32 slot, u64 a, u64 t, i64 e) {
#if PHIP_UNDO_NT
  __builtin_nontemporal_store(u64x2{(u64)slot, a}, p);
  __builtin_nontemporal_store(u64x2{t, (u64)e}, p + 1);
#else
  p[0] = u64x2{(u64)slot, a};
  p[1] = u64x2{t, (u64)e};
#endif
}

template <class In, bool Opt = false>
__global__ __launch_bounds__(kFastBlock) __attribute__((amdgpu_waves_per_eu(8, 8))) void k_receive_fast(
    In in, u32 lo, u32 n, Table T, Sharded miss, u32* ctr,
    const HotHdr* __restrict__ hot, const HotEntry* __restrict__ hot_dir, const u64* dtab,
    u8* __restrict__ mark, UndoLog ulog, uint4* __restrict__ hot_zero) {
  __shared__ u32 hslot[kHotLds];
  __shared__ u64 htag[kHotMax], hw0[kHotMax], hw1[kHotMax], hw2[kHotMax];
  __shared__ u32 hrec[kHotMax], haoff[kHotMax];
  __shared__ u64 htail[kHotTailWords][kHotMax];
  __shared__ u64 hmax[3][kHotMax];
  __shared__ u32 hhits;
  __shared__ u32 hlog[2];

  if (hot_zero)
    for (u32 k = blockIdx.x * kFastBlock + threadIdx.x; k < kHotZeroBytes / sizeof(uint4);
         k += gridDim.x * kFastBlock)
      hot_zero[k] = uint4{0, 0, 0, 0};
  const u32 ndr = !Opt && dtab ? ctr[kCtrNDirty] : 0u;
  const bool iso = !Opt && ndr != 0 && ndr <= kDirtyCap;
  if constexpr (!Opt) n = min(n, iso ? ctr[kCtrStop] : min(ctr[kCtrStop], ctr[kCtrDirty]));
  if (n <= lo) return;
  const u32 nh = hot ? min(hot->n, kHotMax) : 0u;
  for (u32 j = threadIdx.x; j < kHotLds; j += kFastBlock) hslot[j] = 0;
  for (u32 j = threadIdx.x; j < kHotMax; j += kFastBlock) {
    hmax[0][j] = 0; hmax[1][j] = 0; hmax[2][j] = 0;
  }
  if (threadIdx.x == 0) hhits = 0;
  if (Opt && threadIdx.x < 2) hlog[threadIdx.x] = 0;
  __syncthreads();
  for (u32 j = threadIdx.x; j < nh; j += kFastBlock) {
    const HotEntry d = hot_dir[j];
    htag[j] = d.tag; hw0[j] = d.w0; hw1[j] = d.w1; hw2[j] = d.w2;
    hrec[j] = d.slot | (iso && (rec_flags(T.recs[d.slot]) & kRecDirty) ? 0x80000000u : 0u);
    haoff[j] = d.aoff;
    for (u32 k = 0; k < kHotTailWords; ++k) htail[k][j] = d.tail[k];
    u32 hs = hot_home(d.tag);
    while (atomicCAS(&hslot[hs], 0u, j + 1) != 0) hs = (hs + 1) & (kHotLds - 1);
  }
  __syncthreads();

  constexpr u32 kWaves = kFastBlock / 64;
  const u32 lane = threadIdx.x & 63;
  u32 nchunks = (n + 63) / 64;
  u32 hits = 0;
  const u32 wave = __builtin_amdgcn_readfirstlane(threadIdx.x / 64);
  u32 cstride, chunk;
  if (gridDim.x % 8 == 0) {
    const u32 per = (nchunks - lo / 64 + 7) / 8;
    const u32 c0 = lo / 64 + (blockIdx.x % 8) * per;
    nchunks = min(nchunks, c0 + per);
    cstride = gridDim.x / 8 * kWaves;
    chunk = c0 + blockIdx.x / 8 * kWaves + wave;
  } else {
    cstride = gridDim.x * kWaves;
    chunk = lo / 64 + blockIdx.x * kWaves + wave;
  }
  u64x2* lbase = nullptr;
  u32 lcur = 0, lover = 0;
  const u32 lcap = Opt ? ulog.cap - kUndoFlushReserve : 0u;
  if constexpr (Opt) lbase = ulog.base + (size_t)(blockIdx.x * kWaves + wave) * ulog.cap * 2;
  typename In::Pre pre{};
  if (chunk < nchunks) pre = in.pre(min(chunk * 64 + lane, n - 1));
  for (; chunk < nchunks; chunk += cstride) {
    const u32 tid = chunk * 64 + lane;
    bool valid = tid < n;
    const u32 i = tid < n ? tid : n - 1;
    if constexpr (Opt && In::kSoa) {
      if constexpr (In::kOffs) {
        if (in.src.lim) {
          const bool bad = in.src.bad(pre.a, pre.b);
          note_min(valid && bad, i, &ctr[kCtrStop]);
          if (bad) { pre.a = 0; pre.b = 0; valid = false; }
        }
      }
    }
    u64 off, w0, w1, w2, ra, rt;
    u32 len;
    i64 re;
    in.load(i, pre, off, len, w0, w1, w2, ra, rt, re);
    if constexpr (Opt) {
      const bool d = valid && replica_dirty(ra, rt, re);
      const u64 dm = __ballot(d);
      if (dm) {
        if (__lane_id() == (u32)(__ffsll((long long)dm) - 1)) {
          atomicMin(&ctr[kCtrDirty], i);
          atomicAdd(&ctr[kCtrNDirty], (u32)__popcll(dm));
        }
        valid = valid && !d;
      }
    }
    if (chunk + cstride < nchunks) pre = in.pre(min((chunk + cstride) * 64 + lane, n - 1));
    Name nm;
    short_name(w0, w1, w2, off, len, nm);
    const bool shortname = len <= kShortName;
    u64 tail[kHotTailWords] = {};
    if (!shortname) {
      if (len <= kInlineName) {
        const u64* bw = reinterpret_cast<const u64*>(in.blob());
        const u64 last = (off + len - 1) >> 3, w3i = (off >> 3) + 3;
        inline_name(w0, w1, w2, bw[w3i < last ? w3i : last], off, len, nm);
      } else if (In::kSoa && len <= kHotTailName) {
        load_name_tail(in.blob(), off, len, nm, tail);
      } else {
        load_name_wide<true>(in.blob(), off, len, nm);
      }
    }
    const u64 tag = T.tag(nm.h);
    const u64 ea = enc_replica_nz(ra), et = enc_replica_nz(rt), ee = (u64)re ^ kSign;

    bool missed = false;
    bool grows = false;
    u32 gs = 0;
    u64 ga = 0, gt = 0;
    i64 ge = 0;
    if (valid) {
      int hidx = -1;
      if (nh) {
        for (u32 hs = hot_home(tag);; hs = (hs + 1) & (kHotLds - 1)) {
          const u32 e = hslot[hs];
          if (!e) break;
          if (htag[e - 1] == tag && hw0[e - 1] == nm.w0 && hw1[e - 1] == nm.w1 &&
              (shortname || (hw2[e - 1] == nm.w2 &&
                             (len <= kInlineName ||
                              (In::kSoa && len <= kHotTailName
                                   ? tail_match(htail, e - 1, tail)
                                   : long_tail_equal(T.arena, haoff[e - 1], in.blob(), off, len)))))) {
            hidx = (int)e - 1;
            break;
          }
        }
      }
      if (hidx >= 0) {
        if (iso && (hrec[hidx] >> 31)) {
          mark[i] = kMarkDirty;
        } else {
          ++hits;
          if (ea > hmax[0][hidx]) atomicMax(&hmax[0][hidx], ea);
          if (et > hmax[1][hidx]) atomicMax(&hmax[1][hidx], et);
          if (ee > hmax[2][hidx]) atomicMax(&hmax[2][hidx], ee);
        }
      } else {
        u32 s = T.home(tag);
        Rec cur = load_rec48(&T.recs[s]);
        const bool hit = shortname && cur.tag == tag && (cur.name0 & ~0xFF00ull) == nm.w0 &&
                         cur.name1 == nm.w1 && (rec_flags(cur) & kRecPublished);
        int pr = kFound;
        if (!hit) {
          if (shortname && cur.tag == 0) {
            pr = kMiss;
          } else {
            pr = probe(T, nm, in.blob(), &s, &cur);
          }
        }
        if (pr == kFound) {
          if (iso && (rec_flags(cur) & kRecDirty)) {
            mark[i] = kMarkDirty;
          } else if constexpr (Opt) {
            grows = ea > cur.added || et > cur.taken || ee > ((u64)cur.elapsed ^ kSign);
            gs = s; ga = cur.added; gt = cur.taken; ge = cur.elapsed;
          } else {
            Rec* r = &T.recs[s];
            if (ea > cur.added) atomicMax(&r->added, ea);
            if (et > cur.taken) atomicMax(&r->taken, et);
            if (ee > ((u64)cur.elapsed ^ kSign)) atomicMax(&r->elapsed, (i64)(ee ^ kSign));
          }
        } else if (iso && shortname) {
          mark[i] = kMarkDirty;
        } else {
          missed = true;
          if (pr == kFull) atomicOr(&ctr[kCtrTableFull], 1u);
        }
      }
    }
    if constexpr (Opt) {
      const u64 gm = __ballot(grows);
      if (gm) {
        if (grows) {
          const u32 pos = lcur + lane_rank(gm);
          if (pos < lcap) {
            undo_store(lbase + 2 * (size_t)pos, gs, ga, gt, ge);
            Rec* r = &T.recs[gs];
            if (ea > ga) atomicMax(&r->added, ea);
            if (et > gt) atomicMax(&r->taken, et);
            if (ee > ((u64)ge ^ kSign)) atomicMax(&r->elapsed, (i64)(ee ^ kSign));
          }
        }
        const u32 want = lcur + (u32)__popcll(gm);
        lover += want > lcap ? want - lcap : 0u;
        lcur = min(want, lcap);
      }
    }
    miss.append(chunk, missed, i);
  }
  if (hits) atomicAdd(&hhits, hits);
  __syncthreads();
  if (threadIdx.x == 0) {
    if (hhits) atomicAdd(&ctr[kCtrHotHits], hhits);
    if (blockIdx.x == 0) ctr[kCtrHotEntries] = nh;
  }

  if constexpr (Opt) {
    for (u32 jb = wave * 64; jb < nh; jb += kFastBlock) {
      const u32 j = jb + lane;
      bool lg = false;
      u64 xa = 0, xt = 0, xe = 0, ca = 0, ct = 0, ce = 0;
      Rec* r = nullptr;
      if (j < nh) {
        xa = hmax[0][j]; xt = hmax[1][j]; xe = hmax[2][j];
        if (xa | xt | xe) {
          r = &T.recs[hrec[j] & 0x7FFFFFFFu];
          ca = r->added; ct = r->taken; ce = (u64)r->elapsed ^ kSign;
          lg = xa > ca || xt > ct || xe > ce;
        }
      }
      const u64 gm = __ballot(lg);
      if (lg) {
        undo_store(lbase + 2 * (size_t)(lcur + lane_rank(gm)), hrec[j] & 0x7FFFFFFFu, ca, ct,
                   (i64)(ce ^ kSign));
        if (xa > ca) atomicMax(&r->added, xa);
// ... 3408 lines not shown
```

### patrol_amd/engine.py

```python
from __future__ import annotations

import ctypes as C
import os
from dataclasses import dataclass
from typing import Iterable, Sequence

import numpy as np

from . import _lib
from ._lib import (DEVICE_PTRS, phip_config, phip_msgs, phip_ops, phip_results, phip_state,
                   phip_take_reply)


class PatrolHipError(RuntimeError):
    def __init__(self, code: int, msg: str):
        super().__init__(f"libpatrolhip error {code} ({_lib.PHIP_ERR.get(code, '?')}): {msg}")
        self.code = code


def _is_torch(x) -> bool:
    return type(x).__module__.startswith("torch")


def _ptr(x):
# ... 14 lines not shown
def _np(x, dtype):
    if x is None:
        return None
    a = np.ascontiguousarray(x, dtype=dtype)
    return a if a.size else np.zeros(1, dtype)


def names_blob(names: Sequence[bytes]):
    offs = np.zeros(len(names) + 1, dtype=np.uint32)
    if len(names):
        offs[1:] = np.cumsum(np.fromiter((len(x) for x in names), np.int64, len(names)))
    blob = np.zeros(int(offs[-1]) + 8, dtype=np.uint8)
    if offs[-1]:
        blob[:offs[-1]] = np.frombuffer(b"".join(names), dtype=np.uint8)
    return blob, offs


def _evict_flags(shrink: bool, dry_run: bool) -> int:
    return (_lib.EVICT_SHRINK if shrink else 0) | (_lib.EVICT_DRY_RUN if dry_run else 0)


def _evict_dict(st) -> dict:
    return {k: int(getattr(st, k)) for k, _ in _lib.phip_evict_stats._fields_}


def _part_mask(log2_parts: int, mask):
    m = np.ascontiguousarray(mask, np.uint64)
    k = int(log2_parts)
    if 0 <= k <= _lib.DIGEST_MAX_LOG2_PARTS and m.size < max(1, (1 << k) // 64):
        raise ValueError("partition mask shorter than 2^log2_parts bits")
    return m if m.size else np.zeros(1, np.uint64)


def _digest_entries(d):
    s, c = np.asarray(d[0], np.uint64), np.asarray(d[1], np.uint64)
    k = int(s.size).bit_length() - 1
    if s.size != c.size or s.size != 1 << k or k > _lib.DIGEST_MAX_LOG2_PARTS:
        raise ValueError("a digest is 2^k sums and 2^k counts, k <= 20")
    return np.ascontiguousarray(np.stack([s, c], axis=1)), k


def digest_diff(a, b):
    (ea, k), (eb, kb) = _digest_entries(a), _digest_entries(b)
    if k != kb:
        raise ValueError("digest_diff: the digests are of different levels")
    mask = np.zeros(max(1, (1 << k) // 64), np.uint64)
    nd = C.c_uint64()
    rc = _lib.load().phip_digest_diff(ea.ctypes.data, eb.ctypes.data, k, mask.ctypes.data,
                                      C.byref(nd))
    if rc:
        raise PatrolHipError(rc, "phip_digest_diff")
    return mask, int(nd.value)


def digest_fold(d, log2_out: int):
    e, k = _digest_entries(d)
    rc = _lib.load().phip_digest_fold(e.ctypes.data, k, int(log2_out), e.ctypes.data)
    if rc:
        raise PatrolHipError(rc, "phip_digest_fold: log2_out above the digest's level")
    n = 1 << int(log2_out)
    return np.ascontiguousarray(e[:n, 0]), np.ascontiguousarray(e[:n, 1])


@dataclass
class BucketState:
    added: int
    taken: int
    elapsed: int
    created: int

    @property
    def added_f(self) -> float:
        return float(np.array([self.added], np.uint64).view(np.float64)[0])

    @property
    def taken_f(self) -> float:
        return float(np.array([self.taken], np.uint64).view(np.float64)[0])


class GPURepo:

    def __init__(self, device: int = 0, log2_slots: int = 20, arena_bytes: int = 1 << 24,
                 max_load_pct: int = 90, debug_tag_bits: int = 0, grow: bool = True,
                 small: bool = True, hash_seed: int | None = None, isolate: bool = False,
                 classify_first: bool = False):
        self.L = _lib.load()
        flags = (0 if grow else _lib.CFG_NO_GROW) | (0 if small else _lib.CFG_NO_SMALL)
        if isolate:
            flags |= _lib.CFG_ISOLATE
        if classify_first:
            flags |= _lib.CFG_CLASSIFY_FIRST
        if hash_seed is not None:
            flags |= _lib.CFG_FIXED_SEED
        cfg = phip_config(device, log2_slots, arena_bytes, max_load_pct, debug_tag_bits, flags, 0,
                          (hash_seed or 0) & (2**64 - 1))
        h = C.c_void_p()
        rc = self.L.phip_open(C.byref(cfg), C.byref(h))
        if rc != 0:
            raise PatrolHipError(rc, "phip_open failed")
        self.h = h
        self.device = device
        self.owned = True

    @classmethod
    def wrap(cls, handle, device: int):
        r = cls.__new__(cls)
        r.L, r.h, r.device, r.owned = _lib.load(), C.c_void_p(handle), device, False
        return r

    def close(self):
        if getattr(self, "h", None) and getattr(self, "owned", True):
            self.L.phip_close(self.h)
        self.h = None
        self._queued = None

    def __del__(self):
        try:
            self.close()
        except Exception:
            pass

    def __len__(self):
        return int(self.L.phip_len(self.h))

    @property
    def capacity(self) -> int:
        return int(self.L.phip_capacity(self.h))

    def _check(self, rc: int, allow=()):
        if rc < 0 and rc not in allow:
            raise PatrolHipError(rc, self.L.phip_last_error(self.h).decode(errors="replace"))
        return rc

    def flush(self):
        rc = self.L.phip_flush(self.h)
        self._queued = None
        self._check(rc)

    def set_stream(self, stream=None):
        raw = getattr(stream, "cuda_stream", stream)
        self._check(self.L.phip_set_stream(self.h, C.c_void_p(raw) if raw else None))

    def use_torch_stream(self):
        import torch
        s = torch.cuda.current_stream(self.device)
        if not s.cuda_stream:
            raise ValueError("torch's current stream is the default stream; set a torch.cuda.Stream first")
        self.set_stream(s)

    def set_timing(self, on, accumulate: bool = False):
        self.L.phip_set_timing(self.h, (2 if accumulate else 1) if on else 0)

    def last_stats(self):
        out = (C.c_uint64 * 7)()
        k = self.L.phip_last_stats(self.h, out, 7)
        return tuple(int(out[i]) for i in range(k))

    def table_stats(self):
        out = (C.c_uint64 * 4)()
        k = self._check(self.L.phip_table_stats(self.h, out, 4))
        keys = ("buckets", "slots", "max_probe", "sum_probe")
        return {keys[i]: int(out[i]) for i in range(k)}

    def timings(self, max_entries: int = 1 << 14):
        names = (C.c_char_p * max_entries)()
        ms = (C.c_float * max_entries)()
        k = self.L.phip_last_timings(self.h, names, ms, max_entries)
        return [(names[i].decode(), float(ms[i])) for i in range(k)]

    def seed(self, names: Sequence[bytes], added, taken, elapsed, created):
        blob, offs = names_blob(names)
        n = len(names)
        st = np.zeros(max(n, 1), dtype=[("a", "<u8"), ("t", "<u8"), ("e", "<i8"), ("c", "<i8")])
        st["a"][:n], st["t"][:n] = np.asarray(added, np.uint64), np.asarray(taken, np.uint64)
        st["e"][:n], st["c"][:n] = np.asarray(elapsed, np.int64), np.asarray(created, np.int64)
        self._check(self.L.phip_seed(self.h, blob.ctypes.data, offs.ctypes.data, n,
                                     st.ctypes.data, 0))

    def seed_device(self, names, name_offs, states, n: int):
        self._check(self.L.phip_seed(self.h, _ptr(names), _ptr(name_offs), n, _ptr(states),
                                     DEVICE_PTRS))

    def get(self, name: bytes):
        s = phip_state()
        rc = self._check(self.L.phip_get(self.h, name, len(name), C.byref(s)))
        if rc == 0:
            return None
        return BucketState(s.added, s.taken, s.elapsed, s.created)

    def export_datagrams(self, names: Sequence[bytes]):
        n = len(names)
        blob, offs = names_blob(names)
        out = np.zeros(25 * n + int(offs[-1]) + 1, np.uint8)
        found = np.zeros(max(n, 1), np.uint8)
        self._check(self.L.phip_export_datagrams(self.h, blob.ctypes.data, offs.ctypes.data, n,
                                                 out.ctypes.data, found.ctypes.data, 0))
        raw = out.tobytes()
        dgs = [raw[25 * i + int(offs[i]):25 * (i + 1) + int(offs[i + 1])] for i in range(n)]
        return dgs, found[:n]

    def export_states_device(self, names, name_offs, n: int):
        import torch
        dev = names.device
        offs64 = name_offs.to(torch.int64)
        total = int(offs64[-1] - offs64[0])
        out = torch.zeros(_lib.BUCKET_FIXED_SIZE * max(n, 1) + total + 8, dtype=torch.uint8,
                          device=dev)
        found = torch.zeros(max(n, 1), dtype=torch.uint8, device=dev)
        self._check(self.L.phip_export_datagrams(self.h, _ptr(names), _ptr(name_offs), n,
                                                 _ptr(out), _ptr(found), DEVICE_PTRS))
        base = _lib.BUCKET_FIXED_SIZE * torch.arange(n, dtype=torch.int64, device=dev) + \
            (offs64[:-1] - offs64[0])
        words = out[base.unsqueeze(1) + torch.arange(24, device=dev).unsqueeze(0)]
        w = words.view(n, 3, 8).flip(2).contiguous().view(torch.int64).view(n, 3)
        return w[:, 0], w[:, 1], w[:, 2], found[:n].bool()

    def snapshot(self, path=None):
        nb = int(self.L.phip_snapshot_bytes(self.h))
        if nb == 0:
            raise PatrolHipError(-1, "phip_snapshot_bytes failed")
        buf = np.empty(nb, np.uint8)
        self._check(self.L.phip_snapshot(self.h, buf.ctypes.data, nb))
        if path is None:
            return buf
        buf.tofile(path)
        return None

    def restore(self, src):
        buf = np.fromfile(src, np.uint8) if isinstance(src, (str, bytes, os.PathLike)) else \
            np.ascontiguousarray(src, np.uint8)
        self._check(self.L.phip_restore(self.h, buf.ctypes.data, buf.size))

    def evict_idle(self, now: int, idle_ns: int, min_evict: int = 1, shrink: bool = False,
                   dry_run: bool = False) -> dict:
        st = _lib.phip_evict_stats()
        rc = self.L.phip_evict_idle(self.h, int(now), int(idle_ns), int(min_evict), C.byref(st),
                                    _evict_flags(shrink, dry_run))
        self._queued = None
        self._check(rc)
        return _evict_dict(st)

    @staticmethod
    def _sweep_cursor(cursor):
        return _lib.phip_sweep_cursor(*(cursor or (0, 0)))

    @staticmethod
    def _sweep_dict(st) -> dict:
        return {k: int(getattr(st, k)) for k, _ in _lib.phip_sweep_stats._fields_}

    def _sweep_call(self, parts, cur, now, idle_ns, out, out_cap, offs, max_msgs, st, flags):
        if parts is None:
            return self.L.phip_export_sweep(self.h, C.byref(cur), int(now), int(idle_ns), out,
                                            out_cap, offs, max_msgs, C.byref(st), flags)
        k, mask = int(parts[0]), _part_mask(*parts)
        return self.L.phip_export_sweep_parts(self.h, C.byref(cur), int(now), int(idle_ns), k,
                                              mask.ctypes.data, out, out_cap, offs, max_msgs,
                                              C.byref(st), flags)

    def export_sweep(self, cursor=None, max_msgs: int = 1 << 16, out_cap: int | None = None,
                     now: int = 0, idle_ns: int = 0, parts=None):
        if out_cap is None:
            out_cap = _lib.PACKET_SIZE * max_msgs
        cur, st = self._sweep_cursor(cursor), _lib.phip_sweep_stats()
        out = np.zeros(max(int(out_cap), 1), np.uint8)
        offs = np.zeros(int(max_msgs) + 1, np.uint64)
        rc = self._sweep_call(parts, cur, now, idle_ns, out.ctypes.data, int(out_cap),
                              offs.ctypes.data, int(max_msgs), st, 0)
        self._queued = None
        self._check(rc)
        raw = out[:int(st.bytes)].tobytes()
        dgs = [raw[int(offs[i]):int(offs[i + 1])] for i in range(int(st.n))]
        d = self._sweep_dict(st)
        d["offs"] = offs[:int(st.n) + 1]
        return dgs, (int(cur.slot), int(cur.layout)), d

    def export_sweep_device(self, out, offs, cursor, max_msgs: int, now: int = 0,
                            idle_ns: int = 0, parts=None):
        cur, st = self._sweep_cursor(cursor), _lib.phip_sweep_stats()
        cap = int(out.numel() * out.element_size())
        rc = self._sweep_call(parts, cur, now, idle_ns, _ptr(out), cap, _ptr(offs), int(max_msgs),
                              st, DEVICE_PTRS)
        self._queued = None
        self._check(rc)
        return int(st.n), (int(cur.slot), int(cur.layout)), self._sweep_dict(st)

    def sweep_count(self, now: int = 0, idle_ns: int = 0, parts=None) -> dict:
        cur, st = _lib.phip_sweep_cursor(), _lib.phip_sweep_stats()
        rc = self._sweep_call(parts, cur, now, idle_ns, None, 0, None, 0, st, _lib.SWEEP_COUNT)
        self._queued = None
        self._check(rc)
        return self._sweep_dict(st)

    def sweep(self, max_msgs: int = 1 << 16, out_cap: int | None = None, now: int = 0,
              idle_ns: int = 0, parts=None):
        cursor = None
        while True:
            dgs, cursor, st = self.export_sweep(cursor, max_msgs, out_cap, now, idle_ns, parts)
            yield dgs, st
            if st["done"]:
                return

    def digest(self, log2_parts: int):
        k = int(log2_parts)
        out = np.zeros((1 << min(max(k, 0), _lib.DIGEST_MAX_LOG2_PARTS), 2), np.uint64)
        st = _lib.phip_digest_stats()
        rc = self.L.phip_table_digest(self.h, k, out.ctypes.data, C.byref(st), 0)
        self._queued = None
        self._check(rc)
# ... 520 lines not shown
```

Before: 51.80 billion merges/s.

## Reuse hot directory across passes and gate-launch next optimistic pass before host sync

Keeps the hot-key directory in a double-buffered slot and reuses it for up to 32 optimistic passes while the measured overlap with the previous directory stays high. Each reused entry is revalidated against the table before it is used. The next optimistic pass is enqueued before the host reads the previous pass's counters. A device-side gate aborts that pass if the previous one left misses, dirty keys or overflow, and the host then reruns it. Status filling moves into the fast kernel, and the counter mirrors and events are doubled per parity. This removes the per-batch hot-directory rebuild and a host round-trip, at the cost of extra complexity and rerun work when the gate shuts.

```diff
diff --git a/patrol_amd/csrc/phip_engine.hip b/patrol_amd/csrc/phip_engine.hip
--- a/patrol_amd/csrc/phip_engine.hip
+++ b/patrol_amd/csrc/phip_engine.hip
@@ -72,6 +72,11 @@
   const HotEntry* dir = nullptr;
   void* hot_zero = nullptr;
   bool hot_join = false;
+  bool built = false;
+  u32 hot_age = 0;
+  const u32* gate = nullptr;
+  bool gate_shut = false;
+  u8* fill = nullptr;
   u8* mark = nullptr;
   UndoLog log{};
 };
@@ -89,7 +94,19 @@
     uint64_t hot_entries = 0, hot_hits = 0, misses = 0;
     uint64_t ordered = 0;
     uint64_t log_count = 0, log_over = 0;
+    uint64_t hot_age = 0;
+    uint64_t gate_shut = 0;
   } stats;
+  struct HotKeep {
+    void* base = nullptr;
+    u32 slot = 0;
+    bool have = false;
+    u64 gen = 0;
+    u32 served = 0;
+    bool agree = false;
+    u64 ref_hits = 0, ref_n = 0;
+    bool sagged = false;
+  } keep;
   hipStream_t stream = nullptr;
   hipStream_t own_stream = nullptr;
   hipStream_t stream2 = nullptr;
@@ -142,7 +159,7 @@
     OutView ow{};
     FastPass pass{};
   } pend;
-  hipEvent_t ev_ctr = nullptr;
+  hipEvent_t ev_ctr[2] = {nullptr, nullptr};
   int deferred_rc = 0;
 };
 
@@ -239,13 +256,14 @@
   return PHIP_OK;
 }
 
-int check_flags(phip_handle* h) {
-  if (h->ctr_host[kCtrBadName])
+int check_flags(phip_handle* h, const u32* c) {
+  if (c[kCtrBadName])
     return set_err(h, PHIP_ERR_INVALID, "malformed name offsets (names_len check): nothing applied");
-  if (h->ctr_host[kCtrTableFull]) return set_err(h, PHIP_ERR_FULL, "hash table full (probe wrapped)");
-  if (h->ctr_host[kCtrArenaFull]) return set_err(h, PHIP_ERR_ARENA, "long-name arena exhausted");
-  return PHIP_OK;
-}
+  if (c[kCtrTableFull]) return set_err(h, PHIP_ERR_FULL, "hash table full (probe wrapped)");
+  if (c[kCtrArenaFull]) return set_err(h, PHIP_ERR_ARENA, "long-name arena exhausted");
+  return PHIP_OK;
+}
+int check_flags(phip_handle* h) { return check_flags(h, h->ctr_host); }
 
 template <int N>
 int copy_words(const uint64_t (&v)[N], uint64_t* out, int max) {
@@ -254,7 +272,7 @@
   return k;
 }
 
-int finish_pending(phip_handle* h, bool* worked = nullptr);
+int finish_pending(phip_handle* h, bool* worked = nullptr, bool* shut = nullptr);
 int after_error(phip_handle* h, int rc);
 
 int begin_call(phip_handle* h, bool finish_queued = true) {
@@ -494,23 +512,29 @@
 }
 
 template <class Src>
-int build_hot(phip_handle* h, Src src, u32 n, hipStream_t st, u8* status, const HotHdr** hdr_out,
-              const HotEntry** dir_out, void** zero_out) {
-  *hdr_out = nullptr;
-  *dir_out = nullptr;
-  *zero_out = nullptr;
+int build_hot(phip_handle* h, Src src, u32 n, hipStream_t st, u8* status, FastPass* p) {
   if (n < kHotMinBatch) return PHIP_OK;
   constexpr size_t kCnt = size_t(1) << kHotCntBits;
+  constexpr size_t kSlot = sizeof(HotHdr) + kHotMax * sizeof(HotEntry);
   u8* base;
   int rc;
-  if ((rc = ensure(h, B_HOT, kHotZeroBytes + kHotCandMax * sizeof(u32) + sizeof(HotHdr) +
-                                 kHotMax * sizeof(HotEntry), &base)))
+  if ((rc = ensure(h, B_HOT, kHotZeroBytes + kHotCandMax * sizeof(u32) + 2 * kSlot, &base)))
     return rc;
   u32* ckeys = (u32*)base;
   u32* ccnt = ckeys + kCnt;
   u32* sync = ccnt + kCnt;
   u32* cand = sync + kHotSyncWords;
-  HotHdr* hdr = (HotHdr*)(cand + kHotCandMax);
+  u8* slots = (u8*)(cand + kHotCandMax);
+  phip_handle::HotKeep& kp = h->keep;
+  const bool prev = p->kind == PassKind::kOptimistic && kp.have && kp.base == base &&
+                    kp.gen == h->layout_gen;
+  const HotHdr* phdr = prev ? (const HotHdr*)(slots + kp.slot * kSlot) : nullptr;
+  kp.slot = kp.base == base ? kp.slot ^ 1u : 0u;
+  kp.base = base;
+  kp.have = true;
+  kp.gen = h->layout_gen;
+  kp.served = 1;
+  HotHdr* hdr = (HotHdr*)(slots + kp.slot * kSlot);
   HotEntry* dir = (HotEntry*)(hdr + 1);
   if (h->hot_clean != base) HIPCHK(h, hipMemsetAsync(base, 0, kHotZeroBytes, st));
   h->hot_clean = nullptr;
@@ -524,17 +548,20 @@
       const unsigned fill =
           std::min<unsigned>(grid_for(n, kT * 64), 1024 / kT * (unsigned)h->ncu);
       k_hot_dir<Src, kT, 1><<<nblk + fill, kT, 0, st>>>(
-          src, n, stride, nsample, table(h), ckeys, ccnt, sync, cand, hdr, dir, nblk, status);
+          src, n, stride, nsample, table(h), ckeys, ccnt, sync, cand, hdr, dir, nblk, status, phdr,
+          phdr ? (const HotEntry*)(phdr + 1) : nullptr, p->c);
     } else {
       const unsigned nblk = grid_for(nsample, kHotSamplePerBlock);
       k_hot_dir<Src, 256, 4><<<nblk, 256, 0, st>>>(
-          src, n, stride, nsample, table(h), ckeys, ccnt, sync, cand, hdr, dir, nblk, nullptr);
+          src, n, stride, nsample, table(h), ckeys, ccnt, sync, cand, hdr, dir, nblk, nullptr, phdr,
+          phdr ? (const HotEntry*)(phdr + 1) : nullptr, p->c);
     }
   }
   HIPCHK(h, hipGetLastError());
-  *hdr_out = hdr;
-  *dir_out = dir;
-  *zero_out = base;
+  p->hot = hdr;
+  p->dir = dir;
+  p->hot_zero = base;
+  p->built = true;
   return PHIP_OK;
 }
 
@@ -558,7 +585,7 @@
 
 int pack_sharded(phip_handle* h, const Sharded& sh, u32 total_slot, u32* out, u32* total) {
   k_shard_scan<<<1, kShards, 0, h->stream>>>(sh.cnt, h->ctr, total_slot, nullptr, 0, nullptr,
-                                             nullptr);
+                                             nullptr, nullptr);
   HIPCHK(h, hipGetLastError());
   int rc;
   if ((rc = read_ctr(h))) return rc;
@@ -646,18 +673,23 @@
   if (p->n < kHotMinBatch) return PHIP_OK;
   HIPCHK(h, hipStreamWaitEvent(h->stream2, h->ev_fork, 0));
   int rc;
-  if ((rc = build_hot(h, src, p->n, h->stream2, nullptr, &p->hot, &p->dir, &p->hot_zero))) return rc;
+  if ((rc = build_hot(h, src, p->n, h->stream2, nullptr, p))) return rc;
   HIPCHK(h, hipEventRecord(h->ev_join, h->stream2));
   p->hot_join = true;
   return PHIP_OK;
 }
 
+bool keep_take(phip_handle* h, FastPass* p);
 template <class HotSrc>
 int front_optimistic(phip_handle* h, HotSrc hsrc, u8* status, FastPass* p) {
   int rc;
   if ((rc = ensure(h, B_ULCNT, undo_counts(h), &p->log.cnt))) return rc;
+  if (keep_take(h, p)) {
+    p->fill = status;
+    return PHIP_OK;
+  }
   if (p->n >= kHotMinBatch && status)
-    return build_hot(h, hsrc, p->n, h->stream, status, &p->hot, &p->dir, &p->hot_zero);
+    return build_hot(h, hsrc, p->n, h->stream, status, p);
   if (status) HIPCHK(h, hipMemsetAsync(status, PHIP_ST_MERGED, p->n, h->stream));
   if (p->n >= kHotMinBatch) HIPCHK(h, hipEventRecord(h->ev_fork, h->stream));
   return fork_hot(h, hsrc, p);
@@ -719,7 +751,18 @@
     HIPCHK(h, hipGetLastError());
   }
   if (p->kind == PassKind::kOptimistic) return front_optimistic(h, hsrc, status, p);
+  h->keep.agree = false;
   return front_classified(h, in, hsrc, status, p);
+}
+
+inline bool holds(const phip_handle* h, BufId id, size_t bytes) {
+  return h->buf[id].cap >= std::max<size_t>(bytes, 64) + 64;
+}
+inline bool back_fits(const phip_handle* h, u32 n) {
+  return holds(h, B_MISS, (size_t)n * sizeof(u32)) &&
+         holds(h, B_MSHARD, (size_t)kShards * shard_cap((n + 63) / 64, 64) * sizeof(u32)) &&
+         holds(h, B_FSCNT, 4 * kShards * sizeof(u32)) &&
+         holds(h, B_ULOG, (size_t)undo_layout(n, (u32)h->ncu).halves * sizeof(u64x2));
 }
 
 template <class In>
@@ -746,10 +789,12 @@
         const UndoLayout ul = undo_layout(n, (u32)h->ncu);
         p.log.cap = ul.cap;
         if ((rc = ensure(h, B_ULOG, (size_t)ul.halves, &p.log.base))) return rc;
+        u8* kstatus = PHIP_STATUS_IN_KERNEL ? p.fill : nullptr;
+        if (p.fill && !kstatus) HIPCHK(h, hipMemsetAsync(p.fill, PHIP_ST_MERGED, n, h->stream));
         Launch l(h, "k_receive_fast");
         k_receive_fast<In, true><<<ul.grid, kFastBlock, 0, h->stream>>>(
             in, 0, n, table(h), msh, p.c, p.hot, p.dir, nullptr, nullptr, p.log,
-            (uint4*)p.hot_zero);
+            (uint4*)p.hot_zero, p.hot_age != 0, p.gate, kstatus);
       }
       break;
     case PassKind::kClassified:
@@ -757,7 +802,7 @@
       Launch l(h, "k_receive_fast");
       k_receive_fast<In><<<fast_grid(h, n), kFastBlock, 0, h->stream>>>(
           in, 0, n, table(h), msh, p.c, p.hot, p.dir, iso ? dset.key : nullptr, p.mark,
-          UndoLog{}, (uint4*)p.hot_zero);
+          UndoLog{}, (uint4*)p.hot_zero, 0u, nullptr, nullptr);
     }
   }
   HIPCHK(h, hipGetLastError());
@@ -772,34 +817,72 @@
     }
     k_batch_end<In><<<1, kShards, 0, h->stream>>>(
         in, p.c, dset.key, table(h),
-        SubOut{sb.off, sb.len, sb.a, sb.t, sb.e, sb.map, kSubBatchCap}, msh.cnt, h->ctr_map,
-        kCtrWords, queued ? fast_counts(h, p.par ^ 1u) : nullptr, fctr(h, p.par ^ 1u));
+        SubOut{sb.off, sb.len, sb.a, sb.t, sb.e, sb.map, kSubBatchCap}, msh.cnt,
+        h->ctr_map + kCtrWords * (1 + p.par), kCtrWords,
+        queued ? fast_counts(h, p.par ^ 1u) : nullptr, fctr(h, p.par ^ 1u));
   } else {
-    k_shard_scan<<<1, kShards, 0, h->stream>>>(msh.cnt, p.c, kCtrMiss, h->ctr_map, kCtrWords,
+    k_shard_scan<<<1, kShards, 0, h->stream>>>(msh.cnt, p.c, kCtrMiss,
+                                               h->ctr_map + kCtrWords * (1 + p.par), kCtrWords,
                                                queued ? fast_counts(h, p.par ^ 1u) : nullptr,
-                                               fctr(h, p.par ^ 1u));
+                                               fctr(h, p.par ^ 1u), p.gate);
   }
   HIPCHK(h, hipGetLastError());
-  HIPCHK(h, hipEventRecord(h->ev_ctr, h->stream));
-  if (!queued) HIPCHK(h, hipEventSynchronize(h->ev_ctr));
+  HIPCHK(h, hipEventRecord(h->ev_ctr[p.par], h->stream));
+  if (!queued) HIPCHK(h, hipEventSynchronize(h->ev_ctr[p.par]));
   return PHIP_OK;
 }
 
 constexpr u32 kIsoKeep = 256;
 constexpr u32 kOptBackoff = 256;
 
+constexpr u32 kHotKeepPasses = 32;
+bool keep_take(phip_handle* h, FastPass* p) {
+  phip_handle::HotKeep& k = h->keep;
+  if (p->n < kHotMinBatch || !k.have || !k.agree || k.sagged || k.served >= kHotKeepPasses ||
+      k.gen != h->layout_gen || k.base != h->buf[B_HOT].p)
+    return false;
+  constexpr size_t kSlot = sizeof(HotHdr) + kHotMax * sizeof(HotEntry);
+  p->hot = (const HotHdr*)((u8*)k.base + kHotZeroBytes + kHotCandMax * sizeof(u32) + k.slot * kSlot);
+  p->dir = (const HotEntry*)(p->hot + 1);
+  p->hot_age = k.served++;
+  return true;
+}
+bool keep_sagged(const phip_handle* h, const FastPass& p, const u32* c) {
+  const phip_handle::HotKeep& k = h->keep;
+  return p.hot_age != 0 && (unsigned __int128)c[kCtrHotHits] * k.ref_n * 8 <
+                               (unsigned __int128)k.ref_hits * p.n * 7;
+}
+void keep_collect(phip_handle* h, const FastPass& p, const u32* c) {
+  phip_handle::HotKeep& k = h->keep;
+  if (p.kind != PassKind::kOptimistic) {
+    k.agree = false;
+    return;
+  }
+  if (p.built) {
+    k.agree = c[kCtrHotOwn] > 0 && (u64)c[kCtrHotKept] * 8 >= (u64)c[kCtrHotOwn] * 7;
+    k.ref_hits = c[kCtrHotHits];
+    k.ref_n = p.n;
+    k.sagged = false;
+  } else if (keep_sagged(h, p, c)) {
+    k.sagged = true;
+  }
+}
+
+inline const u32* fmirror(const phip_handle* h, u32 par) { return h->ctr_host + kCtrWords * (1 + par); }
+
 bool apply_policy(phip_handle* h, const FastPass& p) {
-  const u32* c = h->ctr_host;
+  const u32* c = fmirror(h, p.par);
   if (p.kind == PassKind::kOptimistic) {
     h->stats.log_count = c[kCtrLogCount];
     h->stats.log_over = c[kCtrLogOver];
-    if (c[kCtrLogOver]) h->opt_left = kOptBackoff;
+    if (c[kCtrLogOver] && !keep_sagged(h, p, c)) h->opt_left = kOptBackoff;
     if (c[kCtrDirty] < p.n || c[kCtrStop] < p.n || c[kCtrLogOver]) return true;
   } else if (h->opt_left) {
     --h->opt_left;
   }
   if (c[kCtrDirty] < p.n) h->iso_left = kIsoKeep;
   else if (h->iso_left) --h->iso_left;
+  keep_collect(h, p, c);
   return false;
 }
 
@@ -814,27 +897,30 @@
 
 int fast_collect(phip_handle* h, const FastPass& p, FastOutcome* o) {
   int rc;
-  if ((rc = check_flags(h))) return rc;
-  o->nmiss = h->ctr_host[kCtrMiss];
+  const u32* c = fmirror(h, p.par);
+  if ((rc = check_flags(h, c))) return rc;
+  o->nmiss = c[kCtrMiss];
   if (o->nmiss) {
     Sharded msh;
     if ((rc = fast_shards(h, p.n, p.par, &msh))) return rc;
     Launch l(h, "k_shard_compact");
-    dim3 grid(grid_for(h->ctr_host[kCtrShardMax]), kShards);
+    dim3 grid(grid_for(c[kCtrShardMax]), kShards);
     k_shard_compact<<<grid, 256, 0, h->stream>>>(msh.base, msh.cap, msh.cnt,
                                                  (u32*)h->buf[B_MISS].p);
     HIPCHK(h, hipGetLastError());
   }
-  const u32 nd = h->ctr_host[kCtrNDirty];
+  const u32 nd = c[kCtrNDirty];
   o->iso_ran = p.kind == PassKind::kIsolating;
   const bool apart = o->iso_ran && nd != 0 && nd <= kDirtyCap;
-  o->first_dirty = apart ? p.n : std::min<u32>(h->ctr_host[kCtrDirty], p.n);
-  o->stop = std::min<u32>(h->ctr_host[kCtrStop], p.n);
-  o->ndef = apart ? h->ctr_host[kCtrNDefer] : 0;
+  o->first_dirty = apart ? p.n : std::min<u32>(c[kCtrDirty], p.n);
+  o->stop = std::min<u32>(c[kCtrStop], p.n);
+  o->ndef = apart ? c[kCtrNDefer] : 0;
   h->stats.ordered = 0;
-  h->stats.hot_entries = h->ctr_host[kCtrHotEntries];
-  h->stats.hot_hits = h->ctr_host[kCtrHotHits];
+  h->stats.hot_entries = c[kCtrHotEntries];
+  h->stats.hot_hits = c[kCtrHotHits];
   h->stats.misses = o->nmiss;
+  h->stats.hot_age = p.hot_age;
+  h->stats.gate_shut = p.gate_shut;
   return PHIP_OK;
 }
 
@@ -1410,12 +1496,17 @@
   return stopped_at_bad_name(h, ow, n, o.stop);
 }
 
-int finish_pending(phip_handle* h, bool* worked) {
+int finish_pending(phip_handle* h, bool* worked, bool* shut) {
   if (worked) *worked = false;
+  if (shut) *shut = false;
   if (!h->pend.active) return PHIP_OK;
   phip_handle::Pending p = h->pend;
   h->pend.active = false;
-  HIPCHK(h, hipEventSynchronize(h->ev_ctr));
+  HIPCHK(h, hipEventSynchronize(h->ev_ctr[p.pass.par]));
+  if (shut && (*shut = gate_shut(fmirror(h, p.pass.par))))
+    h->hot_clean = nullptr;
+  if (p.pass.gate && fmirror(h, p.pass.par)[kCtrGateShut])
+    return set_err(h, PHIP_ERR_INVALID, "internal: a pass ran on as gated, its kernel found the gate shut");
   int rc;
   FastOutcome o;
   if ((rc = fast_settle(h, p.in, p.in.src, p.ow.status, &p.pass, &o))) return rc;
@@ -1837,13 +1928,14 @@
   if ((e = hipEventCreateWithFlags(&h->ev_gather3, hipEventDisableTiming)) != hipSuccess)
     return fail(e);
   if ((e = hipEventCreateWithFlags(&h->ev_pack, hipEventDisableTiming)) != hipSuccess) return fail(e);
-  if ((e = hipEventCreateWithFlags(&h->ev_ctr, hipEventDisableTiming)) != hipSuccess) return fail(e);
+  for (hipEvent_t& ev : h->ev_ctr)
+    if ((e = hipEventCreateWithFlags(&ev, hipEventDisableTiming)) != hipSuccess) return fail(e);
   if ((e = hipMalloc(&h->recs, h->cap * sizeof(Rec))) != hipSuccess) return fail(e);
   if ((e = hipMalloc(&h->aux, h->cap * sizeof(u32))) != hipSuccess) return fail(e);
   if ((e = hipMalloc(&h->arena, h->arena_cap + 64)) != hipSuccess) return fail(e);
   if ((e = hipMalloc(&h->arena_cursor, 64)) != hipSuccess) return fail(e);
   if ((e = hipMalloc(&h->ctr, 3 * kCtrWords * sizeof(u32))) != hipSuccess) return fail(e);
-  if ((e = hipHostMalloc(&h->ctr_host, kCtrWords * sizeof(u32),
+  if ((e = hipHostMalloc(&h->ctr_host, 3 * kCtrWords * sizeof(u32),
                          hipHostMallocMapped | hipHostMallocCoherent)) != hipSuccess ||
       (e = hipHostGetDevicePointer((void**)&h->ctr_map, h->ctr_host, 0)) != hipSuccess)
     return fail(e);
@@ -1885,7 +1977,8 @@
   if (h->ev_gather) (void)hipEventDestroy(h->ev_gather);
   if (h->ev_gather3) (void)hipEventDestroy(h->ev_gather3);
   if (h->ev_pack) (void)hipEventDestroy(h->ev_pack);
-  if (h->ev_ctr) (void)hipEventDestroy(h->ev_ctr);
+  for (hipEvent_t ev : h->ev_ctr)
+    if (ev) (void)hipEventDestroy(ev);
   if (h->stream2) (void)hipStreamDestroy(h->stream2);
   if (h->stream3) (void)hipStreamDestroy(h->stream3);
   if (h->stream4) (void)hipStreamDestroy(h->stream4);
@@ -2181,8 +2274,34 @@
     bool worked = false;
     if ((rc = outputs(h, res, n, true, &ow))) return rc;
     const bool prev = h->pend.active;
+    const phip_handle::HotKeep keep0 = h->keep;
     if ((rc = fast_begin(h, in, src, n, ow.status, ask, !prev, &pass)))
       return after_error(h, rc);
+    if (prev && pass.kind == PassKind::kOptimistic && back_fits(h, n)) {
+      pass.gate = fctr(h, h->pend.pass.par);
+      if ((rc = fast_back(h, in, pass, true))) return after_error(h, rc);
+      bool shut = false;
+      const u64 nfast = h->nfast;
+      if ((rc = finish_pending(h, &worked, &shut))) return after_error(h, rc);
+      if (shut) {
+        if (h->nfast == nfast) {
+          phip_handle::HotKeep k = keep0;
+          k.agree = h->keep.agree;
+          k.ref_hits = h->keep.ref_hits;
+          k.ref_n = h->keep.ref_n;
+          k.sagged = h->keep.sagged;
+          h->keep = k;
+        }
+        if ((rc = fast_begin(h, in, src, n, ow.status, ask, true, &pass)))
+          return after_error(h, rc);
+        pass.gate_shut = true;
+        if ((rc = fast_back(h, in, pass, true))) return after_error(h, rc);
+      } else if (worked) {
+        return after_error(h, set_err(h, PHIP_ERR_INVALID, "internal: work left behind an open gate"));
+      }
+      h->pend = {true, in, now, ow, pass};
+      return PHIP_OK;
+    }
     const u64 nfast = h->nfast, grows = h->grows;
     if (prev && (rc = finish_pending(h, &worked))) return after_error(h, rc);
     if (worked && (h->nfast != nfast || h->grows != grows) &&
@@ -3082,8 +3201,8 @@
   std::lock_guard<std::mutex> g(h->mu);
   if (h->pend.active && !h->deferred_rc) h->deferred_rc = begin_call(h);
   const phip_handle::LastStats& s = h->stats;
-  const uint64_t v[7] = {s.hot_entries, s.hot_hits,  s.misses,  h->grows,
-                         s.ordered,     s.log_count, s.log_over};
+  const uint64_t v[9] = {s.hot_entries, s.hot_hits,  s.misses,   h->grows,  s.ordered,
+                         s.log_count,   s.log_over,  s.hot_age,  s.gate_shut};
   return copy_words(v, out, max);
 }
 
diff --git a/patrol_amd/csrc/phip_kernels.hpp b/patrol_amd/csrc/phip_kernels.hpp
--- a/patrol_amd/csrc/phip_kernels.hpp
+++ b/patrol_amd/csrc/phip_kernels.hpp
@@ -194,6 +194,9 @@
 constexpr u32 kCtrLongBytes = 16;
 constexpr u32 kCtrNDefer = 18;
 constexpr u32 kCtrNSorted = 19;
+constexpr u32 kCtrHotOwn = 20;
+constexpr u32 kCtrHotKept = 21;
+constexpr u32 kCtrGateShut = 22;
 constexpr u32 kCtrWords = 32;
 __host__ __device__ constexpr u32 ctr_reset_value(u32 w) {
   return (w == kCtrStop || w == kCtrDirty) ? ~0u : 0u;
@@ -208,7 +211,14 @@
 static_assert(kCtrLongBytes % 2 == 0 && kCtrLongBytes >= kCtrResetWords &&
               kCtrLongBytes + 2 <= kCtrWords, "an aligned u64 outside the reset");
 static_assert(kCtrNDefer >= kCtrResetWords && kCtrNDefer < kCtrWords &&
-              kCtrNSorted >= kCtrResetWords && kCtrNSorted < kCtrWords, "outside the reset");
+              kCtrNSorted >= kCtrResetWords && kCtrNSorted < kCtrWords &&
+              kCtrHotOwn >= kCtrResetWords && kCtrHotKept < kCtrWords &&
+              kCtrGateShut >= kCtrResetWords && kCtrGateShut < kCtrWords, "outside the reset");
+
+__host__ __device__ inline bool gate_shut(const u32* c) {
+  return c[kCtrDirty] != ~0u || c[kCtrStop] != ~0u || c[kCtrNDirty] != 0 || c[kCtrLogOver] != 0 ||
+         c[kCtrMiss] != 0 || c[kCtrTableFull] != 0;
+}
 static_assert(kCtrResetWords <= kShards && kCtrWords <= kShards,
               "k_batch_reset and shard_scan's host mirror: one lane per word");
 
@@ -219,15 +229,17 @@
 }
 
 __device__ inline void shard_scan(u32* cnt, u32* ctr, u32 tot, u32* host, u32 words, u32* next,
-                                  u32* next_ctr);
+                                  u32* next_ctr, const u32* gate = nullptr);
 __global__ __launch_bounds__(kShards) void k_shard_scan(u32* cnt, u32* ctr, u32 tot, u32* host,
-                                                        u32 words, u32* next, u32* next_ctr) {
-  shard_scan(cnt, ctr, tot, host, words, next, next_ctr);
+                                                        u32 words, u32* next, u32* next_ctr,
+                                                        const u32* gate) {
+  shard_scan(cnt, ctr, tot, host, words, next, next_ctr, gate);
 }
 __device__ inline void shard_scan(u32* cnt, u32* ctr, u32 tot, u32* host, u32 words, u32* next,
-                                  u32* next_ctr) {
+                                  u32* next_ctr, const u32* gate) {
   __shared__ u32 v[kShards];
   __shared__ u32 wmax[kShards / 64];
+  if (gate && gate_shut(gate)) next = nullptr;
   const u32 t = threadIdx.x, c = cnt[t];
   v[t] = c;
   u32 m = c;
@@ -567,15 +579,19 @@
                                                       Table T, u32* ckeys, u32* ccnt, u32* sync,
                                                       u32* cand, HotHdr* hdr,
                                                       HotEntry* __restrict__ dir, u32 nblk,
-                                                      u8* __restrict__ status) {
+                                                      u8* __restrict__ status,
+                                                      const HotHdr* prev_hdr,
+                                                      const HotEntry* prev_dir, u32* ctr) {
   constexpr u32 kPerBlock = kThreads * kRounds;
   constexpr u32 kL = 2 * kPerBlock;
   static_assert(kHotHist % kThreads == 0 && 4096 % kThreads == 0, "the last workgroup's shares");
   constexpr u32 kWords = 2 * kL > kHotHist ? 2 * kL : kHotHist;
   __shared__ u32 lds[kWords];
   __shared__ u32 part[kThreads];
-  __shared__ u32 sel[kHotMax];
-  __shared__ u32 best, nsel, last;
+  __shared__ u32 sel[kHotMax], selcnt[kHotMax];
+  __shared__ u32 best, nsel, last, own, kept;
+  constexpr u32 kPrevSet = 4096;
+  static_assert(kWords >= kPrevSet && kPrevSet * 2 >= kHotMax * 3, "the previous directory's set");
   if (blockIdx.x >= nblk) {
     constexpr u32 b4 = PHIP_ST_MERGED * 0x01010101u;
     const u64 head = min((u64)n, (u64)(-(uintptr_t)status & 15));
@@ -674,7 +690,7 @@
   for (u32 k = 0; k < kU; ++k) hh0[k] = k * kThreads + threadIdx.x < ncand ? hh0[k] & mask : ~0u;
   u32* hist = lds;
   for (u32 e = threadIdx.x; e < kHotHist; e += kThreads) hist[e] = 0;
-  if (threadIdx.x == 0) { best = kHotHist; nsel = 0; }
+  if (threadIdx.x == 0) { best = kHotHist; nsel = 0; own = 0; kept = 0; }
   __syncthreads();
   auto counts = [&](const u32 (&hh)[kU], u32 (&cc)[kU], u32 (&kk)[kU]) {
 #pragma unroll
@@ -729,7 +745,10 @@
     for (u32 k = 0; k < kU; ++k) {
       if (cc[k] < thresh) continue;
       const u32 idx = atomicAdd(&nsel, 1u);
-      if (idx < kHotMax) sel[idx] = kk[k] - 1;
+      if (idx < kHotMax) {
+        sel[idx] = kk[k] - 1;
+        selcnt[idx] = cc[k];
+      }
     }
   };
   pick(cc0, kk0);
@@ -740,12 +759,36 @@
   }
   __syncthreads();
   const u32 ns = min(nsel, kHotMax);
+  const u32 np = prev_hdr ? min(prev_hdr->n, kHotMax) : 0u;
+  for (u32 e = threadIdx.x; e < kPrevSet; e += kThreads) lds[e] = 0;
+  __syncthreads();
+  for (u32 j = threadIdx.x; j < np; j += kThreads) {
+    const u32 s = prev_dir[j].slot;
+    u32 ph = (s * 2654435761u) & (kPrevSet - 1);
+    for (;;) {
+      const u32 old = atomicCAS(&lds[ph], 0u, s + 1);
+      if (old == 0 || old == s + 1) break;
+      ph = (ph + 1) & (kPrevSet - 1);
+    }
+  }
+  __syncthreads();
+  u32 o = 0, kp = 0;
 #pragma unroll
   for (u32 k = 0; k < (kHotMax + kThreads - 1) / kThreads; ++k) {
     const u32 j = k * kThreads + threadIdx.x;
-    if (j < ns) dir[j] = hot_entry(T, sel[j]);
-  }
+    if (j >= ns) continue;
+    const u32 s = sel[j];
+    dir[j] = hot_entry(T, s);
+    o += selcnt[j];
+    for (u32 ph = (s * 2654435761u) & (kPrevSet - 1); lds[ph]; ph = (ph + 1) & (kPrevSet - 1))
+      if (lds[ph] == s + 1) { kp += selcnt[j]; break; }
+  }
+  if (o) atomicAdd(&own, o);
+  if (kp) atomicAdd(&kept, kp);
+  __syncthreads();
   if (threadIdx.x == 0) {
+    ctr[kCtrHotOwn] = own;
+    ctr[kCtrHotKept] = kept;
     hdr->n = nsel;
     hdr->thresh = thresh;
     st_co32(&sync[0], 0u);
@@ -1095,6 +1138,9 @@
 #ifndef PHIP_UNDO_NT
 #define PHIP_UNDO_NT 1
 #endif
+#ifndef PHIP_STATUS_IN_KERNEL
+#define PHIP_STATUS_IN_KERNEL 1
+#endif
 constexpr u32 kUndoFlushReserve = 64 * ((kHotMax + kFastBlock - 1) / kFastBlock);
 struct UndoLog {
   u64x2* base = nullptr;
@@ -1130,7 +1176,26 @@
 __global__ __launch_bounds__(kFastBlock) __attribute__((amdgpu_waves_per_eu(8, 8))) void k_receive_fast(
     In in, u32 lo, u32 n, Table T, Sharded miss, u32* ctr,
     const HotHdr* __restrict__ hot, const HotEntry* __restrict__ hot_dir, const u64* dtab,
-    u8* __restrict__ mark, UndoLog ulog, uint4* __restrict__ hot_zero) {
+    u8* __restrict__ mark, UndoLog ulog, uint4* __restrict__ hot_zero, u32 hot_kept,
+    const u32* gate, u8* __restrict__ status) {
+  if constexpr (Opt) {
+    const bool shut = gate && gate_shut(gate);
+    if (blockIdx.x == 0 && threadIdx.x == 0) ctr[kCtrGateShut] = shut;
+    if (shut) return;
+    if (PHIP_STATUS_IN_KERNEL == 1 && status) {
+      constexpr u32 b4 = PHIP_ST_MERGED * 0x01010101u;
+      const u64 head = min((u64)n, (u64)(-(uintptr_t)status & 15));
+      const u64 n16 = (n - head) / 16;
+      uint4* body = reinterpret_cast<uint4*>(status + head);
+      for (u64 k = (u64)blockIdx.x * kFastBlock + threadIdx.x; k < n16; k += (u64)gridDim.x * kFastBlock)
+        body[k] = uint4{b4, b4, b4, b4};
+      if (blockIdx.x == 0) {
+        if (threadIdx.x < head) status[threadIdx.x] = PHIP_ST_MERGED;
+        const u64 done = head + n16 * 16;
+        if (done + threadIdx.x < n) status[done + threadIdx.x] = PHIP_ST_MERGED;
+      }
+    }
+  }
   __shared__ u32 hslot[kHotLds];
   __shared__ u64 htag[kHotMax], hw0[kHotMax], hw1[kHotMax], hw2[kHotMax];
   __shared__ u32 hrec[kHotMax], haoff[kHotMax];
@@ -1161,6 +1226,17 @@
     hrec[j] = d.slot | (iso && (rec_flags(T.recs[d.slot]) & kRecDirty) ? 0x80000000u : 0u);
     haoff[j] = d.aoff;
     for (u32 k = 0; k < kHotTailWords; ++k) htail[k][j] = d.tail[k];
+    if (hot_kept) {
+      bool same = d.slot <= T.mask();
+      if (same) {
+        const Rec r = load_rec(&T.recs[d.slot]);
+        const bool arena = (r.name0 & 0xFFu) > kInlineName;
+        same = r.tag == d.tag && (rec_flags(r) & kRecPublished) &&
+               (arena ? (r.name0 & 0xFFu) : (r.name0 & ~0xFF00ull)) == d.w0 && r.name1 == d.w1 &&
+               r.name2 == d.w2 && (arena ? (u32)(r.name0 >> 32) : 0u) == d.aoff;
+      }
+      if (!same) continue;
+    }
     u32 hs = hot_home(d.tag);
     while (atomicCAS(&hslot[hs], 0u, j + 1) != 0) hs = (hs + 1) & (kHotLds - 1);
   }
@@ -1192,6 +1268,16 @@
     const u32 tid = chunk * 64 + lane;
     bool valid = tid < n;
     const u32 i = tid < n ? tid : n - 1;
+    if constexpr (Opt && PHIP_STATUS_IN_KERNEL == 2) {
+      if (status) {
+        constexpr u32 b4 = PHIP_ST_MERGED * 0x01010101u;
+        if ((u64)chunk * 64 + 64 <= n && ((uintptr_t)status & 15) == 0) {
+          if (lane < 4) reinterpret_cast<uint4*>(status + (size_t)chunk * 64)[lane] = uint4{b4, b4, b4, b4};
+        } else if (tid < n) {
+          status[tid] = PHIP_ST_MERGED;
+        }
+      }
+    }
     if constexpr (Opt && In::kSoa) {
       if constexpr (In::kOffs) {
         if (in.src.lim) {
diff --git a/patrol_amd/engine.py b/patrol_amd/engine.py
--- a/patrol_amd/engine.py
+++ b/patrol_amd/engine.py
@@ -190,8 +190,8 @@
         self.L.phip_set_timing(self.h, (2 if accumulate else 1) if on else 0)
 
     def last_stats(self):
-        out = (C.c_uint64 * 7)()
-        k = self.L.phip_last_stats(self.h, out, 7)
+        out = (C.c_uint64 * 9)()
+        k = self.L.phip_last_stats(self.h, out, 9)
         return tuple(int(out[i]) for i in range(k))
 
     def table_stats(self):
```

Measured after the change: 53.03 billion merges/s, median of 6. 2.4% higher.
